# Inception3D/Motion324

Hardware: AMD Instinct MI355X
Metric: frames/sec (32-frame clip, 2048 pts, 512x512) (higher is better)
Workload: dtype bf16; 1 GPU; Motion_Latent_Model.forward inference, B=1 x 32 frames x 2048 points x 512x512 video, 4096 surface samples, training.frames=32, random-init weights (one clip per GPU; BASELINE configs[1]); the clip sits in the replayed graph's input buffers in HBM; bf16 speed mode with the decoder's residual stream in bf16 and the head fused (no [rows, C] intermediate) (secondary.headline_without_precision_shortcu; parallelism=clip-parallel x1

## Files before the change

include/m324.h:

```cpp
#ifndef M324_H
#define M324_H

#ifdef __cplusplus
extern "C" {
#endif

typedef enum { M324_OK = 0, M324_ERR_INVALID = -1, M324_ERR_HIP = -2, M324_ERR_UNSUPPORTED = -3 } m324_status;
typedef enum { M324_F32 = 0, M324_BF16 = 1, M324_MXFP8 = 2 } m324_dtype;
typedef enum { M324_ACT_NONE = 0, M324_ACT_GELU = 1 } m324_act;
typedef enum { M324_AUX_NONE = 0, M324_AUX_STORE_PREACT = 1, M324_AUX_MUL_GELU_GRAD = 2, M324_AUX_QKV_HEADS = 3,
               M324_AUX_QKV_HEADS_VT = 4, M324_AUX_N3 = 5, M324_AUX_STORE_GELU_GRAD = 6, M324_AUX_MUL = 7 } m324_aux_mode;

int m324_abi_version(void);
int m324_last_error(char* buf, int n);
int m324_device_info(char* name, int n);
int m324_set_tunable(const char* name, int value);

typedef struct {
    const void* A;  long lda;
    const void* W;  long ldw;
    void* C;        long ldc;
    int M, N, K;
    int in_dtype, out_dtype;
    const float* bias;
    int act;
    const float* gamma;
    const float* residual; long ldr; int res_rows;
    int row_gin, row_gout, row_off;
    int batch;
    long strideA, strideW, strideC;
    void* aux; long ldaux; int aux_mode;
    void* qkv_q; void* qkv_k; void* qkv_v;
    const float* qkv_qw; const float* qkv_kw;
    float qkv_eps, qkv_qscale;
    int qkv_L, qkv_H;
    const float* ln_rowstat; const float* ln_colsum;
    float* ln_stats_out;
    void* ln_copy_out; long ln_ldcopy;
    int ln_ncb; float ln_eps;
} m324_gemm_args;
int m324_gemm(const m324_gemm_args* a, void* stream);
int m324_gemm_pair(const m324_gemm_args* a, const m324_gemm_args* b, void* stream);
int m324_gemm_plan(const m324_gemm_args* a, char* buf, int n);

int m324_mx_quant(const void* x, int x_dtype, long ldx, int rows, int K, void* q, long ldq, void* s, long lds, void* stream);
int m324_layernorm_mx(const float* x, long ldx, const float* w, const float* b, float eps, int rows, int C, void* q, long ldq,
                      void* s, long lds, void* stream);
int m324_gemm_mx(const m324_gemm_args* a, const void* A_scale, long lds_a, const void* W_scale, long lds_w, void* C_scale,
                 long lds_c, void* stream);

int m324_rowstats_finish(const float* part, int ncb, int M, float eps, float* rowstat, void* stream);
int m324_rowstats(const float* x, long ldx, int rows, int C, float eps, float* rowstat, void* copy, long ldcopy, void* stream);

int m324_n3_finish(const float* part, int ncb, int M, const float* bias3, float* out, void* stream);

int m324_gemm_tn(const void* X, long ldx, const void* Y, long ldy, float* C, long ldc, int M, int N, int Kc,
                 int slices, long strideC, void* stream);

int m324_layernorm(const float* x, long ldx, const float* w, const float* b, float eps,
                   void* y, long ldy, int out_dtype, int rows, int C,
                   int gin, int gout, int off, void* stream);
int m324_layernorm_pair(const float* x0, long ldx0, const float* w0, const float* b0, float eps0, void* y0, long ldy0, int rows0,
                        int gin0, int gout0, int off0, const float* x1, long ldx1, const float* w1, const float* b1, float eps1,
                        void* y1, long ldy1, int rows1, int gin1, int gout1, int off1, int C, int out_dtype, void* stream);
int m324_layernorm_in(const void* x, int x_dtype, long ldx, const float* w, const float* b, float eps,
                      void* y, long ldy, int out_dtype, int rows, int C,
                      int gin, int gout, int off, void* stream);

int m324_qkv_split(const void* q_src, long ldq, const void* k_src, long ldk, const void* v_src, long ldv,
                   const float* q_w, const float* k_w, float eps, float q_scale,
                   void* Q, void* K, void* V, void* Qt, void* Kt, void* Vt,
                   int B, int L, int H, int dtype, void* stream);

enum { M324_ATTN_Q_PRESCALED = 1, M324_ATTN_V_ROWMAJOR = 2, M324_ATTN_SCORES_BOUNDED = 4 };
int m324_attention(const void* Q, long q_bstride, const void* K, const void* Vt, void* O, long ldo,
                   int B, int H, int Lq, int Lk, float scale, int q_prescaled, float* lse, int dtype, void* stream);
int m324_attention_plan(int B, int H, int Lq, int Lk, int flags, int dtype, char* buf, int n);

int m324_attention_merge(const void* O0, const float* lse0, const void* O1, const float* lse1, const void* O2, const float* lse2,
                         long ldp, void* O, long ldo, int B, int H, int Lq, int dtype, void* stream);

int m324_patchify(const float* video, int F, int Hin, int Win, int size, int patch,
                  void* out, int Kp, int dtype, void* stream);
int m324_patchify_u8(const unsigned char* video, int F, int Hin, int Win, int size, int patch,
                     void* out, int Kp, int dtype, void* stream);

int m324_point_encode(const float* xyz, int P, void* out, long ld, int dtype, void* stream);
int m324_point_concat(const float* normal, const float* rgb, int P, void* feat, int C, int Kp,
                      int dtype, void* stream);

int m324_dino_cls_rows(const float* cls, const float* pos0, float* x, int F, int rows_per_frame, int C,
                       void* stream);

int m324_assemble_tokens(const float* dino_x, const float* dino_w, const float* dino_b, float eps_dino,
                         const float* pos, const float* sp0, const float* spr, const float* mesh,
                         const float* ln_w, float eps_in, float* out,
                         int B, int T, int K, int P, int C, float drop_p, unsigned long long drop_seed, void* stream);

int m324_linear_n3(const void* A, long lda, const float* W, const float* bias, float* out,
                   int M, int K, int dtype, void* stream);

int m324_mse(const float* pred, const float* target, long n, float weight, float* partial, float* out,
             void* stream);

int m324_smooth_trajectories(const float* trajs, float* tmp, float* out, int B, int T, int N,
                             float threshold, float sigma, void* stream);
int m324_smooth_savgol(const float* trajs, float* out, int B, int T, int N, const double* coef, int window, void* stream);
int m324_smooth_oneeuro(const float* trajs, float* out, int B, int T, int N, float mincutoff, float beta, float dcutoff,
                        void* stream);
int m324_nearest_point(const float* query, int n_query, const float* ref, int n_ref, int* index, void* stream);

int m324_transpose(const void* in, long ld_in, void* out, long ld_out, int rows, int cols, int rows_pad,
                   int dtype, void* stream);
int m324_colsum(const void* x, long ld, float* out, int rows, int cols, int dtype, int accumulate,
                float* scratch, int scratch_rows, void* stream);
typedef struct {
    float* dst;
    const float* src;
    long ld;
    int rows, cols;
    int accumulate;
    int chain;
} m324_colsum_item;
int m324_colsum_multi(const m324_colsum_item* items, int n, void* stream);
int m324_gelu(const void* z, void* h, long n, int dtype, void* stream);
int m324_gelu_bwd(const void* z, const void* dh, void* dz, long n, int dtype, void* stream);
int m324_layernorm_bwd(const float* x, long ldx, const float* w, float eps, const void* dy, long ldy, int dy_dtype,
                       float* dx, long lddx, int accumulate, float* partial, int n_partial, int rows, int C,
                       int gin, int gout, int off, void* stream);
int m324_layernorm_bwd_cast(const float* x, long ldx, const float* w, float eps, const void* dy, long ldy, int dy_dtype,
                            float* dx, long lddx, int accumulate, float* partial, int n_partial, int rows, int C,
                            int gin, int gout, int off, void* dx_bf16, long ldc, void* stream);

int m324_cast(const void* in, long ld_in, int in_dtype, void* out, long ld_out, int out_dtype, int rows, int cols,
              void* stream);
int m324_attention_delta(const void* O, const void* dO, long ld, float* D, int B, int H, int L, int dtype, void* stream);
int m324_attention_bwd(const void* Qs, long q_bstride, const void* K, const void* V, const void* dO, const float* lse,
                       const float* D, void* dQ, void* dK, void* dV, int B, int H, int Lq, int Lk, float scale,
                       int dtype, void* stream);
int m324_attention_bwd_mfma(const void* Qs, const void* Qst, long q_bstride, long qt_bstride, const void* K, const void* Kt,
                            const void* V, const void* dO, const void* dOt, const float* lse, const float* D,
                            void* dQ, void* dK, void* dV, int B, int H, int Lq, int Lk, float scale, void* stream);
int m324_qkv_split_bwd(const void* dQ, const void* dK, const void* dV, const void* q_raw, long ldq, const void* k_raw,
                       long ldk, const float* q_w, const float* k_w, float eps, void* dq_out, long ldoq, void* dk_out,
                       long ldok, void* dv_out, long ldov, float* partial, int n_partial, int B, int L, int H, int dtype,
                       void* stream);
int m324_linear_n3_bwd(const void* A, long lda, const float* W, const float* dout, void* dA, long ldda, float* partial,
                       int n_partial, int M, int K, int dtype, const void* mul, long ldmul, void* stream);
int m324_mse_bwd(const float* pred, const float* target, const float* grad_scale, float coef, float* d, long n,
                 void* stream);
int m324_adamw(float* p, const float* g, float* m, float* v, long n, float lr, float beta1, float beta2, float eps,
               float weight_decay, int step, const float* grad_scale, void* stream);
int m324_adamw_flat(float* p, const float* g, float* m, float* v, long n, long n_decay, float lr, float beta1, float beta2,
                    float eps, float weight_decay, int step, const float* grad_scale, void* stream);
typedef struct m324_mirror_item {
    long src_off, dst_off, dstT_off;
    long first_tile;
    int rows, cols, ldT, pad_;
} m324_mirror_item;
int m324_weight_mirror(const float* src, void* dst, void* dstT, const m324_mirror_item* items_dev, int n_items, long n_tiles,
                       void* stream);
int m324_grad_sumsq(float* g, long n, int sanitize, float* partial, float* out, int accumulate, void* stream);

typedef struct m324_comm m324_comm;
int m324_comm_unique_id(char* hex, int n);
int m324_comm_init(m324_comm** comm, const char* unique_id_hex, int rank, int world);
int m324_comm_allreduce(m324_comm* comm, void* buf, long count, int dtype, int average, void* stream);
int m324_comm_allgather(m324_comm* comm, const void* send, void* recv, long count_per_rank, int dtype, void* stream);
int m324_comm_destroy(m324_comm* comm);

#ifdef __cplusplus
}
#endif
#endif
```

motion324_amd/Pcd_motion.py:

```python
from __future__ import annotations

import contextlib
import os

from typing import Dict, Optional

import torch
import torch.nn as nn
import torch.nn.functional as F

from . import ops, parallel, switches
from .easydict import EasyDict as edict
from .image_encoder import DINO_EPS, DinoEncoder
from .latent import MotionLatent
from .lib import ACT_GELU, M324Error
from .loss import MSELossComputer
from .prepared import Prepared, bump_generation, compute_dtype, pad_k
from .timing import span
from . import transformer as _transformer
from .transformer import (LN_EPS, LNFold, QK_Norm_CrossAttentionBlock, QK_Norm_TransformerBlock, fusion_off, init_weights,
                          mx_scope)

AUTO_GRAPH = switches.flag("M324_AUTO_GRAPH")
FUSE_HEAD_N3 = switches.flag("M324_FUSE_HEAD")
# ... 535 lines not shown
                    pf, Q = hoisted[b]
                elif paired is not None:
                    pf, Q = paired
                else:
                    pf = self._point_features(P, pcd[b, n0:n1], nrm[b, n0:n1].contiguous(), rgb[b, n0:n1].contiguous())
                if tchunk < T and hoisted is None and paired is None:
                    with span("stage:decoder_cross_attn_block", 0.0):
                        Q = dec.project_q(P, pf, 1, n1 - n0)
                for t0 in range(0, T, tchunk):
                    if frame_chunks:
                        t0 = min(t0, T - tchunk)
                    t1 = min(T, t0 + tchunk)
                    with span("stage:decoder_cross_attn_block", 0.0):
                        x, fold_d = self.decoder_block(P, Kd[b * T + t0:b * T + t1], Vd[b * T + t0:b * T + t1], pf,
                                                       None if (hoisted is None and paired is None and tchunk == T) else Q)
                    if cap is not None and n0 == 0 and n1 == N and tchunk == T:
                        cap.setdefault("decoder_out_t0", []).append(x[:N].clone())
                    if fold_d is not None:
                        hw, hcs, hb = P.folded(head_ln.weight, head_ln.bias, head_fc1.weight, head_fc1.bias)
                        h, lnk = fold_d.xb, dict(ln=fold_d.ln(head_ln.eps, hcs))
                    else:
                        h = torch.empty(x.shape, dtype=P.dtype, device=dev)
                        ops.layernorm(x, P.vec(head_ln.weight), P.vec(head_ln.bias), head_ln.eps, h)
                        hw, hb, lnk = P.mat(head_fc1.weight), P.vec(head_fc1.bias), {}
                    whole = n0 == 0 and n1 == N and tchunk == T
                    o = out[b] if whole else torch.empty((t1 - t0, n1 - n0, 3), dtype=torch.float32, device=dev)
                    if FUSE_HEAD_N3 and P.dtype == torch.bfloat16 and C % 256 == 0 and not torch.is_grad_enabled():
                        part = torch.empty((C // 64, x.shape[0], 3), dtype=torch.float32, device=dev)
                        ops.gemm(h, hw, None, bias=hb, act=ACT_GELU, n3=(w3, part), **lnk)
                        ops.n3_finish(part, b3, o)
                    else:
                        h2 = torch.empty(x.shape, dtype=P.dtype, device=dev)
                        ops.gemm(h, hw, h2, bias=hb, act=ACT_GELU, **lnk)
                        ops.linear_n3(h2, w3, b3, o)
                    if not whole:
                        out[b, t0:t1, n0:n1] = o
        if cap is not None and "decoder_out_t0" in cap:
            cap["decoder_out_t0"] = torch.stack(cap["decoder_out_t0"], dim=0)
        return out

    def _forward(self, sample: Dict[str, torch.Tensor], shard):
        latent_in = sample.get("m324_latent")
        encode_only = bool(sample.get("m324_encode_only", False))
        keep_latent = bool(sample.get("m324_keep_latent", False)) or encode_only
        if latent_in is not None or keep_latent:
            self._latent_guard(shard, latent_in is not None and keep_latent)
        if latent_in is not None:
            return self._forward_decode(sample, latent_in)
        ref_pcd = sample["rgb_video"] if encode_only else sample["ref_pcd"]
        dev = ref_pcd.device
        if dev.type != "cuda":
            raise M324Error("motion324_amd.Motion_Latent_Model runs only on a HIP device (model.to('cuda'), inputs on "
                            "'cuda'); there is no CPU fallback on this path")
        P = Prepared.for_module(self, dev, compute_dtype())
        mx = mx_scope(_transformer.MX_ROLES if shard is None and self.mx_effective() else ())
        cap = getattr(self, "_capture", None)
        B, N = ref_pcd.shape[0], (0 if encode_only else ref_pcd.shape[1])
        C, K = self.embed_dim, self.num_learnable_tokens
        S = sample["ref_shape_pcd"].shape[1]

        main_stream = torch.cuda.current_stream(dev)
        side = _side_stream(dev) if OVERLAP_SHAPE_ENCODER and cap is None else None
        if side is not None:
            side.wait_stream(main_stream)
        mesh_in, anchor_in = sample.get("m324_mesh_tokens"), sample.get("m324_anchor_tokens")
        keep_reuse = bool(sample.get("m324_keep_reuse", False))
        if (mesh_in is not None or anchor_in is not None) and (shard is not None or cap is not None):
            raise M324Error("m324_mesh_tokens / m324_anchor_tokens: single-GPU inference windows only")
        with torch.cuda.stream(side) if side is not None else contextlib.nullcontext():
            if mesh_in is not None:
                mesh = self._f32c(mesh_in).reshape(B * K, C)
            else:
                pts = self._point_features(P, self._f32c(sample["ref_shape_pcd"]).reshape(-1, 3),
                                           self._f32c(sample["ref_shape_normals"]), self._f32c(sample["ref_shape_rgbs"]))
                query = P.derived(f"latent_tokens_x{B}", (self.learnable_tokens,),
                                  lambda: self.learnable_tokens.detach().to(device=P.device, dtype=torch.float32).reshape(K, C).repeat(B, 1))
                mesh = self.encoder_cross_attn.run(P, query, pts, B, K, S)
                if cap is not None:
                    cap["shape_point_feat"], cap["encoder_out"] = pts.clone(), mesh.clone()
                for blk in self.points_transformer_blocks:
                    blk.run(P, mesh, B, K)
                if cap is not None:
                    cap["mesh_feat"] = mesh.clone()
            hoisted = None
            if (HOIST_DECODER_Q and side is not None and not encode_only and torch.cuda.is_current_stream_capturing()
                    and DECODE_ROWS // (sample["rgb_video"].shape[1] + (anchor_in is not None)) >= N):
                pcd_h, nrm_h, rgb_h = (self._f32c(sample[k]) for k in ("ref_pcd", "ref_normal", "ref_rgb"))
                hoisted = []
                for b in range(B):
                    pf_b = self._point_features(P, pcd_h[b], nrm_h[b].contiguous(), rgb_h[b].contiguous())
                    hoisted.append((pf_b, self.decoder_cross_attn.project_q(P, pf_b, 1, N)))

        video = sample["rgb_video"]
        T_full = video.shape[1]
        t0, kv_gather = 0, None
        if shard is not None:
            from . import parallel
            rank, world, group, t_local_of = shard
            if t_local_of is not None:
                T_full = t_local_of
            mine = parallel.partition(T_full, world, rank)
            if len(mine) == 0:
                raise M324Error(f"frame-parallel forward: {T_full} frames cannot feed {world} ranks")
            t0 = mine.start
            if t_local_of is None:
                video = video[:, mine.start:mine.stop]
            elif video.shape[1] != len(mine):
                raise M324Error(f"frame-parallel forward: rank {rank} of {world} owns {len(mine)} of {T_full} frames, rgb_video has {video.shape[1]}")
        video = video.detach().contiguous() if video.dtype == torch.uint8 else self._f32c(video)
        _, T, Hin, Win, _ = video.shape
        Pn = self.num_patches_h * self.num_patches_w
        if anchor_in is not None:
            if B != 1 or tuple(anchor_in.shape) != (1 + Pn, C):
                raise M324Error(f"m324_anchor_tokens: expected [{1 + Pn}, {C}] with one sample per call, got {tuple(anchor_in.shape)} (B = {B})")
            dino_x = torch.empty(((T + 1) * (1 + Pn), C), dtype=torch.float32, device=dev)
            ops.cast(self._f32c(anchor_in), torch.float32, out=dino_x[:1 + Pn])
            with mx:
                self.image_encoder.run(P, video.reshape(T, Hin, Win, 3), out=dino_x[1 + Pn:])
            T += 1
            T_full = T
        else:
            with mx:
                dino_x = self.image_encoder.run(P, video.reshape(B * T, Hin, Win, 3))

        if side is not None:
            main_stream.wait_stream(side)
            mesh.record_stream(main_stream)

        enc = self.image_encoder.model
        drop_p = self.drop_rate if self.training else 0.0
        drop_seed = int(torch.randint(0, 2 ** 62, (1,)).item()) if drop_p > 0.0 else 0
        pos = self._video_pos(P, T_full)[t0 * Pn:(t0 + T) * Pn]
        sp_rest = P.f32(self.special_token_rest).reshape(4, C)
        sp_first = P.f32(self.special_token_0).reshape(4, C) if t0 == 0 else sp_rest
        tok = ops.assemble_tokens(dino_x, P.vec(enc.norm.weight), P.vec(enc.norm.bias), DINO_EPS, pos, sp_first, sp_rest,
                                  mesh, P.vec(self.transformer_input_layernorm.weight),
                                  self.transformer_input_layernorm.eps, B, T, K, Pn, drop_p, drop_seed)
        Lt = 4 + K + Pn
        if cap is not None:
            dn = torch.empty((B * T * Pn, C), dtype=torch.float32, device=dev)
            ops.layernorm(dino_x, P.vec(enc.norm.weight), P.vec(enc.norm.bias), DINO_EPS, dn, row_map=(Pn, Pn + 1, 1))
            cap["dino_tokens"], cap["trunk_in"] = dn, tok.clone()

        if shard is not None and parallel.collectives_on(shard[1]):
            rank, world, group = shard[:3]
            kv_gather = _KVGather(B, T, Lt, parallel.counts(T_full, world), group, dev, rank=rank)

        fold = None
        if LNFold.usable(P, tok.shape[0], C) and "trunk.mlp" not in mx.roles:
            fold = LNFold(tok)
            if "trunk.qkv" not in mx.roles:
                fold.from_stream(tok, self.global_transformer_blocks[0].norm1.eps)
        n_pairs = len(self.global_transformer_blocks)
        for i, (gblk, lblk) in enumerate(zip(self.global_transformer_blocks, self.local_transformer_blocks)):
            with mx:
                gblk.run(P, tok, B, T * Lt, kv_gather=kv_gather, fold=fold)
                lblk.run(P, tok, B * T, Lt, fold=fold, feed_next=i + 1 < n_pairs)
            if cap is not None and "trunk_block0" not in cap:
                cap["trunk_block0"] = tok.clone()
        if cap is not None:
            cap["trunk_out"] = tok.clone()

        latent = None
        if keep_latent:
            latent = torch.empty((B * T, K * C), dtype=torch.float32, device=dev)
            ops.cast(tok.view(B * T, Lt * C)[:, 4 * C:(4 + K) * C], torch.float32, out=latent)
            latent = latent.view(B, T, K, C)
        if encode_only:
            return edict(input_data=sample, latent=latent)
        out = self._decode(P, sample, tok, (K, Lt, 4), B, T, hoisted, cap)

        if shard is not None and parallel.collectives_on(shard[1]):
            rank, world, group = shard[:3]
            frames = parallel.counts(T_full, world)
            buf = torch.zeros((max(frames), B, N, 3), dtype=torch.float32, device=dev)
            buf[:T] = out.transpose(0, 1)
            parts = torch.empty((world,) + tuple(buf.shape), dtype=torch.float32, device=dev)
            from . import graph
            seg = graph.active_segmenter()
            if seg is not None:
                seg.cut(lambda: parallel.all_gather_into(parts, buf, group=group))
            else:
                parallel.all_gather_into(parts, buf, group=group)
            if all(f == frames[0] for f in frames):
                out = parts.reshape(T_full, B, N, 3).transpose(0, 1).contiguous()
            else:
                out = torch.cat([parts[r, :f] for r, f in enumerate(frames)], dim=0).transpose(0, 1).contiguous()
        result = edict(input_data=sample, pcd_moved=out)
        if latent is not None:
            result.latent = latent
        if keep_reuse:
            Ld = 1 + Pn
            anchor = dino_x[:Ld] if B == 1 else dino_x.view(B, T, Ld, C)[:, 0].reshape(B * Ld, C).contiguous()
            result.reuse = edict(mesh_tokens=mesh, anchor_tokens=anchor)
        if "point_clouds" in sample:
            m = self.loss_computer(out, sample["point_clouds"].to(dev))
            lm = edict()
            lm.loss = m.loss
            lm.xyz_loss = m.coord_mse_loss
            result.loss_metrics = lm
        return result
```

motion324_amd/csrc/attention.hip:

```cpp
#include <stdio.h>
#include <stdlib.h>
#include <type_traits>
#include "common.h"

namespace {

constexpr int QW = 32;
constexpr int NW = 4;
constexpr int QB = QW * NW;
constexpr int KV = 64;
constexpr float LOG2E = 1.4426950408889634f;

__device__ __forceinline__ int k_off(int row, int c16) { return row * 128 + ((c16 ^ ((row >> 1) & 7)) << 4); }
typedef __attribute__((address_space(3))) void lds_ptr_t;
typedef __attribute__((address_space(1))) const void glb_ptr_t;
constexpr int ASTAGE = 16384;

__device__ __forceinline__ void dma_piece(__amdgpu_buffer_rsrc_t rs, unsigned char* lds, unsigned voff, unsigned soff) {
    __builtin_amdgcn_raw_ptr_buffer_load_lds(rs, (lds_ptr_t*)lds, 16, voff, soff, 0, 0);
}
__device__ __forceinline__ __amdgpu_buffer_rsrc_t dma_rsrc(const void* base, long bytes) {
    return __builtin_amdgcn_make_buffer_rsrc(const_cast<void*>(base), 0, (int)(bytes > 0x7FFFFFFFl ? 0x7FFFFFFFl : bytes), 0x00020000);
}


template <typename F>
__device__ __forceinline__ void store_row_chunks(const f32x16 (&acc)[2], float mul, int hi, bool ok, F&& put) {
#pragma unroll
    for (int db = 0; db < 2; ++db)
#pragma unroll
        for (int gp = 0; gp < 2; ++gp) {
            uint32_t a[2], c[2];
#pragma unroll
            for (int k = 0; k < 2; ++k) {
                a[k] = pack_bf16x2(acc[db][(2 * gp) * 4 + 2 * k] * mul, acc[db][(2 * gp) * 4 + 2 * k + 1] * mul);
                c[k] = pack_bf16x2(acc[db][(2 * gp + 1) * 4 + 2 * k] * mul, acc[db][(2 * gp + 1) * 4 + 2 * k + 1] * mul);
                const auto sw = __builtin_amdgcn_permlane32_swap(a[k], c[k], false, false);
                a[k] = sw[0];
                c[k] = sw[1];
            }
            if (ok) put(db * 4 + 2 * gp + hi, make_uint4(a[0], a[1], c[0], c[1]));
        }
}

typedef __attribute__((ext_vector_type(4))) short a_s16x4_t;
typedef __attribute__((ext_vector_type(8))) short a_s16x8_t;
typedef __attribute__((address_space(3))) a_s16x4_t a_lds_s16x4_t;

template <bool PRESCALED, int NQ, int NWV, bool VROW = false, int NST = 3>
__global__ __launch_bounds__(NWV * 64, NWV == 8 ? (VROW ? 2 : 4) : ((NST == 1 || NST == 2) ? 4 : 1)) void attn_bf16_kernel(const bf16_t* __restrict__ Q, long q_bstride,
                                                        const bf16_t* __restrict__ K, const bf16_t* __restrict__ Vt,
                                                        bf16_t* __restrict__ O, long ldo, int H, int Lq, int Lk,
                                                        int Lkp, float scale_log2e, float* __restrict__ lse, int nqt) {
    __shared__ __attribute__((aligned(1024))) unsigned char smem[NST * ASTAGE + (NST == 1 ? NWV * 4096 : 0)];
    const int tid = threadIdx.x, lane = tid & 63;
    const int wave = __builtin_amdgcn_readfirstlane(tid >> 6);
    const int l31 = lane & 31, hi = lane >> 5;
    int b = blockIdx.z, h = blockIdx.y, qt = blockIdx.x;
    if (nqt > 0) {
        const int nb = gridDim.x, q = nb >> 3, r = nb & 7, x = qt & 7, loc = qt >> 3;
        const int lid = (x < r ? x * (q + 1) : r * (q + 1) + (x - r) * q) + loc;
        qt = lid % nqt;
        h = (lid / nqt) % H;
        b = lid / (nqt * H);
    }
    const int q0 = (qt * NWV + wave) * (QW * NQ);

    const bf16_t* Qh = Q + (long)b * q_bstride + (long)h * Lq * 64;
    const bf16_t* Kh = K + ((long)b * H + h) * (long)Lk * 64;
    const bf16_t* Vh = Vt + ((long)b * H + h) * (VROW ? (long)Lk * 64 : 64 * (long)Lkp);

    bf16x8 qf[NQ][4];
#pragma unroll
    for (int n = 0; n < NQ; ++n) {
        const int q = q0 + n * QW + l31;
        const bool ok = q < Lq;
#pragma unroll
        for (int ks = 0; ks < 4; ++ks) {
            uint4 v = ok ? *reinterpret_cast<const uint4*>(Qh + (long)q * 64 + ks * 16 + hi * 8) : make_uint4(0, 0, 0, 0);
            qf[n][ks] = *reinterpret_cast<bf16x8*>(&v);
        }
    }

    constexpr int GPW = 8 / NWV;
    constexpr int PPT = 2 * GPW;
    unsigned vk[GPW], vv[GPW];
#pragma unroll
    for (int i = 0; i < GPW; ++i) {
        const int srow = (wave * GPW + i) * 8 + (lane >> 3);
        const int scol = ((lane & 7) ^ ((srow >> 1) & 7)) * 8;
        vk[i] = (unsigned)((srow * 64 + scol) * 2);
        vv[i] = VROW ? (unsigned)((srow * 64 + ((lane & 7) ^ (4 * ((srow >> 1) & 1))) * 8) * 2)
                     : (unsigned)(((long)srow * Lkp + scol) * 2);
    }
    const __amdgpu_buffer_rsrc_t rk = dma_rsrc(Kh, (long)Lk * 128);
    const __amdgpu_buffer_rsrc_t rv = dma_rsrc(Vh, VROW ? (long)Lk * 128 : 64l * Lkp * 2);
    auto issue_tile = [&](int t) {
        const int kv0 = t * KV;
        unsigned char* sk = smem + (t % NST) * ASTAGE + wave * (GPW * 1024);
        unsigned char* sv = sk + 8192;
#pragma unroll
        for (int i = 0; i < GPW; ++i) dma_piece(rk, sk + i * 1024, vk[i], (unsigned)(kv0 * 128));
#pragma unroll
        for (int i = 0; i < GPW; ++i) dma_piece(rv, sv + i * 1024, vv[i], (unsigned)(VROW ? kv0 * 128 : kv0 * 2));
    };

    f32x16 o[NQ][2];
#pragma unroll
    for (int n = 0; n < NQ; ++n)
#pragma unroll
        for (int i = 0; i < 2; ++i)
#pragma unroll
            for (int r = 0; r < 16; ++r) o[n][i][r] = 0.f;
    constexpr float THR = 8.0f;
    float m_ref[NQ], l_run[NQ];
#pragma unroll
    for (int n = 0; n < NQ; ++n) m_ref[n] = 0.f, l_run[n] = 0.f;
    bool first = true;

    const int nt = (Lk + KV - 1) / KV;
    issue_tile(0);
    if (NST != 2 && nt > 1) issue_tile(1);
    const int ko0 = k_off(l31, hi);

    const bool idle = q0 >= Lq;
    auto tiles = [&](auto guard_tag) {
        constexpr bool GUARD = decltype(guard_tag)::value;
        for (int t = 0; t < nt; ++t) {
            if (NST != 2 && t + 1 < nt) asm volatile("s_waitcnt vmcnt(%0)" ::"n"(PPT) : "memory");
            else asm volatile("s_waitcnt vmcnt(0)" ::: "memory");
            __builtin_amdgcn_s_barrier();
            asm volatile("" ::: "memory");
            if (NST == 2) {
                if (t + 1 < nt) issue_tile(t + 1);
            } else if (t + 2 < nt) issue_tile(t + 2);
            if (GUARD && idle) continue;
            const unsigned char* sk = smem + (t % NST) * ASTAGE;
            const unsigned char* sv = sk + 8192;
            const int kos = ko0 + (t % NST) * ASTAGE;

            f32x16 s[NQ][2];
    #pragma unroll
            for (int n = 0; n < NQ; ++n) {
                const float init = PRESCALED ? -m_ref[n] : -m_ref[n] / scale_log2e;
    #pragma unroll
                for (int kb = 0; kb < 2; ++kb)
    #pragma unroll
                    for (int r = 0; r < 16; ++r) s[n][kb][r] = init;
            }
            if constexpr (NQ == 1 && !VROW && NWV == 8) {
                bf16x8 kfa[8];
                auto rd = [&](int i) { kfa[i] = *reinterpret_cast<const bf16x8*>(smem + (i & 1) * 4096 + (kos ^ ((i >> 1) << 5))); };
                rd(0); rd(1); rd(2); rd(3);
                __builtin_amdgcn_sched_barrier(0);
    #pragma unroll
                for (int i = 0; i < 8; ++i) {
                    s[0][i & 1] = __builtin_amdgcn_mfma_f32_32x32x16_bf16(kfa[i], qf[0][i >> 1], s[0][i & 1], 0, 0, 0);
                    if (i + 4 < 8) rd(i + 4);
                    __builtin_amdgcn_sched_group_barrier(0x008, 1, 0);
                    if (i + 4 < 8) __builtin_amdgcn_sched_group_barrier(0x100, 1, 0);
                }
            } else {
    #pragma unroll
            for (int kb = 0; kb < 2; ++kb)
    #pragma unroll
                for (int ks = 0; ks < 4; ++ks) {
                    bf16x8 kf = *reinterpret_cast<const bf16x8*>(smem + kb * 4096 + (kos ^ (ks << 5)));
    #pragma unroll
                    for (int n = 0; n < NQ; ++n)
                        s[n][kb] = __builtin_amdgcn_mfma_f32_32x32x16_bf16(kf, qf[n][ks], s[n][kb], 0, 0, 0);
                }
            }
            if (!PRESCALED) {
    #pragma unroll
                for (int n = 0; n < NQ; ++n)
    #pragma unroll
                    for (int kb = 0; kb < 2; ++kb)
    #pragma unroll
                        for (int r = 0; r < 16; ++r) s[n][kb][r] *= scale_log2e;
            }
            const int kv0 = t * KV;
            if (kv0 + KV > Lk) {
    #pragma unroll
                for (int n = 0; n < NQ; ++n)
    #pragma unroll
                    for (int kb = 0; kb < 2; ++kb)
    #pragma unroll
                        for (int r = 0; r < 16; ++r)
                            if (kv0 + kb * 32 + (r & 3) + 8 * (r >> 2) + 4 * hi >= Lk) s[n][kb][r] = -INFINITY;
            }
            float mx[NQ];
            bool calm = true;
    #pragma unroll
            for (int n = 0; n < NQ; ++n) {
                float v = -INFINITY;
    #pragma unroll
                for (int kb = 0; kb < 2; ++kb)
    #pragma unroll
                    for (int r = 0; r < 16; ++r) v = fmaxf(v, s[n][kb][r]);
                mx[n] = v;
                calm = calm && (v <= THR);
            }
            if (first || !__all(calm)) {
    #pragma unroll
                for (int n = 0; n < NQ; ++n) {
                    mx[n] = fmaxf(mx[n], __shfl_xor(mx[n], 32, 64));
                    const float shift = first ? mx[n] : fmaxf(mx[n], 0.f);
                    const float alpha = first ? 0.f : __builtin_amdgcn_exp2f(-shift);
                    m_ref[n] += shift;
                    l_run[n] *= alpha;
    #pragma unroll
                    for (int i = 0; i < 2; ++i)
    #pragma unroll
                        for (int r = 0; r < 16; ++r) o[n][i][r] *= alpha;
    #pragma unroll
                    for (int kb = 0; kb < 2; ++kb)
    #pragma unroll
                        for (int r = 0; r < 16; ++r) s[n][kb][r] -= shift;
                }
                first = false;
            }
            bf16x8 pf[NQ][4];
    #pragma unroll
            for (int n = 0; n < NQ; ++n) {
                f32x2 rs2 = {0.f, 0.f};
    #pragma unroll
                for (int kb = 0; kb < 2; ++kb) {
                    uint32_t pk[8];
    #pragma unroll
                    for (int r = 0; r < 16; r += 2) {
                        f32x2 p = {__builtin_amdgcn_exp2f(s[n][kb][r]), __builtin_amdgcn_exp2f(s[n][kb][r + 1])};
                        rs2 += p;
                        pk[r >> 1] = pack_bf16x2(p[0], p[1]);
                    }
                    uint4 lo = make_uint4(pk[0], pk[1], pk[2], pk[3]), hi4 = make_uint4(pk[4], pk[5], pk[6], pk[7]);
                    pf[n][kb * 2] = *reinterpret_cast<bf16x8*>(&lo);
                    pf[n][kb * 2 + 1] = *reinterpret_cast<bf16x8*>(&hi4);
                }
                l_run[n] += rs2[0] + rs2[1];
            }

    #pragma unroll
            for (int j = 0; j < 4; ++j) {
    #pragma unroll
                for (int db = 0; db < 2; ++db) {
                    bf16x8 vf;
                    if constexpr (VROW) {
                        const int li = lane & 15, gg = lane >> 4;
                        const int d0 = db * 32 + 16 * (gg & 1) + 4 * (li & 3);
                        const int off = (j * 16 + 4 * hi + (li >> 2)) * 128 + (((d0 >> 3) ^ (4 * ((li >> 3) & 1))) << 4) + ((d0 & 7) << 1);
                        const a_s16x4_t lo = __builtin_amdgcn_ds_read_tr16_b64_v4i16((a_lds_s16x4_t*)(sv + off));
                        const a_s16x4_t hi4 = __builtin_amdgcn_ds_read_tr16_b64_v4i16((a_lds_s16x4_t*)(sv + off + 8 * 128));
                        const a_s16x8_t v8 = __builtin_shufflevector(lo, hi4, 0, 1, 2, 3, 4, 5, 6, 7);
                        vf = __builtin_bit_cast(bf16x8, v8);
                    } else {
                        vf = *reinterpret_cast<const bf16x8*>(smem + 8192 + db * 4096 + (kos ^ (j << 5)));
                    }
    #pragma unroll
                    for (int n = 0; n < NQ; ++n)
                        o[n][db] = __builtin_amdgcn_mfma_f32_32x32x16_bf16(vf, pf[n][j], o[n][db], 0, 0, 0);
                }
            }

        }
    };
    if (NWV == 4 && NQ == 1 && NST == 3 && (qt + 1) * NWV * QW > Lq) tiles(std::true_type{});
    else tiles(std::false_type{});

#pragma unroll
    for (int n = 0; n < NQ; ++n) {
        const float l_tot = l_run[n] + __shfl_xor(l_run[n], 32, 64);
        const float inv = 1.0f / l_tot;
        const int q = q0 + n * QW + l31;
        if (lse && q < Lq && hi == 0) lse[((long)b * H + h) * Lq + q] = m_ref[n] + log2f(l_tot);
        unsigned char* scr = NST == 1 ? smem + ASTAGE + wave * 4096 : smem + ((nt + (wave >> 2)) % NST) * ASTAGE + (wave & 3) * 4096;
        if (n > 0) asm volatile("s_waitcnt lgkmcnt(0)" ::: "memory");
#pragma unroll
        for (int db = 0; db < 2; ++db)
#pragma unroll
            for (int gp = 0; gp < 2; ++gp) {
                uint32_t a[2], c[2];
#pragma unroll
                for (int k = 0; k < 2; ++k) {
                    a[k] = pack_bf16x2(o[n][db][(2 * gp) * 4 + 2 * k] * inv, o[n][db][(2 * gp) * 4 + 2 * k + 1] * inv);
                    c[k] = pack_bf16x2(o[n][db][(2 * gp + 1) * 4 + 2 * k] * inv, o[n][db][(2 * gp + 1) * 4 + 2 * k + 1] * inv);
                    const auto sw = __builtin_amdgcn_permlane32_swap(a[k], c[k], false, false);
                    a[k] = sw[0];
                    c[k] = sw[1];
                }
                const int chunk = db * 4 + 2 * gp + hi;
                *reinterpret_cast<uint4*>(scr + l31 * 128 + ((chunk ^ (l31 & 7)) << 4)) = make_uint4(a[0], a[1], c[0], c[1]);
            }
        const int r8 = lane >> 3, c8 = lane & 7;
        bf16_t* obase = O + ((long)b * Lq + q0 + n * QW) * ldo + h * 64 + c8 * 8;
#pragma unroll
        for (int p = 0; p < 4; ++p) {
            const int r = p * 8 + r8;
            const uint4 v = *reinterpret_cast<const uint4*>(scr + r * 128 + ((c8 ^ (r & 7)) << 4));
            if (q0 + n * QW + r < Lq) *reinterpret_cast<uint4*>(obase + (long)r * ldo) = v;
        }
    }
}

template <int FB, bool NT>
__global__ __launch_bounds__(256, 3) void attn_frames_kernel(const bf16_t* __restrict__ Q, const bf16_t* __restrict__ K,
                                                             const bf16_t* __restrict__ Vt, bf16_t* __restrict__ O, long ldo, int H, int Lq,
                                                             int Lk, int Lkp, float* __restrict__ lse) {
    __shared__ __attribute__((aligned(1024))) unsigned char smem[2 * ASTAGE + 4 * 4096];
    const int tid = threadIdx.x, lane = tid & 63;
    const int wave = __builtin_amdgcn_readfirstlane(tid >> 6);
    const int l31 = lane & 31, hi = lane >> 5;
    const int h = blockIdx.y, qt = blockIdx.x, b0 = blockIdx.z * FB;
    const int q0 = (qt * 4 + wave) * QW;
    const int q = q0 + l31;
    const bf16_t* Qh = Q + (long)h * Lq * 64;
    bf16x8 qf[4];
#pragma unroll
    for (int ks = 0; ks < 4; ++ks) {
        uint4 v = q < Lq ? *reinterpret_cast<const uint4*>(Qh + (long)q * 64 + ks * 16 + hi * 8) : make_uint4(0, 0, 0, 0);
        qf[ks] = *reinterpret_cast<bf16x8*>(&v);
    }
    unsigned vk[2], vv[2];
#pragma unroll
    for (int i = 0; i < 2; ++i) {
        const int srow = (wave * 2 + i) * 8 + (lane >> 3);
        const int scol = ((lane & 7) ^ ((srow >> 1) & 7)) * 8;
        vk[i] = (unsigned)((srow * 64 + scol) * 2);
        vv[i] = (unsigned)((srow * Lkp + scol) * 2);
    }
    auto issue = [&](int j) {
        const long bh = (long)(b0 + j) * H + h;
        const __amdgpu_buffer_rsrc_t rk = dma_rsrc(K + bh * (long)Lk * 64, (long)Lk * 128);
        const __amdgpu_buffer_rsrc_t rv = dma_rsrc(Vt + bh * 64 * Lkp, 64l * Lkp * 2);
        unsigned char* sk = smem + (j & 1) * ASTAGE + wave * 2048;
#pragma unroll
        for (int i = 0; i < 2; ++i) dma_piece(rk, sk + i * 1024, vk[i], 0u);
#pragma unroll
        for (int i = 0; i < 2; ++i) dma_piece(rv, sk + 8192 + i * 1024, vv[i], 0u);
    };
    unsigned char* scr = smem + 2 * ASTAGE + wave * 4096;
    const int r8 = lane >> 3, c8 = lane & 7;
    auto flush = [&](int j) {
        bf16_t* obase = O + ((long)(b0 + j) * Lq + q0) * ldo + h * 64 + c8 * 8;
#pragma unroll
        for (int p = 0; p < 4; ++p) {
            const int r = p * 8 + r8;
            const uint4 v = *reinterpret_cast<const uint4*>(scr + r * 128 + ((c8 ^ (r & 7)) << 4));
            if (q0 + r < Lq) {
                if (NT) __builtin_nontemporal_store(*reinterpret_cast<const f32x4*>(&v), reinterpret_cast<f32x4*>(obase + (long)r * ldo));
                else *reinterpret_cast<uint4*>(obase + (long)r * ldo) = v;
            }
        }
    };
    const int ko0 = k_off(l31, hi);
    issue(0);
#pragma unroll 1
    for (int j = 0; j < FB; ++j) {
        asm volatile("s_waitcnt vmcnt(0)" ::: "memory");
        __builtin_amdgcn_s_barrier();
        asm volatile("" ::: "memory");
        if (j + 1 < FB) issue(j + 1);
        if (j > 0) flush(j - 1);
        const int kos = ko0 + (j & 1) * ASTAGE;
        f32x16 s[2];
#pragma unroll
        for (int kb = 0; kb < 2; ++kb) {
#pragma unroll
            for (int r = 0; r < 16; ++r) s[kb][r] = 0.f;
#pragma unroll
            for (int ks = 0; ks < 4; ++ks) {
                const bf16x8 kf = *reinterpret_cast<const bf16x8*>(smem + kb * 4096 + (kos ^ (ks << 5)));
                s[kb] = __builtin_amdgcn_mfma_f32_32x32x16_bf16(kf, qf[ks], s[kb], 0, 0, 0);
            }
        }
        if (Lk < KV) {
#pragma unroll
            for (int kb = 0; kb < 2; ++kb)
#pragma unroll
                for (int r = 0; r < 16; ++r)
                    if (kb * 32 + (r & 3) + 8 * (r >> 2) + 4 * hi >= Lk) s[kb][r] = -INFINITY;
        }
        float mx = -INFINITY;
#pragma unroll
        for (int kb = 0; kb < 2; ++kb)
#pragma unroll
            for (int r = 0; r < 16; ++r) mx = fmaxf(mx, s[kb][r]);
        mx = fmaxf(mx, __shfl_xor(mx, 32, 64));
        f32x2 rs2 = {0.f, 0.f};
        bf16x8 pf[4];
#pragma unroll
        for (int kb = 0; kb < 2; ++kb) {
            uint32_t pk[8];
#pragma unroll
            for (int r = 0; r < 16; r += 2) {
                f32x2 p = {__builtin_amdgcn_exp2f(s[kb][r] - mx), __builtin_amdgcn_exp2f(s[kb][r + 1] - mx)};
                rs2 += p;
                pk[r >> 1] = pack_bf16x2(p[0], p[1]);
            }
            uint4 lo = make_uint4(pk[0], pk[1], pk[2], pk[3]), hi4 = make_uint4(pk[4], pk[5], pk[6], pk[7]);
            pf[kb * 2] = *reinterpret_cast<bf16x8*>(&lo);
            pf[kb * 2 + 1] = *reinterpret_cast<bf16x8*>(&hi4);
        }
        f32x16 o[2];
#pragma unroll
        for (int db = 0; db < 2; ++db) {
#pragma unroll
            for (int r = 0; r < 16; ++r) o[db][r] = 0.f;
#pragma unroll
            for (int jj = 0; jj < 4; ++jj) {
                const bf16x8 vf = *reinterpret_cast<const bf16x8*>(smem + 8192 + db * 4096 + (kos ^ (jj << 5)));
                o[db] = __builtin_amdgcn_mfma_f32_32x32x16_bf16(vf, pf[jj], o[db], 0, 0, 0);
            }
        }
        float l_tot = rs2[0] + rs2[1];
        l_tot += __shfl_xor(l_tot, 32, 64);
        const float inv = 1.0f / l_tot;
        if (lse && q < Lq && hi == 0) lse[((long)(b0 + j) * H + h) * Lq + q] = mx + log2f(l_tot);
        store_row_chunks(o, inv, hi, true, [&](int chunk, uint4 v) {
            *reinterpret_cast<uint4*>(scr + l31 * 128 + ((chunk ^ (l31 & 7)) << 4)) = v;
        });
    }
    flush(FB - 1);
}


template <int NWV>
__device__ __forceinline__ void dma_rows(unsigned char* part, __amdgpu_buffer_rsrc_t rs, long row_stride, int row0, long col0, int wave,
                                         int lane) {
    constexpr int G = 8 / NWV;
    const unsigned soff = (unsigned)(((long)row0 * row_stride + col0) * 2);
#pragma unroll
    for (int i = 0; i < G; ++i) {
        const int r = (wave * G + i) * 8 + (lane >> 3);
        const int c = (lane & 7) ^ ((r >> 1) & 7);
        __builtin_amdgcn_raw_ptr_buffer_load_lds(rs, (lds_ptr_t*)(part + (wave * G + i) * 8 * 128), 16,
                                                 (unsigned)(((long)r * row_stride + c * 8) * 2), soff, 0, 0);
    }
}

__device__ __forceinline__ void pack_frags(const f32x16 (&x)[2], bf16x8 (&f)[4]) {
#pragma unroll
    for (int kb = 0; kb < 2; ++kb) {
        uint32_t pk[8];
#pragma unroll
        for (int r = 0; r < 16; r += 2) pk[r >> 1] = pack_bf16x2(x[kb][r], x[kb][r + 1]);
        uint4 lo = make_uint4(pk[0], pk[1], pk[2], pk[3]), hi4 = make_uint4(pk[4], pk[5], pk[6], pk[7]);
        f[kb * 2] = *reinterpret_cast<bf16x8*>(&lo);
        f[kb * 2 + 1] = *reinterpret_cast<bf16x8*>(&hi4);
    }
}

template <int NWV>
__global__ __launch_bounds__(NWV * 64) void attn_bwd_dq_mfma_kernel(const bf16_t* __restrict__ Qs, long q_bstride,
                                                               const bf16_t* __restrict__ K, const bf16_t* __restrict__ V,
// ... 413 lines not shown
        }
        float mx = -INFINITY;
#pragma unroll
        for (int kb = 0; kb < 2; ++kb)
#pragma unroll
            for (int r = 0; r < 16; ++r) mx = fmaxf(mx, s[kb][r]);
        mx = fmaxf(mx, __shfl_xor(mx, 32, 64));
        const float m_new = fmaxf(m_run, mx * scale_log2e);
        const float alpha = exp2f(m_run - m_new);
        m_run = m_new;
        float rs = 0.f;
#pragma unroll
        for (int kb = 0; kb < 2; ++kb)
#pragma unroll
            for (int r = 0; r < 16; ++r) {
                s[kb][r] = exp2f(fmaf(s[kb][r], scale_log2e, -m_new));
                rs += s[kb][r];
            }
        l_run = l_run * alpha + rs;
#pragma unroll
        for (int i = 0; i < 2; ++i)
#pragma unroll
            for (int r = 0; r < 16; ++r) o[i][r] *= alpha;
#pragma unroll
        for (int kb = 0; kb < 2; ++kb)
#pragma unroll
            for (int r = 0; r < 16; ++r) {
                const int kv = kb * 32 + (r & 3) + 8 * (r >> 2) + 4 * hi;
#pragma unroll
                for (int db = 0; db < 2; ++db)
                    o[db] = __builtin_amdgcn_mfma_f32_32x32x2f32(sv[(db * 32 + l31) * FLD + kv], s[kb][r], o[db], 0, 0, 0);
            }
    }
    const float l_tot = l_run + __shfl_xor(l_run, 32, 64);
    const float inv = 1.0f / l_tot;
    const int q = q0 + l31;
    if (lse && q < Lq && hi == 0) lse[((long)b * H + h) * Lq + q] = m_run + log2f(l_tot);
    if (q < Lq) {
        float* orow = O + ((long)b * Lq + q) * ldo + h * 64;
#pragma unroll
        for (int db = 0; db < 2; ++db)
#pragma unroll
            for (int g = 0; g < 4; ++g) {
                float4 w = make_float4(o[db][g * 4 + 0] * inv, o[db][g * 4 + 1] * inv, o[db][g * 4 + 2] * inv,
                                       o[db][g * 4 + 3] * inv);
                *reinterpret_cast<float4*>(orow + db * 32 + g * 8 + hi * 4) = w;
            }
    }
}

}

void m324_attn_pwg_launch(const void* Q, long q_bstride, const void* K, const void* Vt, void* O, long ldo, int B, int H, int Lq, int Lk,
                          float* lse, bool bounded, hipStream_t s);

enum AttnFamily { ATTN_F32, ATTN_PWG, ATTN_PWG_BOUNDED, ATTN_FRAMES, ATTN_BF16 };
struct AttnPlan {
    AttnFamily family;
    bool ps, vrow;
    int nw, nst;
    dim3 grid;
    unsigned threads;
    int nqt;
};

static AttnPlan attn_plan(int B, int H, int Lq, int Lk, int flags, int dtype) {
    AttnPlan p{};
    p.nw = NW, p.nst = 3, p.threads = 256;
    p.grid = dim3(ceil_div(Lq, QB), H, B);
    if (dtype != M324_BF16) {
        p.family = ATTN_F32;
        return p;
    }
    const bool vrow = (flags & M324_ATTN_V_ROWMAJOR) != 0, ps = (flags & M324_ATTN_Q_PRESCALED) != 0;
    const int fnw = m324::tunable(m324::TUN_ATTN_NW);
    const bool w8 = fnw ? fnw == 8 : (Lq >= 2048 && Lk >= 512);
    if (m324::tunable(m324::TUN_ATTN_PWG) != 0 && ps && !vrow && fnw == 0 && Lq >= 2048 && Lk >= 512) {
        p.family = (flags & M324_ATTN_SCORES_BOUNDED) ? ATTN_PWG_BOUNDED : ATTN_PWG;
        p.grid = dim3((unsigned)((long)ceil_div(Lq, 256) * H * B));
        return p;
    }
    p.family = ATTN_BF16, p.ps = ps, p.vrow = vrow, p.nw = w8 ? 8 : 4, p.threads = p.nw * 64;
    p.grid.x = ceil_div(Lq, w8 ? 2 * QB : QB);
    const bool one_tile = ps && !w8 && !vrow && Lk <= KV;
    if (w8 || (!one_tile && p.grid.x > 1 && (long)p.grid.x * H * B >= 512)) {
        p.nqt = (int)p.grid.x;
        p.grid = dim3(p.grid.x * H * B, 1, 1);
    }
    if (ps && !w8 && Lk > KV && Lk <= 16 * KV) {
        p.nst = 2;
    } else if (one_tile && (flags & 256) && B % 2 == 0 && Lq >= 512 && m324::tunable(m324::TUN_ATTN_EXP) != 8) {
        p.family = ATTN_FRAMES;
        p.grid.z = B / 2;
    } else if (one_tile) {
        p.nst = 1;
    }
    return p;
}

static constexpr int attn_key(bool ps, int nw, bool vrow, int nst) { return (int)ps | nw << 1 | (int)vrow << 5 | nst << 6; }

extern "C" int m324_attention(const void* Q, long q_bstride, const void* K, const void* Vt, void* O, long ldo, int B,
                              int H, int Lq, int Lk, float scale, int q_prescaled, float* lse, int dtype, void* stream) {
    M324_REQUIRE(Q && K && Vt && O, "m324_attention: null pointer");
    M324_REQUIRE(B > 0 && H > 0 && Lq > 0 && Lk > 0, "m324_attention: empty problem B=%d H=%d Lq=%d Lk=%d", B, H, Lq, Lk);
    M324_REQUIRE(ldo >= (long)H * 64, "m324_attention: ldo too small");
    M324_REQUIRE(H <= 65535 && B <= 65535, "m324_attention: grid too large");
    M324_REQUIRE(!(q_prescaled & M324_ATTN_V_ROWMAJOR) || dtype == M324_BF16, "m324_attention: row-major V needs the bf16 kernel (transposing LDS reads)");
    if (dtype != M324_BF16 && dtype != M324_F32) M324_FAIL(M324_ERR_UNSUPPORTED, "m324_attention: dtype %d", dtype);
    M324_REQUIRE(dtype == M324_BF16 ? (ldo * 2) % 8 == 0 : ldo % 4 == 0, "m324_attention: ldo misaligned");
    const int Lkp = (Lk + 63) / 64 * 64;
    hipStream_t s = (hipStream_t)stream;
    const float sl = (q_prescaled & M324_ATTN_Q_PRESCALED) ? 1.0f : scale * LOG2E;
    const AttnPlan p = attn_plan(B, H, Lq, Lk, (q_prescaled & 7) | (q_bstride == 0 ? 256 : 0), dtype);
#define M324_ATTN(PS, NWV, VROW, NST)                                                                                   \
    case attn_key(PS, NWV, VROW, NST):                                                                                  \
        hipLaunchKernelGGL((attn_bf16_kernel<PS, 1, NWV, VROW, NST>), p.grid, dim3(p.threads), 0, s,                    \
                           (const bf16_t*)Q, q_bstride, (const bf16_t*)K, (const bf16_t*)Vt, (bf16_t*)O, ldo, H, Lq, Lk, \
                           Lkp, sl, lse, p.nqt);                                                                         \
        break
    switch (p.family) {
        case ATTN_F32:
            hipLaunchKernelGGL(attn_f32_kernel, p.grid, dim3(p.threads), 0, s, (const float*)Q, q_bstride, (const float*)K,
                               (const float*)Vt, (float*)O, ldo, H, Lq, Lk, Lkp, sl, lse);
            break;
        case ATTN_PWG:
        case ATTN_PWG_BOUNDED:
            M324_REQUIRE((long)ceil_div(Lq, 256) * H * B < (1l << 31), "m324_attention: grid too large");
            m324_attn_pwg_launch(Q, q_bstride, K, Vt, O, ldo, B, H, Lq, Lk, lse, p.family == ATTN_PWG_BOUNDED, s);
            break;
        case ATTN_FRAMES:
            hipLaunchKernelGGL((attn_frames_kernel<2, true>), p.grid, dim3(p.threads), 0, s, (const bf16_t*)Q,
                               (const bf16_t*)K, (const bf16_t*)Vt, (bf16_t*)O, ldo, H, Lq, Lk, Lkp, lse);
            break;
        case ATTN_BF16:
            switch (attn_key(p.ps, p.nw, p.vrow, p.nst)) {
                M324_ATTN(true, 4, false, 3); M324_ATTN(true, 8, false, 3);
                M324_ATTN(false, 4, false, 3); M324_ATTN(false, 8, false, 3);
                M324_ATTN(true, 4, true, 3); M324_ATTN(true, 8, true, 3);
                M324_ATTN(false, 4, true, 3); M324_ATTN(false, 8, true, 3);
                M324_ATTN(true, 4, false, 2); M324_ATTN(true, 4, true, 2);
                M324_ATTN(true, 4, false, 1);
                default:
                    M324_FAIL(M324_ERR_UNSUPPORTED, "m324_attention: attn_bf16_kernel<%d, 1, %d, %d, %d> is not built", (int)p.ps, p.nw,
                              (int)p.vrow, p.nst);
            }
            break;
    }
#undef M324_ATTN
    M324_CHECK_LAUNCH("m324_attention");
    return M324_OK;
}

extern "C" int m324_attention_plan(int B, int H, int Lq, int Lk, int flags, int dtype, char* buf, int n) {
    M324_REQUIRE(buf && n > 0 && B > 0 && H > 0 && Lq > 0 && Lk > 0, "m324_attention_plan: bad arguments");
    const AttnPlan p = attn_plan(B, H, Lq, Lk, flags, dtype);
    const char* tf[2] = {"false", "true"};
    char name[96];
    switch (p.family) {
        case ATTN_F32: snprintf(name, sizeof(name), "attn_f32_kernel"); break;
        case ATTN_PWG: snprintf(name, sizeof(name), "attn_pwg_kernel"); break;
        case ATTN_PWG_BOUNDED: snprintf(name, sizeof(name), "attn_pwg_bounded_kernel"); break;
        case ATTN_FRAMES: snprintf(name, sizeof(name), "attn_frames_kernel<2, true>"); break;
        case ATTN_BF16: snprintf(name, sizeof(name), "attn_bf16_kernel<%s, 1, %d, %s, %d>", tf[p.ps], p.nw, tf[p.vrow], p.nst); break;
    }
    snprintf(buf, (size_t)n, "%s grid=%ldx%ux%u", name, (long)p.grid.x * p.threads, p.grid.y, p.grid.z);
    return p.family == ATTN_F32 ? 0 : p.nw;
}

extern "C" int m324_attention_bwd_mfma(const void* Qs, const void* Qst, long q_bstride, long qt_bstride, const void* K,
                                       const void* Kt, const void* V, const void* dO, const void* dOt, const float* lse,
                                       const float* D, void* dQ, void* dK, void* dV, int B, int H, int Lq, int Lk, float scale,
                                       void* stream) {
    M324_REQUIRE(Qs && Qst && K && Kt && V && dO && dOt && lse && D && dQ && dK && dV, "m324_attention_bwd_mfma: null pointer");
    M324_REQUIRE(B > 0 && H > 0 && Lq > 0 && Lk > 0 && H <= 65535 && B <= 65535, "m324_attention_bwd_mfma: bad sizes");
    const int Lkp = (Lk + 63) / 64 * 64, Lqp = (Lq + 63) / 64 * 64;
    hipStream_t s = (hipStream_t)stream;
    const int fbw = m324::tunable(m324::TUN_ATTN_BWD_NW);
    const bool big = Lk >= 1024;
    const bool dq8 = fbw == 8 || fbw == 84, dkv8 = fbw == 8 || fbw == 48 || fbw == 2;
    if (fbw == 2 && big)
        hipLaunchKernelGGL(attn_bwd_dq2_mfma_kernel, dim3(ceil_div(Lq, 2 * QB), H, B), dim3(256), 0, s, (const bf16_t*)Qs, q_bstride,
                           (const bf16_t*)K, (const bf16_t*)V, (const bf16_t*)Kt, (const bf16_t*)dO, lse, D, (bf16_t*)dQ, H, Lq, Lk, Lkp, scale);
    else if (dq8)
        hipLaunchKernelGGL(attn_bwd_dq_mfma_kernel<8>, dim3(ceil_div(Lq, 2 * QB), H, B), dim3(512), 0, s, (const bf16_t*)Qs,
                           q_bstride, (const bf16_t*)K, (const bf16_t*)V, (const bf16_t*)Kt, (const bf16_t*)dO, lse, D,
                           (bf16_t*)dQ, H, Lq, Lk, Lkp, scale);
    else
        hipLaunchKernelGGL(attn_bwd_dq_mfma_kernel<4>, dim3(ceil_div(Lq, QB), H, B), dim3(256), 0, s, (const bf16_t*)Qs,
                           q_bstride, (const bf16_t*)K, (const bf16_t*)V, (const bf16_t*)Kt, (const bf16_t*)dO, lse, D,
                           (bf16_t*)dQ, H, Lq, Lk, Lkp, scale);
    if (dkv8)
        hipLaunchKernelGGL(attn_bwd_dkv_mfma_kernel<8>, dim3(ceil_div(Lk, 2 * QB), H, B), dim3(512), 0, s, (const bf16_t*)Qs,
                           (const bf16_t*)Qst, q_bstride, qt_bstride, (const bf16_t*)K, (const bf16_t*)V, (const bf16_t*)dO,
                           (const bf16_t*)dOt, lse, D, (bf16_t*)dK, (bf16_t*)dV, H, Lq, Lk, Lqp);
    else
        hipLaunchKernelGGL(attn_bwd_dkv_mfma_kernel<4>, dim3(ceil_div(Lk, QB), H, B), dim3(256), 0, s, (const bf16_t*)Qs,
                           (const bf16_t*)Qst, q_bstride, qt_bstride, (const bf16_t*)K, (const bf16_t*)V, (const bf16_t*)dO,
                           (const bf16_t*)dOt, lse, D, (bf16_t*)dK, (bf16_t*)dV, H, Lq, Lk, Lqp);
    M324_CHECK_LAUNCH("m324_attention_bwd_mfma");
    return M324_OK;
}
```

motion324_amd/csrc/elementwise.hip:

```cpp
#include "common.h"

namespace {

constexpr int LN_MAXV = 4;

__device__ __forceinline__ long remap_row(long r, int gin, int gout, int off) {
    return gin > 0 ? (r / gin) * gout + (r % gin) + off : r;
}

#define LN_FOR(i, c) _Pragma("unroll") for (int i = 0, c = lane * 4; i < LN_MAXV; ++i, c += 256) if (c < C)

__device__ __forceinline__ void row_load(float4 (&v)[LN_MAXV], const float* src, int lane, int C) {
    LN_FOR(i, c) v[i] = *reinterpret_cast<const float4*>(src + c);
}
__device__ __forceinline__ void row_stats(const float4 (&v)[LN_MAXV], int lane, int C, float eps, float& mean, float& rstd) {
    float s = 0.f;
    LN_FOR(i, c) s += v[i].x + v[i].y + v[i].z + v[i].w;
    mean = wave_sum(s) / (float)C;
    float q = 0.f;
    LN_FOR(i, c) {
        float a = v[i].x - mean, b = v[i].y - mean, cc = v[i].z - mean, d = v[i].w - mean;
        q += a * a + b * b + cc * cc + d * d;
    }
    rstd = rsqrtf(wave_sum(q) / (float)C + eps);
}

template <typename T>
__device__ __forceinline__ void store4(T* p, float a, float b, float c, float d);
template <>
__device__ __forceinline__ void store4<float>(float* p, float a, float b, float c, float d) {
    *reinterpret_cast<float4*>(p) = make_float4(a, b, c, d);
}
template <>
__device__ __forceinline__ void store4<bf16_t>(bf16_t* p, float a, float b, float c, float d) {
    *reinterpret_cast<uint2*>(p) = make_uint2(pack_bf16x2(a, b), pack_bf16x2(c, d));
}
template <typename T>
__device__ __forceinline__ float4 load4(const T* p);
template <>
__device__ __forceinline__ float4 load4<float>(const float* p) { return *reinterpret_cast<const float4*>(p); }
template <>
__device__ __forceinline__ float4 load4<bf16_t>(const bf16_t* p) {
    uint2 u = *reinterpret_cast<const uint2*>(p);
    return make_float4(__uint_as_float(u.x << 16), __uint_as_float(u.x & 0xffff0000u), __uint_as_float(u.y << 16),
                       __uint_as_float(u.y & 0xffff0000u));
}

template <typename T, typename TX = float>
__global__ __launch_bounds__(256) void layernorm1_kernel(const TX* __restrict__ x, long ldx, const float* __restrict__ w,
                                                         const float* __restrict__ b, float eps, T* __restrict__ y, long ldy,
                                                         int rows, int C, int gin, int gout, int off) {
    const int lane = threadIdx.x & 63;
    const long row = (long)blockIdx.x * 4 + (threadIdx.x >> 6);
    if (row >= rows) return;
    const TX* xr = x + remap_row(row, gin, gout, off) * ldx;
    float4 v[LN_MAXV];
    LN_FOR(i, c) v[i] = load4<TX>(xr + c);
    float mean, rstd;
    row_stats(v, lane, C, eps, mean, rstd);
    T* yr = y + row * ldy;
    LN_FOR(i, c) {
        float4 ww = *reinterpret_cast<const float4*>(w + c);
        float4 bb = b ? *reinterpret_cast<const float4*>(b + c) : make_float4(0.f, 0.f, 0.f, 0.f);
        store4<T>(yr + c, (v[i].x - mean) * rstd * ww.x + bb.x, (v[i].y - mean) * rstd * ww.y + bb.y,
                  (v[i].z - mean) * rstd * ww.z + bb.z, (v[i].w - mean) * rstd * ww.w + bb.w);
    }
}

template <typename T, typename TX = float>
__device__ __forceinline__ void ln_rows2(const TX* __restrict__ x, long ldx, const float* __restrict__ w, const float* __restrict__ b,
                                         float eps, T* __restrict__ y, long ldy, int rows, int C, int gin, int gout, int off, int block) {
    const int lane = threadIdx.x & 63;
    const long row0 = (long)block * 8 + (threadIdx.x >> 6) * 2;
    if (row0 >= rows) return;
    const bool two = row0 + 1 < rows;
    const long row1 = two ? row0 + 1 : row0;
    const TX* xa = x + remap_row(row0, gin, gout, off) * ldx;
    const TX* xb = x + remap_row(row1, gin, gout, off) * ldx;
    float4 va[LN_MAXV], vb[LN_MAXV];
    LN_FOR(i, c) { va[i] = load4<TX>(xa + c); vb[i] = load4<TX>(xb + c); }
    float sa = 0.f, sb = 0.f;
    LN_FOR(i, c) { sa += va[i].x + va[i].y + va[i].z + va[i].w; sb += vb[i].x + vb[i].y + vb[i].z + vb[i].w; }
    wave_sum2(sa, sb);
    const float ma = sa / (float)C, mb = sb / (float)C;
    float qa = 0.f, qb = 0.f;
    LN_FOR(i, c) {
        float p = va[i].x - ma, q = va[i].y - ma, r = va[i].z - ma, t = va[i].w - ma;
        qa += p * p + q * q + r * r + t * t;
        p = vb[i].x - mb, q = vb[i].y - mb, r = vb[i].z - mb, t = vb[i].w - mb;
        qb += p * p + q * q + r * r + t * t;
    }
    wave_sum2(qa, qb);
    const float ra = rsqrtf(qa / (float)C + eps), rb = rsqrtf(qb / (float)C + eps);
    T* ya = y + row0 * ldy;
    T* yb = y + row1 * ldy;
    LN_FOR(i, c) {
        const float4 ww = *reinterpret_cast<const float4*>(w + c);
        const float4 bb = b ? *reinterpret_cast<const float4*>(b + c) : make_float4(0.f, 0.f, 0.f, 0.f);
        store4<T>(ya + c, (va[i].x - ma) * ra * ww.x + bb.x, (va[i].y - ma) * ra * ww.y + bb.y,
                  (va[i].z - ma) * ra * ww.z + bb.z, (va[i].w - ma) * ra * ww.w + bb.w);
        store4<T>(yb + c, (vb[i].x - mb) * rb * ww.x + bb.x, (vb[i].y - mb) * rb * ww.y + bb.y,
                  (vb[i].z - mb) * rb * ww.z + bb.z, (vb[i].w - mb) * rb * ww.w + bb.w);
    }
}

template <typename T, typename TX = float>
__global__ __launch_bounds__(256) void layernorm_kernel(const TX* __restrict__ x, long ldx, const float* __restrict__ w,
                                                        const float* __restrict__ b, float eps, T* __restrict__ y, long ldy,
                                                        int rows, int C, int gin, int gout, int off) {
    ln_rows2<T, TX>(x, ldx, w, b, eps, y, ldy, rows, C, gin, gout, off, (int)blockIdx.x);
}

struct LnProblem {
    const float* x; long ldx;
    const float* w; const float* b; float eps;
    void* y; long ldy;
    int rows, gin, gout, off;
};
template <typename T>
__global__ __launch_bounds__(256) void layernorm_pair_kernel(LnProblem p0, LnProblem p1, int C, int blocks0) {
    if ((int)blockIdx.x < blocks0)
        ln_rows2<T, float>(p0.x, p0.ldx, p0.w, p0.b, p0.eps, (T*)p0.y, p0.ldy, p0.rows, C, p0.gin, p0.gout, p0.off, (int)blockIdx.x);
    else
        ln_rows2<T, float>(p1.x, p1.ldx, p1.w, p1.b, p1.eps, (T*)p1.y, p1.ldy, p1.rows, C, p1.gin, p1.gout, p1.off, (int)blockIdx.x - blocks0);
}

__global__ __launch_bounds__(256) void rowstats_finish_kernel(const float2* __restrict__ part, int ncb, int M, float eps,
                                                              float2* __restrict__ rowstat) {
    const long m = (long)blockIdx.x * 256 + threadIdx.x;
    if (m >= M) return;
    if ((ncb & 1) == 0) {
        const int h = ncb >> 1;
        float mean[2], m2[2];
        for (int half = 0; half < 2; ++half) {
            const float2 p0 = part[(long)(half * h) * M + m];
            mean[half] = p0.x * (1.0f / 64.0f), m2[half] = p0.y;
            for (int i = 1; i < h; ++i) {
                const float2 pb = part[(long)(half * h + i) * M + m];
                const float d = pb.x * (1.0f / 64.0f) - mean[half];
                mean[half] = fmaf(d, 1.0f / (float)(i + 1), mean[half]);
                m2[half] = m2[half] + fmaf(d * d, 64.0f * (float)i / (float)(i + 1), pb.y);
            }
        }
        const float d = mean[1] - mean[0];
        const float mm2 = (m2[0] + m2[1]) + (d * d) * (32.0f * (float)h);
        const float mean_ = fmaf(0.5f, d, mean[0]);
        const float rstd = rsqrtf(mm2 / (64.0f * (float)ncb) + eps);
        rowstat[m] = make_float2(rstd, -rstd * mean_);
        return;
    }
    float s = 0.f;
    for (int b = 0; b < ncb; ++b) s += part[(long)b * M + m].x;
    const float n = 64.0f * (float)ncb, mean = s / n;
    float m2 = 0.f;
    for (int b = 0; b < ncb; ++b) {
        const float2 pb = part[(long)b * M + m];
        const float d = pb.x * (1.0f / 64.0f) - mean;
        m2 += fmaf(64.0f * d, d, pb.y);
    }
    const float rstd = rsqrtf(m2 / n + eps);
    rowstat[m] = make_float2(rstd, -rstd * mean);
}

__global__ __launch_bounds__(256) void rowstats_kernel(const float* __restrict__ x, long ldx, int rows, int C, float eps,
                                                       float2* __restrict__ rowstat, bf16_t* __restrict__ copy, long ldcopy) {
    const int lane = threadIdx.x & 63;
    const long row = (long)blockIdx.x * 4 + (threadIdx.x >> 6);
    if (row >= rows) return;
    float4 v[LN_MAXV];
    row_load(v, x + row * ldx, lane, C);
    float mean, rstd;
    row_stats(v, lane, C, eps, mean, rstd);
    if (lane == 0) rowstat[row] = make_float2(rstd, -rstd * mean);
    if (copy) {
        LN_FOR(i, c) store4<bf16_t>(copy + row * ldcopy + c, v[i].x, v[i].y, v[i].z, v[i].w);
    }
}

template <typename T>
__global__ __launch_bounds__(256) void qkv_split_kernel(const T* __restrict__ qs, long ldq, const T* __restrict__ ks, long ldk,
                                                        const T* __restrict__ vs, long ldv, const float* __restrict__ qw,
                                                        const float* __restrict__ kw, float eps, float q_scale,
                                                        T* __restrict__ Q, T* __restrict__ K, T* __restrict__ V,
                                                        T* __restrict__ Qt, T* __restrict__ Kt, T* __restrict__ Vt, int L, int H,
                                                        int Lp) {
    __shared__ float tile[64][65];
    const int t = threadIdx.x, tok = t >> 2, part = t & 3;
    const int b = blockIdx.z, h = blockIdx.y, l0 = blockIdx.x * 64;
    const int l = l0 + tok;
    const bool ok = l < L;
    const long srow = (long)b * L + l;
    const long hbase = ((long)b * H + h);

    auto one = [&](const T* src, long ld, const float* w, float post, T* dst, T* dstT) {
        float v[16];
        if (ok) {
            const T* p = src + srow * ld + h * 64 + part * 16;
            float lo[8], hi8[8];
            load8(p, lo);
            load8(p + 8, hi8);
#pragma unroll
            for (int i = 0; i < 8; ++i) { v[i] = lo[i]; v[8 + i] = hi8[i]; }
        } else {
#pragma unroll
            for (int i = 0; i < 16; ++i) v[i] = 0.f;
        }
        if (w) {
            float ss = 0.f;
#pragma unroll
            for (int i = 0; i < 16; ++i) ss += v[i] * v[i];
            ss += __shfl_xor(ss, 1, 64);
            ss += __shfl_xor(ss, 2, 64);
            const float r = rsqrtf(ss * (1.0f / 64.0f) + eps);
#pragma unroll
            for (int i = 0; i < 16; ++i) v[i] = v[i] * r * w[part * 16 + i];
        }
        if (post != 1.0f) {
#pragma unroll
            for (int i = 0; i < 16; ++i) v[i] *= post;
        }
        if (dst && ok) {
            T* o = dst + (hbase * L + l) * 64 + part * 16;
            const float lo[8] = {v[0], v[1], v[2], v[3], v[4], v[5], v[6], v[7]};
            const float hi8[8] = {v[8], v[9], v[10], v[11], v[12], v[13], v[14], v[15]};
            store8(o, lo);
            store8(o + 8, hi8);
        }
        if (dstT) {
            __syncthreads();
#pragma unroll
            for (int i = 0; i < 16; ++i) tile[part * 16 + i][tok] = v[i];
            __syncthreads();
            const int d = t >> 2;
            T* o = dstT + (hbase * 64 + d) * (long)Lp + l0 + part * 16;
            const float* tr = &tile[d][part * 16];
            const float c0[8] = {tr[0], tr[1], tr[2], tr[3], tr[8], tr[9], tr[10], tr[11]};
            const float c1[8] = {tr[4], tr[5], tr[6], tr[7], tr[12], tr[13], tr[14], tr[15]};
            store8(o, c0);
            store8(o + 8, c1);
        }
    };
    if (qs) one(qs, ldq, qw, q_scale, Q, Qt);
    if (ks) one(ks, ldk, kw, 1.0f, K, Kt);
    if (vs) one(vs, ldv, nullptr, 1.0f, V, Vt);
}

template <typename TIN>
__device__ __forceinline__ float patch_tap(const TIN* p, int c) {
    if constexpr (sizeof(TIN) == 1) return (float)p[c] / 255.0f;
    else return p[c];
}
template <typename T, typename TIN>
__global__ __launch_bounds__(256) void patchify_kernel(const TIN* __restrict__ video, int F, int Hin, int Win, int size,
                                                       int patch, T* __restrict__ out, int Kp) {
    const long idx = (long)blockIdx.x * 256 + threadIdx.x;
    const long total = (long)F * size * size;
    if (idx >= total) return;
    const int ox = (int)(idx % size), oy = (int)((idx / size) % size), f = (int)(idx / ((long)size * size));
    const float sh = (float)Hin / (float)size, sw = (float)Win / (float)size;
    float fy = fmaxf(sh * ((float)oy + 0.5f) - 0.5f, 0.f), fx = fmaxf(sw * ((float)ox + 0.5f) - 0.5f, 0.f);
    const int y0 = min((int)fy, Hin - 1), x0 = min((int)fx, Win - 1);
    const int y1 = min(y0 + 1, Hin - 1), x1 = min(x0 + 1, Win - 1);
    const float ly = fy - (float)y0, lx = fx - (float)x0;
    const float hy = 1.f - ly, hx = 1.f - lx;
    const TIN* base = video + (long)f * Hin * Win * 3;
    const TIN* p00 = base + ((long)y0 * Win + x0) * 3;
    const TIN* p01 = base + ((long)y0 * Win + x1) * 3;
    const TIN* p10 = base + ((long)y1 * Win + x0) * 3;
    const TIN* p11 = base + ((long)y1 * Win + x1) * 3;
    const float mean[3] = {0.485f, 0.456f, 0.406f}, stdv[3] = {0.229f, 0.224f, 0.225f};
    const int g = size / patch;
    const int py = oy / patch, ky = oy % patch, px = ox / patch, kx = ox % patch;
    T* orow = out + ((long)f * g * g + (long)py * g + px) * Kp;
#pragma unroll
    for (int c = 0; c < 3; ++c) {
        const float v = hy * (hx * patch_tap(p00, c) + lx * patch_tap(p01, c)) + ly * (hx * patch_tap(p10, c) + lx * patch_tap(p11, c));
        Elem<T>::store(orow + c * patch * patch + ky * patch + kx, (v - mean[c]) / stdv[c]);
    }
    if (ky == 0 && kx == 0)
        for (int c = 3 * patch * patch; c < Kp; ++c) Elem<T>::store(orow + c, 0.f);
}

template <typename T>
__global__ __launch_bounds__(256) void point_encode_kernel(const float* __restrict__ xyz, int P, T* __restrict__ out, long ld) {
    const long idx = (long)blockIdx.x * 256 + threadIdx.x;
    const long p = idx >> 6;
    const int c = (int)(idx & 63);
    if (p >= P) return;
    float v = 0.f;
    if (c < 48) {
        const int cc = c % 24, axis = cc >> 3, j = cc & 7;
        const float e = (float)(1 << j) * 3.14159274101257324f;
        const float arg = xyz[p * 3 + axis] * e;
        v = c < 24 ? sinf(arg) : cosf(arg);
    } else if (c < 51) {
        v = xyz[p * 3 + (c - 48)];
    }
    Elem<T>::store(out + p * ld + c, v);
}

template <typename T>
__global__ __launch_bounds__(256) void point_concat_kernel(const float* __restrict__ normal, const float* __restrict__ rgb,
                                                           int P, T* __restrict__ feat, int C, int Kp) {
    const int w = Kp - C;
    const long idx = (long)blockIdx.x * 256 + threadIdx.x;
    const long p = idx / w;
    const int c = (int)(idx % w);
    if (p >= P) return;
    float v = 0.f;
    if (c < 3) v = normal[p * 3 + c];
    else if (c < 6) v = rgb[p * 3 + c - 3];
    Elem<T>::store(feat + p * Kp + C + c, v);
}

__global__ void dino_cls_kernel(const float* __restrict__ cls, const float* __restrict__ pos0, float* __restrict__ x, int F,
                                int rpf, int C) {
    const long idx = (long)blockIdx.x * 256 + threadIdx.x;
    if (idx >= (long)F * C) return;
    const int c = (int)(idx % C);
    const long f = idx / C;
    x[f * rpf * C + c] = cls[c] + pos0[c];
}

__device__ __forceinline__ unsigned long long splitmix64(unsigned long long x) {
    unsigned long long z = x + 0x9E3779B97F4A7C15ull;
    z = (z ^ (z >> 30)) * 0xBF58476D1CE4E5B9ull;
    z = (z ^ (z >> 27)) * 0x94D049BB133111EBull;
    return z ^ (z >> 31);
// ... 438 lines not shown
        for (int k = 0; k < 8; ++k) {
            const float cdf = 0.5f * (1.0f + erff(x[k] * 0.70710678118654752440f));
            const float pdf = 0.39894228040143267794f * expf(-0.5f * x[k] * x[k]);
            g[k] *= cdf + x[k] * pdf;
        }
        store8(dz + i * 8, g);
    }
}

constexpr int LNB_WAVES = 8;
template <typename T, bool CAST>
__global__ __launch_bounds__(64 * LNB_WAVES) void layernorm_bwd_kernel(const float* __restrict__ x, long ldx, const float* __restrict__ w,
                                                            float eps, const T* __restrict__ dy, long ldy,
                                                            float* __restrict__ dx, long lddx, int accumulate,
                                                            float* __restrict__ partial, int rows, int C, int gin, int gout,
                                                            int off, bf16_t* __restrict__ dxc, long ldc) {
    constexpr int NB = CAST ? 3 : 2;
    extern __shared__ float lnb_red[];
    const int lane = threadIdx.x & 63, wave = threadIdx.x >> 6;
    const int gw = blockIdx.x * LNB_WAVES + wave, nw = gridDim.x * LNB_WAVES;
    float4 pw[LN_MAXV], pb[LN_MAXV], pc[CAST ? LN_MAXV : 1];
    LN_FOR(i, c) { pw[i] = make_float4(0.f, 0.f, 0.f, 0.f); pb[i] = make_float4(0.f, 0.f, 0.f, 0.f); if (CAST) pc[i] = pw[i]; }
    for (long row = gw; row < rows; row += nw) {
        const long xr = remap_row(row, gin, gout, off);
        float4 v[LN_MAXV];
        row_load(v, x + xr * ldx, lane, C);
        float mean, rstd;
        row_stats(v, lane, C, eps, mean, rstd);
        float4 g[LN_MAXV];
        float s1 = 0.f, s2 = 0.f;
        LN_FOR(i, c) {
            const float4 d = load4<T>(dy + row * ldy + c);
            const float4 ww = *reinterpret_cast<const float4*>(w + c);
            v[i].x = (v[i].x - mean) * rstd; v[i].y = (v[i].y - mean) * rstd;
            v[i].z = (v[i].z - mean) * rstd; v[i].w = (v[i].w - mean) * rstd;
            pw[i].x += d.x * v[i].x; pw[i].y += d.y * v[i].y; pw[i].z += d.z * v[i].z; pw[i].w += d.w * v[i].w;
            pb[i].x += d.x; pb[i].y += d.y; pb[i].z += d.z; pb[i].w += d.w;
            g[i] = make_float4(d.x * ww.x, d.y * ww.y, d.z * ww.z, d.w * ww.w);
            s1 += g[i].x + g[i].y + g[i].z + g[i].w;
            s2 += g[i].x * v[i].x + g[i].y * v[i].y + g[i].z * v[i].z + g[i].w * v[i].w;
        }
        s1 = wave_sum(s1) / (float)C;
        s2 = wave_sum(s2) / (float)C;
        float* dr = dx + xr * lddx;
        LN_FOR(i, c) {
            float4 o = make_float4(rstd * (g[i].x - s1 - v[i].x * s2), rstd * (g[i].y - s1 - v[i].y * s2),
                                   rstd * (g[i].z - s1 - v[i].z * s2), rstd * (g[i].w - s1 - v[i].w * s2));
            if (accumulate) {
                const float4 p = *reinterpret_cast<const float4*>(dr + c);
                o.x += p.x; o.y += p.y; o.z += p.z; o.w += p.w;
            }
            *reinterpret_cast<float4*>(dr + c) = o;
            if constexpr (CAST) {
                const uint32_t lo = pack_bf16x2(o.x, o.y), hi2 = pack_bf16x2(o.z, o.w);
                *reinterpret_cast<uint2*>(dxc + xr * ldc + c) = make_uint2(lo, hi2);
                pc[i].x += __uint_as_float(lo << 16); pc[i].y += __uint_as_float(lo & 0xFFFF0000u);
                pc[i].z += __uint_as_float(hi2 << 16); pc[i].w += __uint_as_float(hi2 & 0xFFFF0000u);
            }
        }
    }
    float* mine = lnb_red + wave * 2 * C;
    LN_FOR(i, c) {
        *reinterpret_cast<float4*>(mine + c) = pw[i];
        *reinterpret_cast<float4*>(mine + C + c) = pb[i];
    }
    __syncthreads();
    float* pr = partial + (long)blockIdx.x * NB * C;
    for (int c = threadIdx.x; c < 2 * C; c += 64 * LNB_WAVES) {
        float a = lnb_red[c];
#pragma unroll
        for (int w = 1; w < LNB_WAVES; ++w) a += lnb_red[w * 2 * C + c];
        pr[c] = a;
    }
    if constexpr (CAST) {
        __syncthreads();
        LN_FOR(i, c) *reinterpret_cast<float4*>(mine + c) = pc[i];
        __syncthreads();
        for (int c = threadIdx.x; c < C; c += 64 * LNB_WAVES) {
            float a = lnb_red[c];
#pragma unroll
            for (int w = 1; w < LNB_WAVES; ++w) a += lnb_red[w * 2 * C + c];
            pr[2 * C + c] = a;
        }
    }
}

__global__ __launch_bounds__(256) void n3_finish_kernel(const float* __restrict__ part, int ncb, int M, const float* __restrict__ bias3,
                                                        float* __restrict__ out) {
    const long i = (long)blockIdx.x * 256 + threadIdx.x;
    if (i >= (long)M * 3) return;
    float s = bias3[i % 3];
    for (int cb = 0; cb < ncb; ++cb) s += part[(long)cb * M * 3 + i];
    out[i] = s;
}

template <typename T>
__global__ __launch_bounds__(256) void attention_merge_kernel(const T* __restrict__ O0, const float* __restrict__ l0, const T* __restrict__ O1,
                                                              const float* __restrict__ l1, const T* __restrict__ O2,
                                                              const float* __restrict__ l2, long ldp, T* __restrict__ O, long ldo, int B,
                                                              int H, int Lq) {
    const long i = (long)blockIdx.x * 256 + threadIdx.x;
    const int cpr = H * 8;
    if (i >= (long)B * Lq * cpr) return;
    const long row = i / cpr;
    const int c = (int)(i - row * cpr), h = c >> 3;
    const long b = row / Lq, q = row - b * Lq;
    const long li = (b * H + h) * Lq + q;
    const float a0 = l0[li], a1 = l1[li], a2 = O2 ? l2[li] : -INFINITY;
    const float m = fmaxf(a0, fmaxf(a1, a2));
    float w0 = exp2f(a0 - m), w1 = exp2f(a1 - m), w2 = O2 ? exp2f(a2 - m) : 0.f;
    const float inv = 1.0f / (w0 + w1 + w2);
    w0 *= inv, w1 *= inv, w2 *= inv;
    float x[8], y[8];
    load8(O0 + row * ldp + c * 8, x);
    load8(O1 + row * ldp + c * 8, y);
#pragma unroll
    for (int e = 0; e < 8; ++e) x[e] = w0 * x[e] + w1 * y[e];
    if (O2) {
        load8(O2 + row * ldp + c * 8, y);
#pragma unroll
        for (int e = 0; e < 8; ++e) x[e] = fmaf(w2, y[e], x[e]);
    }
    store8(O + row * ldo + c * 8, x);
}

}

#define DISPATCH_DTYPE(dtype, name, ...)                                  \
    if ((dtype) == M324_BF16) { using T = bf16_t; __VA_ARGS__; }          \
    else if ((dtype) == M324_F32) { using T = float; __VA_ARGS__; }       \
    else M324_FAIL(M324_ERR_UNSUPPORTED, name ": dtype %d", (int)(dtype))

extern "C" int m324_rowstats_finish(const float* part, int ncb, int M, float eps, float* rowstat, void* stream) {
    M324_REQUIRE(part && rowstat && ncb > 0 && M > 0, "m324_rowstats_finish: bad arguments (ncb=%d M=%d)", ncb, M);
    M324_REQUIRE(((uintptr_t)part % 8) == 0 && ((uintptr_t)rowstat % 8) == 0, "m324_rowstats_finish: tables must be 8-byte aligned");
    hipLaunchKernelGGL(rowstats_finish_kernel, dim3(ceil_div(M, 256)), dim3(256), 0, (hipStream_t)stream,
                       reinterpret_cast<const float2*>(part), ncb, M, eps, reinterpret_cast<float2*>(rowstat));
    M324_CHECK_LAUNCH("m324_rowstats_finish");
    return M324_OK;
}

extern "C" int m324_rowstats(const float* x, long ldx, int rows, int C, float eps, float* rowstat, void* copy, long ldcopy,
                             void* stream) {
    M324_REQUIRE(x && rowstat && rows > 0, "m324_rowstats: bad arguments");
    M324_REQUIRE(C % 4 == 0 && C > 0 && C <= 256 * LN_MAXV && ldx % 4 == 0 && ldx >= C, "m324_rowstats: C=%d ldx=%ld unsupported", C, ldx);
    M324_REQUIRE(((uintptr_t)rowstat % 8) == 0 && (!copy || (ldcopy % 4 == 0 && ldcopy >= C && ((uintptr_t)copy % 8) == 0)),
                 "m324_rowstats: misaligned outputs");
    hipLaunchKernelGGL(rowstats_kernel, dim3(ceil_div(rows, 4)), dim3(256), 0, (hipStream_t)stream, x, ldx, rows, C, eps,
                       reinterpret_cast<float2*>(rowstat), static_cast<bf16_t*>(copy), ldcopy);
    M324_CHECK_LAUNCH("m324_rowstats");
    return M324_OK;
}

extern "C" int m324_layernorm_in(const void* x, int x_dtype, long ldx, const float* w, const float* b, float eps, void* y, long ldy,
                                 int out_dtype, int rows, int C, int gin, int gout, int off, void* stream) {
    if (x_dtype == M324_F32) return m324_layernorm((const float*)x, ldx, w, b, eps, y, ldy, out_dtype, rows, C, gin, gout, off, stream);
    M324_REQUIRE(x && w && y, "m324_layernorm_in: null pointer");
    M324_REQUIRE(x_dtype == M324_BF16 && out_dtype == M324_BF16, "m324_layernorm_in: a bf16 input needs a bf16 output");
    M324_REQUIRE(rows > 0 && C % 4 == 0 && C > 0 && C <= 256 * LN_MAXV && ldx % 4 == 0 && ldy % 4 == 0,
                 "m324_layernorm_in: rows=%d C=%d ldx=%ld ldy=%ld unsupported", rows, C, ldx, ldy);
    if (m324::tunable(m324::TUN_LN_ROWS) == 1)
        hipLaunchKernelGGL((layernorm1_kernel<bf16_t, bf16_t>), dim3(ceil_div(rows, 4)), dim3(256), 0, (hipStream_t)stream,
                           (const bf16_t*)x, ldx, w, b, eps, (bf16_t*)y, ldy, rows, C, gin, gout, off);
    else
    hipLaunchKernelGGL((layernorm_kernel<bf16_t, bf16_t>), dim3(ceil_div(rows, 8)), dim3(256), 0, (hipStream_t)stream,
                       (const bf16_t*)x, ldx, w, b, eps, (bf16_t*)y, ldy, rows, C, gin, gout, off);
    M324_CHECK_LAUNCH("m324_layernorm_in");
    return M324_OK;
}

extern "C" int m324_layernorm(const float* x, long ldx, const float* w, const float* b, float eps, void* y, long ldy,
                              int out_dtype, int rows, int C, int gin, int gout, int off, void* stream) {
    M324_REQUIRE(x && w && y, "m324_layernorm: null pointer");
    M324_REQUIRE(rows > 0, "m324_layernorm: rows=%d", rows);
    M324_REQUIRE(C % 4 == 0 && C > 0 && C <= 256 * LN_MAXV, "m324_layernorm: C=%d unsupported", C);
    M324_REQUIRE(ldx % 4 == 0 && ldy % 4 == 0, "m324_layernorm: leading dims must be multiples of 4");
    hipStream_t s = (hipStream_t)stream;
    if (m324::tunable(m324::TUN_LN_ROWS) == 1) {
        DISPATCH_DTYPE(out_dtype, "m324_layernorm",
                       hipLaunchKernelGGL(layernorm1_kernel<T>, dim3(ceil_div(rows, 4)), dim3(256), 0, s, x, ldx, w, b, eps,
                                          (T*)y, ldy, rows, C, gin, gout, off));
    } else {
        DISPATCH_DTYPE(out_dtype, "m324_layernorm",
                       hipLaunchKernelGGL(layernorm_kernel<T>, dim3(ceil_div(rows, 8)), dim3(256), 0, s, x, ldx, w, b, eps,
                                          (T*)y, ldy, rows, C, gin, gout, off));
    }
    M324_CHECK_LAUNCH("m324_layernorm");
    return M324_OK;
}

extern "C" int m324_layernorm_pair(const float* x0, long ldx0, const float* w0, const float* b0, float eps0, void* y0, long ldy0, int rows0,
                                   int gin0, int gout0, int off0, const float* x1, long ldx1, const float* w1, const float* b1, float eps1,
                                   void* y1, long ldy1, int rows1, int gin1, int gout1, int off1, int C, int out_dtype, void* stream) {
    M324_REQUIRE(x0 && w0 && y0 && x1 && w1 && y1, "m324_layernorm_pair: null pointer");
    M324_REQUIRE(rows0 > 0 && rows1 > 0, "m324_layernorm_pair: rows=%d, %d", rows0, rows1);
    M324_REQUIRE(C % 4 == 0 && C > 0 && C <= 256 * LN_MAXV, "m324_layernorm_pair: C=%d unsupported", C);
    M324_REQUIRE(ldx0 % 4 == 0 && ldy0 % 4 == 0 && ldx1 % 4 == 0 && ldy1 % 4 == 0, "m324_layernorm_pair: leading dims must be multiples of 4");
    const LnProblem p0{x0, ldx0, w0, b0, eps0, y0, ldy0, rows0, gin0, gout0, off0}, p1{x1, ldx1, w1, b1, eps1, y1, ldy1, rows1, gin1, gout1, off1};
    const int blocks0 = ceil_div(rows0, 8);
    hipStream_t s = (hipStream_t)stream;
    DISPATCH_DTYPE(out_dtype, "m324_layernorm_pair",
                   hipLaunchKernelGGL(layernorm_pair_kernel<T>, dim3(blocks0 + ceil_div(rows1, 8)), dim3(256), 0, s, p0, p1, C, blocks0));
    M324_CHECK_LAUNCH("m324_layernorm_pair");
    return M324_OK;
}

extern "C" int m324_qkv_split(const void* q_src, long ldq, const void* k_src, long ldk, const void* v_src, long ldv,
                              const float* q_w, const float* k_w, float eps, float q_scale, void* Q, void* K, void* V, void* Qt,
                              void* Kt, void* Vt, int B, int L, int H, int dtype, void* stream) {
    M324_REQUIRE(B > 0 && L > 0 && H > 0, "m324_qkv_split: empty problem");
    M324_REQUIRE((!q_src || Q || Qt) && (!k_src || K || Kt) && (!v_src || V || Vt), "m324_qkv_split: missing output");
    const int al = dtype == M324_BF16 ? 8 : 4;
    M324_REQUIRE(ldq % al == 0 && ldk % al == 0 && ldv % al == 0, "m324_qkv_split: leading dims must be multiples of %d", al);
    const int Lp = (L + 63) / 64 * 64;
    dim3 grid(Lp / 64, H, B);
    hipStream_t s = (hipStream_t)stream;
    DISPATCH_DTYPE(dtype, "m324_qkv_split",
                   hipLaunchKernelGGL(qkv_split_kernel<T>, grid, dim3(256), 0, s, (const T*)q_src, ldq, (const T*)k_src, ldk,
                                      (const T*)v_src, ldv, q_w, k_w, eps, q_scale, (T*)Q, (T*)K, (T*)V, (T*)Qt, (T*)Kt, (T*)Vt,
                                      L, H, Lp));
    M324_CHECK_LAUNCH("m324_qkv_split");
    return M324_OK;
}

template <typename TIN>
static int patchify_launch(const TIN* video, int F, int Hin, int Win, int size, int patch, void* out, int Kp, int dtype, void* stream, const char* what) {
    M324_REQUIRE(video && out, "%s: null pointer", what);
    M324_REQUIRE(F > 0 && Hin > 0 && Win > 0 && size > 0 && patch > 0 && size % patch == 0, "%s: bad geometry", what);
    M324_REQUIRE(Kp >= 3 * patch * patch, "%s: Kp=%d too small", what, Kp);
    const long total = (long)F * size * size;
    hipStream_t s = (hipStream_t)stream;
    if (dtype == M324_BF16)
        hipLaunchKernelGGL((patchify_kernel<bf16_t, TIN>), dim3(ceil_div(total, 256)), dim3(256), 0, s, video, F, Hin, Win, size, patch, (bf16_t*)out, Kp);
    else if (dtype == M324_F32)
        hipLaunchKernelGGL((patchify_kernel<float, TIN>), dim3(ceil_div(total, 256)), dim3(256), 0, s, video, F, Hin, Win, size, patch, (float*)out, Kp);
    else
        M324_FAIL(M324_ERR_UNSUPPORTED, "%s: dtype %d", what, dtype);
    M324_CHECK_LAUNCH(what);
    return M324_OK;
}

extern "C" int m324_patchify(const float* video, int F, int Hin, int Win, int size, int patch, void* out, int Kp, int dtype,
                             void* stream) {
    return patchify_launch<float>(video, F, Hin, Win, size, patch, out, Kp, dtype, stream, "m324_patchify");
}

extern "C" int m324_patchify_u8(const unsigned char* video, int F, int Hin, int Win, int size, int patch, void* out, int Kp, int dtype,
                                void* stream) {
    return patchify_launch<unsigned char>(video, F, Hin, Win, size, patch, out, Kp, dtype, stream, "m324_patchify_u8");
}

extern "C" int m324_point_encode(const float* xyz, int P, void* out, long ld, int dtype, void* stream) {
    M324_REQUIRE(xyz && out && P > 0 && ld >= 64, "m324_point_encode: bad arguments");
    hipStream_t s = (hipStream_t)stream;
    DISPATCH_DTYPE(dtype, "m324_point_encode",
                   hipLaunchKernelGGL(point_encode_kernel<T>, dim3(ceil_div((long)P * 64, 256)), dim3(256), 0, s, xyz, P,
                                      (T*)out, ld));
    M324_CHECK_LAUNCH("m324_point_encode");
    return M324_OK;
}

extern "C" int m324_point_concat(const float* normal, const float* rgb, int P, void* feat, int C, int Kp, int dtype,
                                 void* stream) {
    M324_REQUIRE(normal && rgb && feat && P > 0 && Kp >= C + 6, "m324_point_concat: bad arguments");
    hipStream_t s = (hipStream_t)stream;
    DISPATCH_DTYPE(dtype, "m324_point_concat",
                   hipLaunchKernelGGL(point_concat_kernel<T>, dim3(ceil_div((long)P * (Kp - C), 256)), dim3(256), 0, s,
                                      normal, rgb, P, (T*)feat, C, Kp));
    M324_CHECK_LAUNCH("m324_point_concat");
    return M324_OK;
}

extern "C" int m324_dino_cls_rows(const float* cls, const float* pos0, float* x, int F, int rows_per_frame, int C,
                                  void* stream) {
    M324_REQUIRE(cls && pos0 && x && F > 0 && C > 0, "m324_dino_cls_rows: bad arguments");
    hipLaunchKernelGGL(dino_cls_kernel, dim3(ceil_div((long)F * C, 256)), dim3(256), 0, (hipStream_t)stream, cls, pos0, x, F,
                       rows_per_frame, C);
    M324_CHECK_LAUNCH("m324_dino_cls_rows");
    return M324_OK;
}

extern "C" int m324_assemble_tokens(const float* dino_x, const float* dino_w, const float* dino_b, float eps_dino,
                                    const float* pos, const float* sp0, const float* spr, const float* mesh,
                                    const float* ln_w, float eps_in, float* out, int B, int T, int K, int P, int C,
                                    float drop_p, unsigned long long drop_seed, void* stream) {
    M324_REQUIRE(dino_x && dino_w && dino_b && pos && sp0 && spr && mesh && out, "m324_assemble_tokens: null pointer");
    M324_REQUIRE(drop_p >= 0.f && drop_p < 1.f, "m324_assemble_tokens: drop_p=%g outside [0,1)", (double)drop_p);
    const unsigned drop_thr = (unsigned)(drop_p * 16777216.0f);
    const float drop_scale = 1.0f / (1.0f - drop_p);
    M324_REQUIRE(C % 4 == 0 && C <= 256 * LN_MAXV, "m324_assemble_tokens: C=%d unsupported", C);
    const long rows = (long)B * T * (4 + K + P);
    hipLaunchKernelGGL(assemble_kernel, dim3(ceil_div(rows, 4)), dim3(256), 0, (hipStream_t)stream, dino_x, dino_w, dino_b,
                       eps_dino, pos, sp0, spr, mesh, ln_w, eps_in, out, B, T, K, P, C, drop_thr, drop_scale, drop_seed);
    M324_CHECK_LAUNCH("m324_assemble_tokens");
    return M324_OK;
}

extern "C" int m324_attention_merge(const void* O0, const float* lse0, const void* O1, const float* lse1, const void* O2, const float* lse2,
                                    long ldp, void* O, long ldo, int B, int H, int Lq, int dtype, void* stream) {
    M324_REQUIRE(O0 && lse0 && O1 && lse1 && O && (!O2 == !lse2), "m324_attention_merge: two or three (output, lse) parts");
    M324_REQUIRE(B > 0 && H > 0 && Lq > 0 && ldp >= (long)H * 64 && ldo >= (long)H * 64, "m324_attention_merge: bad sizes");
    const int esz = dtype == M324_BF16 ? 2 : 4;
    M324_REQUIRE((ldp * esz) % 16 == 0 && (ldo * esz) % 16 == 0 && ((uintptr_t)O0 % 16) == 0 && ((uintptr_t)O1 % 16) == 0 &&
                     ((uintptr_t)O2 % 16) == 0 && ((uintptr_t)O % 16) == 0,
                 "m324_attention_merge: rows must be 16-byte aligned");
    const long n = (long)B * Lq * H * 8;
// ... 254 lines not shown
```

motion324_amd/csrc/gemm.hip:

```cpp

#include <stdio.h>
#include "gemm_tile.h"

namespace {

template <typename TIN, typename TOUT>
__global__ __launch_bounds__(256, 2) void gemm_kernel(const TIN* __restrict__ A, long lda, const TIN* __restrict__ W,
                                                      long ldw, TOUT* C, long ldc, int M, int N, int K,
                                                      Epilogue ep) {
    __shared__ __attribute__((aligned(16))) unsigned char smem[4 * TILE_BYTES];
    constexpr int EPC = Elem<TIN>::PER16;
    constexpr int BK = ROWB / sizeof(TIN);

    const int tid = threadIdx.x, lane = tid & 63, wave = tid >> 6;
    const int wm = wave >> 1, wn = wave & 1;
    const int l31 = lane & 31, hi = lane >> 5;
    const int m0 = blockIdx.y * BM, n0 = blockIdx.x * BN;

    int srow[4], schk[4];
    const TIN* ga[4];
    const TIN* gb[4];
    bool aval[4], bval[4];
#pragma unroll
    for (int i = 0; i < 4; ++i) {
// ... 1015 lines not shown
    }
    if (rc != M324_OK) return rc;
    M324_CHECK_LAUNCH("m324_gemm");
    return M324_OK;
}

}


extern "C" int m324_gemm_plan(const m324_gemm_args* a, char* buf, int n) {
    M324_REQUIRE(a && buf && n > 0, "m324_gemm_plan: bad arguments");
    const GemmPlan p = make_plan(a);
    const char* tout = a->out_dtype == M324_BF16 ? "unsigned short" : "float";
    const char* tin = a->in_dtype == M324_BF16 ? "unsigned short" : "float";
    char targs[64];
    if (p.variant == 1) snprintf(targs, sizeof(targs), "%s, %s", tin, tout);
    else if (p.variant == 9) snprintf(targs, sizeof(targs), "%s, %d", tout, p.actx);
    else if (p.variant == 2 || p.variant == 5) snprintf(targs, sizeof(targs), "%s, %s, %d, %d", tin, tout, p.actx, p.res);
    else snprintf(targs, sizeof(targs), "%s, %d, %d", tout, p.actx, p.res);
    snprintf(buf, (size_t)n, "%s<%s> grid=%ldx%dx1", p.name, targs, p.wg * p.threads, p.grid_y);
    return p.variant;
}

extern "C" int m324_gemm_tn(const void* X, long ldx, const void* Y, long ldy, float* C, long ldc, int M, int N, int Kc,
                            int slices, long strideC, void* stream) {
    M324_REQUIRE(X && Y && C, "m324_gemm_tn: null pointer");
    M324_REQUIRE(M > 0 && N >= 8 && Kc >= 8 && N % 8 == 0 && Kc % 8 == 0, "m324_gemm_tn: bad sizes M=%d N=%d Kc=%d", M, N, Kc);
    M324_REQUIRE(ldx >= N && ldy >= Kc && ldx % 8 == 0 && ldy % 8 == 0 && ldc >= Kc && ldc % 4 == 0 &&
                     ((uintptr_t)X % 16) == 0 && ((uintptr_t)Y % 16) == 0 && ((uintptr_t)C % 16) == 0,
                 "m324_gemm_tn: operands must be 16-byte aligned with leading dimensions that are multiples of 8");
    M324_REQUIRE(slices >= 1 && slices <= 65535 && (slices == 1 || strideC >= (long)N * ldc), "m324_gemm_tn: bad slicing");
    const int ks = ((M + slices - 1) / slices + 63) / 64 * 64;
    M324_REQUIRE((long)ks * (slices - 1) < M, "m324_gemm_tn: %d slices leave an empty slice for M=%d", slices, M);
    M324_REQUIRE(((long)ks + 64) * (ldx > ldy ? ldx : ldy) * 2 < 0x7FFFFFFFl,
                 "m324_gemm_tn: a slice of %d tokens x leading dimension %ld exceeds the 2 GiB the staging offsets cover; use more slices",
                 ks, ldx > ldy ? ldx : ldy);
    const bool big = m324::tunable(m324::TUN_GEMM_TN) != 128 && M % 32 == 0 && N % 256 == 0 && Kc % 256 == 0 && M / slices >= 256;
    if (big) {
        const int ntj = Kc / 256;
        const int ntiles = (N / 256) * ntj;
        hipLaunchKernelGGL(gemm_tn_pipe_kernel, dim3(ntiles * slices), dim3(512), 0, (hipStream_t)stream, (const bf16_t*)X, ldx,
                           (const bf16_t*)Y, ldy, C, ldc, M, N, Kc, ks, strideC, ntj, ntiles, slices, m324::tunable(m324::TUN_XCD) & 1);
    } else {
        const int ntj = ceil_div(Kc, 128), ntiles = ceil_div(N, 128) * ntj;
        hipLaunchKernelGGL(gemm_tn_kernel, dim3(ntiles * slices), dim3(256), 0, (hipStream_t)stream, (const bf16_t*)X, ldx,
                           (const bf16_t*)Y, ldy, C, ldc, M, N, Kc, ks, strideC, ntj, ntiles, slices, m324::tunable(m324::TUN_XCD) & 1);
    }
    M324_CHECK_LAUNCH("m324_gemm_tn");
    return M324_OK;
}

static int gemm_validate(const m324_gemm_args* a) {
    const bool qkv_mode = a && (a->aux_mode == M324_AUX_QKV_HEADS || a->aux_mode == M324_AUX_QKV_HEADS_VT);
    const bool n3_mode = a && a->aux_mode == M324_AUX_N3;
    M324_REQUIRE(a && a->A && a->W && (a->C || qkv_mode || n3_mode), "m324_gemm: null pointer");
    M324_REQUIRE(a->M > 0 && a->N > 0 && a->K > 0, "m324_gemm: empty problem M=%d N=%d K=%d", a->M, a->N, a->K);
    const int bk = a->in_dtype == M324_BF16 ? 64 : 32;
    M324_REQUIRE(a->K % bk == 0, "m324_gemm: K=%d must be a multiple of %d", a->K, bk);
    const int esz = a->in_dtype == M324_BF16 ? 2 : 4;
    M324_REQUIRE((a->lda * esz) % 16 == 0 && (a->ldw * esz) % 16 == 0 && ((uintptr_t)a->A % 16) == 0 &&
                     ((uintptr_t)a->W % 16) == 0,
                 "m324_gemm: A/W rows must be 16-byte aligned");
    M324_REQUIRE(a->lda >= a->K && a->ldw >= a->K && a->ldc >= a->N, "m324_gemm: leading dimension too small");
    M324_REQUIRE(257l * (a->lda > a->ldw ? a->lda : a->ldw) * esz + (long)a->K * esz < 0x7FFFFFFFl,
                 "m324_gemm: leading dimension %ld too large for the 256-row staging window", a->lda > a->ldw ? a->lda : a->ldw);
    M324_REQUIRE(!a->residual || a->ldr >= a->N, "m324_gemm: ldr too small");
    M324_REQUIRE(a->batch <= 1 || (vec_ok(a) && !a->residual && a->batch <= 65535),
                 "m324_gemm: a batched launch needs a vectorisable, residual-free problem");
    M324_REQUIRE(a->aux_mode >= 0 && a->aux_mode <= M324_AUX_MUL, "m324_gemm: aux_mode %d", a->aux_mode);
    if (n3_mode) {
        M324_REQUIRE(a->aux && a->qkv_qw && a->act == M324_ACT_GELU && !a->residual && !a->gamma && a->row_gin <= 0 && a->batch <= 1,
                     "m324_gemm: M324_AUX_N3 = Linear + GELU + [3, N] contraction: aux (partial sums) and qkv_qw (the [3, N] weight) "
                     "must be given, no residual / gamma / row map / batch");
        M324_REQUIRE(a->in_dtype == M324_BF16 && a->out_dtype == M324_BF16 && a->N % 256 == 0 && a->K % 64 == 0 && a->K >= 128,
                     "m324_gemm: M324_AUX_N3 needs bf16, N %% 256 == 0, K %% 64 == 0, K >= 128 (N=%d K=%d)", a->N, a->K);
        M324_REQUIRE(((uintptr_t)a->qkv_qw % 16) == 0 && (!a->bias || ((uintptr_t)a->bias % 16) == 0), "m324_gemm: M324_AUX_N3 operands misaligned");
    }
    if (qkv_mode) {
        M324_REQUIRE(a->aux_mode != M324_AUX_QKV_HEADS_VT || a->qkv_L % 64 == 0,
                     "m324_gemm: M324_AUX_QKV_HEADS_VT needs qkv_L %% 64 == 0 (L=%d)", a->qkv_L);
        const int parts = (a->qkv_q ? 1 : 0) + (a->qkv_k ? 1 : 0) + (a->qkv_v ? 1 : 0);
        const bool shape_ok = (a->qkv_q && a->qkv_k && a->qkv_v) || (!a->qkv_q && a->qkv_k && a->qkv_v) || (a->qkv_q && !a->qkv_k && !a->qkv_v);
        M324_REQUIRE(shape_ok && a->qkv_H > 0 && a->N == parts * a->qkv_H * 64,
                     "m324_gemm: M324_AUX_QKV_HEADS outputs must be q|k|v, k|v or q with N = parts * H * 64 (N=%d H=%d parts=%d)", a->N,
                     a->qkv_H, parts);
        M324_REQUIRE(a->in_dtype == M324_BF16 && a->out_dtype == M324_BF16 &&
                         a->qkv_L > 0 && a->M % a->qkv_L == 0 && !a->residual && !a->gamma &&
                         a->act == M324_ACT_NONE && a->row_gin <= 0 && a->batch <= 1 && a->M > 64 && vec_ok(a),
                     "m324_gemm: M324_AUX_QKV_HEADS needs a plain bf16 [B*L, 3*H*64] projection with M > 64");
        M324_REQUIRE(a->aux_mode != M324_AUX_QKV_HEADS_VT || a->qkv_v, "m324_gemm: M324_AUX_QKV_HEADS_VT without a V output");
        M324_REQUIRE(((uintptr_t)a->qkv_q % 16) == 0 && ((uintptr_t)a->qkv_k % 16) == 0 && ((uintptr_t)a->qkv_v % 16) == 0 &&
                         (!a->qkv_qw || ((uintptr_t)a->qkv_qw % 16) == 0) && (!a->qkv_kw || ((uintptr_t)a->qkv_kw % 16) == 0),
                     "m324_gemm: misaligned qkv outputs / norm weights");
    } else if (a->aux_mode && !n3_mode) {
        const int osz = a->out_dtype == M324_BF16 ? 2 : 4;
        M324_REQUIRE(a->aux && a->ldaux >= a->N && a->ldaux % 4 == 0 && ((uintptr_t)a->aux % (4 * osz)) == 0 && vec_ok(a) &&
                         a->row_gin <= 0 && a->batch <= 1,
                     "m324_gemm: aux operand needs a vectorisable, un-remapped, un-batched problem with ldaux >= N");
        M324_REQUIRE((a->aux_mode != M324_AUX_STORE_PREACT && a->aux_mode != M324_AUX_STORE_GELU_GRAD) || a->act == M324_ACT_GELU,
                     "m324_gemm: M324_AUX_STORE_PREACT / M324_AUX_STORE_GELU_GRAD only make sense with an activation");
        M324_REQUIRE((a->aux_mode != M324_AUX_MUL_GELU_GRAD && a->aux_mode != M324_AUX_MUL) || a->act == M324_ACT_NONE,
                     "m324_gemm: M324_AUX_MUL_GELU_GRAD / M324_AUX_MUL exclude an activation");
        M324_REQUIRE(!a->residual, "m324_gemm: the aux operand excludes a residual");
    }
    if (a->ln_rowstat || a->ln_stats_out || a->ln_copy_out) {
        M324_REQUIRE(a->in_dtype == M324_BF16 && a->N % 64 == 0 && a->M > 64 && vec_ok(a) && a->batch <= 1 && a->K >= 128,
                     "m324_gemm: the LayerNorm fold needs a bf16, vectorisable, un-batched problem with M > 64, N %% 64 == 0 and "
                     "K >= 128 (M=%d N=%d K=%d)", a->M, a->N, a->K);
        M324_REQUIRE(a->aux_mode != M324_AUX_STORE_PREACT && a->aux_mode != M324_AUX_MUL_GELU_GRAD && a->aux_mode != M324_AUX_STORE_GELU_GRAD &&
                         a->aux_mode != M324_AUX_MUL,
                     "m324_gemm: the LayerNorm fold is an inference feature (no training aux modes)");
        if (a->ln_rowstat) {
            M324_REQUIRE(!a->ln_stats_out && !a->ln_copy_out, "m324_gemm: one GEMM either consumes or produces LayerNorm statistics");
            M324_REQUIRE(!a->residual && !a->gamma && a->row_gin <= 0, "m324_gemm: a folded LayerNorm consumer takes no residual / gamma / row map");
            M324_REQUIRE(a->act == M324_ACT_NONE || a->out_dtype == M324_BF16, "m324_gemm: LayerNorm fold + GELU needs a bf16 output");
        } else {
            M324_REQUIRE(a->ln_stats_out && a->residual && a->act == M324_ACT_NONE,
                         "m324_gemm: a LayerNorm statistics producer is a residual update without activation");
            M324_REQUIRE((a->out_dtype == M324_F32) == (a->ln_copy_out != nullptr),
                         "m324_gemm: ln_copy_out goes with an fp32 output (and only with it)");
        }
        M324_REQUIRE(!a->ln_rowstat || (a->ln_colsum && ((uintptr_t)a->ln_rowstat % 8) == 0 && ((uintptr_t)a->ln_colsum % 16) == 0),
                     "m324_gemm: ln_rowstat needs ln_colsum (16-byte aligned) and an 8-byte aligned row table");
        M324_REQUIRE(!a->ln_rowstat || a->ln_ncb <= 0 || (a->ln_ncb <= 16 && a->ln_ncb % 2 == 0 && a->ln_ncb * 64 == a->K && a->ln_eps >= 0.f &&
                                                           (long)a->ln_ncb * a->M * 8 < (1l << 32)),
                     "m324_gemm: an unmerged row table has K / 64 blocks of 64 columns, an even count <= 16, and less than 4 GiB "
                     "(ln_ncb=%d K=%d M=%d)", a->ln_ncb, a->K, a->M);
        M324_REQUIRE((!a->ln_stats_out && !a->ln_copy_out) || (a->row_gin <= 0 && a->aux_mode == M324_AUX_NONE),
                     "m324_gemm: ln_stats_out / ln_copy_out describe the rows of C: no row remap, no aux mode");
        M324_REQUIRE(!a->ln_stats_out || ((uintptr_t)a->ln_stats_out % 8) == 0, "m324_gemm: ln_stats_out misaligned");
        M324_REQUIRE(!a->ln_copy_out || (a->out_dtype == M324_F32 && a->ln_ldcopy >= a->N && a->ln_ldcopy % 4 == 0 &&
                                         ((uintptr_t)a->ln_copy_out % 8) == 0),
                     "m324_gemm: ln_copy_out is the bf16 twin of an fp32 output (ldcopy >= N, multiple of 4, 8-byte aligned)");
    }
    return M324_OK;
}

extern "C" int m324_gemm(const m324_gemm_args* a, void* stream) {
    const int rc = gemm_validate(a);
    if (rc != M324_OK) return rc;
    hipStream_t s = (hipStream_t)stream;
    if (a->in_dtype == M324_BF16 && a->out_dtype == M324_BF16) return launch<bf16_t, bf16_t>(a, s);
    if (a->in_dtype == M324_BF16 && a->out_dtype == M324_F32) return launch<bf16_t, float>(a, s);
    if (a->in_dtype == M324_F32 && a->out_dtype == M324_F32) return launch<float, float>(a, s);
    M324_FAIL(M324_ERR_UNSUPPORTED, "m324_gemm: unsupported dtype pair in=%d out=%d", a->in_dtype, a->out_dtype);
}

extern "C" int m324_gemm_pair(const m324_gemm_args* a, const m324_gemm_args* b, void* stream) {
    int rc = gemm_validate(a);
    if (rc != M324_OK) return rc;
    rc = gemm_validate(b);
    if (rc != M324_OK) return rc;
    const GemmPlan pa = make_plan(a), pb = make_plan(b);
    if (pa.variant != 13 || pa.actx != 4 || pb.variant != 13 || pb.actx != 4)
        M324_FAIL(M324_ERR_UNSUPPORTED, "m324_gemm_pair: built for two bf16 head-major projections on the 128 x 128 chunk ring");
    auto problem = [](const m324_gemm_args* g, const GemmPlan& p) {
        return Ring2Problem{(const bf16_t*)g->A, g->lda, (const bf16_t*)g->W, g->ldw, g->C, g->ldc, g->M, g->N, g->K, make_epilogue(g),
                            ceil_div(g->N, BN), xcd_mode(g), (int)p.wg};
    };
    const Ring2Problem p0 = problem(a, pa), p1 = problem(b, pb);
    hipLaunchKernelGGL((gemm_ring2_pair_kernel<bf16_t, 4, 0>), dim3(p0.tiles + p1.tiles), dim3(256), 0, (hipStream_t)stream, p0, p1);
    M324_CHECK_LAUNCH("m324_gemm_pair");
    return M324_OK;
}
```

motion324_amd/lib.py:

```python
from __future__ import annotations

import ctypes as C
import os
import threading

HERE = os.path.dirname(os.path.abspath(__file__))
LIB_PATH = os.environ.get("M324_LIB") or os.path.join(HERE, "libm324.so")

F32, BF16, MXFP8 = 0, 1, 2
ACT_NONE, ACT_GELU = 0, 1
ABI_VERSION = 23
ERR_UNSUPPORTED = -3


class M324Error(RuntimeError):
    pass


class GemmArgs(C.Structure):
    _fields_ = [
        ("A", C.c_void_p), ("lda", C.c_long),
        ("W", C.c_void_p), ("ldw", C.c_long),
        ("C", C.c_void_p), ("ldc", C.c_long),
        ("M", C.c_int), ("N", C.c_int), ("K", C.c_int),
        ("in_dtype", C.c_int), ("out_dtype", C.c_int),
        ("bias", C.c_void_p),
        ("act", C.c_int),
        ("gamma", C.c_void_p),
        ("residual", C.c_void_p), ("ldr", C.c_long), ("res_rows", C.c_int),
        ("row_gin", C.c_int), ("row_gout", C.c_int), ("row_off", C.c_int),
        ("batch", C.c_int),
        ("strideA", C.c_long), ("strideW", C.c_long), ("strideC", C.c_long),
        ("aux", C.c_void_p), ("ldaux", C.c_long), ("aux_mode", C.c_int),
        ("qkv_q", C.c_void_p), ("qkv_k", C.c_void_p), ("qkv_v", C.c_void_p),
        ("qkv_qw", C.c_void_p), ("qkv_kw", C.c_void_p),
        ("qkv_eps", C.c_float), ("qkv_qscale", C.c_float), ("qkv_L", C.c_int), ("qkv_H", C.c_int),
        ("ln_rowstat", C.c_void_p), ("ln_colsum", C.c_void_p),
        ("ln_stats_out", C.c_void_p),
        ("ln_copy_out", C.c_void_p), ("ln_ldcopy", C.c_long), ("ln_ncb", C.c_int), ("ln_eps", C.c_float),
    ]


class ColsumItem(C.Structure):
    _fields_ = [("dst", C.c_void_p), ("src", C.c_void_p), ("ld", C.c_long), ("rows", C.c_int), ("cols", C.c_int),
                ("accumulate", C.c_int), ("chain", C.c_int)]


class MirrorItem(C.Structure):
    _fields_ = [("src_off", C.c_long), ("dst_off", C.c_long), ("dstT_off", C.c_long), ("first_tile", C.c_long), ("rows", C.c_int),
                ("cols", C.c_int), ("ldT", C.c_int), ("pad_", C.c_int)]


_P, _L, _I, _F = C.c_void_p, C.c_long, C.c_int, C.c_float

SIGNATURES = {
    "m324_abi_version": [],
    "m324_last_error": [C.c_char_p, _I],
    "m324_device_info": [C.c_char_p, _I],
    "m324_set_tunable": [C.c_char_p, _I],
    "m324_gemm": [C.POINTER(GemmArgs), _P],
    "m324_gemm_plan": [C.POINTER(GemmArgs), C.c_char_p, _I],
    "m324_gemm_pair": [C.POINTER(GemmArgs), C.POINTER(GemmArgs), _P],
    "m324_mx_quant": [_P, _I, _L, _I, _I, _P, _L, _P, _L, _P],
    "m324_layernorm_mx": [_P, _L, _P, _P, _F, _I, _I, _P, _L, _P, _L, _P],
    "m324_gemm_mx": [C.POINTER(GemmArgs), _P, _L, _P, _L, _P, _L, _P],
    "m324_attention_plan": [_I, _I, _I, _I, _I, _I, C.c_char_p, _I],
    "m324_gemm_tn": [_P, _L, _P, _L, _P, _L, _I, _I, _I, _I, _L, _P],
    "m324_n3_finish": [_P, _I, _I, _P, _P, _P],
    "m324_rowstats_finish": [_P, _I, _I, _F, _P, _P],
    "m324_rowstats": [_P, _L, _I, _I, _F, _P, _P, _L, _P],
    "m324_layernorm": [_P, _L, _P, _P, _F, _P, _L, _I, _I, _I, _I, _I, _I, _P],
    "m324_layernorm_in": [_P, _I, _L, _P, _P, _F, _P, _L, _I, _I, _I, _I, _I, _I, _P],
    "m324_layernorm_pair": [_P, _L, _P, _P, _F, _P, _L, _I, _I, _I, _I, _P, _L, _P, _P, _F, _P, _L, _I, _I, _I, _I, _I, _I, _P],
    "m324_qkv_split": [_P, _L, _P, _L, _P, _L, _P, _P, _F, _F, _P, _P, _P, _P, _P, _P, _I, _I, _I, _I, _P],
    "m324_attention": [_P, _L, _P, _P, _P, _L, _I, _I, _I, _I, _F, _I, _P, _I, _P],
    "m324_attention_merge": [_P, _P, _P, _P, _P, _P, _L, _P, _L, _I, _I, _I, _I, _P],
    "m324_patchify": [_P, _I, _I, _I, _I, _I, _P, _I, _I, _P],
    "m324_patchify_u8": [_P, _I, _I, _I, _I, _I, _P, _I, _I, _P],
    "m324_point_encode": [_P, _I, _P, _L, _I, _P],
    "m324_point_concat": [_P, _P, _I, _P, _I, _I, _I, _P],
    "m324_dino_cls_rows": [_P, _P, _P, _I, _I, _I, _P],
    "m324_assemble_tokens": [_P, _P, _P, _F, _P, _P, _P, _P, _P, _F, _P, _I, _I, _I, _I, _I, _F, C.c_ulonglong, _P],
    "m324_linear_n3": [_P, _L, _P, _P, _P, _I, _I, _I, _P],
    "m324_mse": [_P, _P, _L, _F, _P, _P, _P],
    "m324_smooth_trajectories": [_P, _P, _P, _I, _I, _I, _F, _F, _P],
    "m324_smooth_savgol": [_P, _P, _I, _I, _I, _P, _I, _P],
    "m324_smooth_oneeuro": [_P, _P, _I, _I, _I, _F, _F, _F, _P],
    "m324_nearest_point": [_P, _I, _P, _I, _P, _P],
    "m324_transpose": [_P, _L, _P, _L, _I, _I, _I, _I, _P],
    "m324_colsum": [_P, _L, _P, _I, _I, _I, _I, _P, _I, _P],
    "m324_colsum_multi": [C.POINTER(ColsumItem), _I, _P],
    "m324_gelu": [_P, _P, _L, _I, _P],
    "m324_gelu_bwd": [_P, _P, _P, _L, _I, _P],
    "m324_cast": [_P, _L, _I, _P, _L, _I, _I, _I, _P],
    "m324_attention_delta": [_P, _P, _L, _P, _I, _I, _I, _I, _P],
    "m324_attention_bwd": [_P, _L, _P, _P, _P, _P, _P, _P, _P, _P, _I, _I, _I, _I, _F, _I, _P],
    "m324_attention_bwd_mfma": [_P, _P, _L, _L, _P, _P, _P, _P, _P, _P, _P, _P, _P, _P, _I, _I, _I, _I, _F, _P],
    "m324_qkv_split_bwd": [_P, _P, _P, _P, _L, _P, _L, _P, _P, _F, _P, _L, _P, _L, _P, _L, _P, _I, _I, _I, _I, _I, _P],
    "m324_linear_n3_bwd": [_P, _L, _P, _P, _P, _L, _P, _I, _I, _I, _I, _P, _L, _P],
    "m324_mse_bwd": [_P, _P, _P, _F, _P, _L, _P],
    "m324_adamw": [_P, _P, _P, _P, _L, _F, _F, _F, _F, _F, _I, _P, _P],
    "m324_adamw_flat": [_P, _P, _P, _P, _L, _L, _F, _F, _F, _F, _F, _I, _P, _P],
    "m324_weight_mirror": [_P, _P, _P, _P, _I, _L, _P],
    "m324_grad_sumsq": [_P, _L, _I, _P, _P, _I, _P],
    "m324_comm_unique_id": [C.c_char_p, _I],
    "m324_comm_init": [C.POINTER(C.c_void_p), C.c_char_p, _I, _I],
    "m324_comm_allreduce": [_P, _P, _L, _I, _I, _P],
    "m324_comm_allgather": [_P, _P, _P, _L, _I, _P],
    "m324_comm_destroy": [_P],
    "m324_layernorm_bwd": [_P, _L, _P, _F, _P, _L, _I, _P, _L, _I, _P, _I, _I, _I, _I, _I, _I, _P],
    "m324_layernorm_bwd_cast": [_P, _L, _P, _F, _P, _L, _I, _P, _L, _I, _P, _I, _I, _I, _I, _I, _I, _P, _L, _P],
}

_lib = None
_lock = threading.Lock()


def load() -> C.CDLL:
    global _lib
    if _lib is not None:
        return _lib
    with _lock:
        if _lib is not None:
            return _lib
        if not os.path.exists(LIB_PATH):
            raise M324Error(
                f"{LIB_PATH} not found: the HIP extension is not built. Run `python -m motion324_amd.build` "
                "(there is no CPU or PyTorch fallback on this path).")
        lib = C.CDLL(LIB_PATH)
        for name, argtypes in SIGNATURES.items():
            fn = getattr(lib, name)
            fn.argtypes = argtypes
            fn.restype = C.c_int
        if lib.m324_abi_version() != ABI_VERSION:
            raise M324Error(f"libm324 ABI {lib.m324_abi_version()} != binding {ABI_VERSION}; rebuild")
        _lib = lib
    return _lib


def last_error() -> str:
    buf = C.create_string_buffer(512)
    load().m324_last_error(buf, 512)
    return buf.value.decode(errors="replace")


def check(rc: int, what: str) -> None:
    if rc != 0:
        raise M324Error(f"{what} failed ({rc}): {last_error()}")


TUNABLE_DEFAULT = -2 ** 31


def set_tunable(name: str, value: int = TUNABLE_DEFAULT) -> None:
    check(load().m324_set_tunable(name.encode(), int(value)), "m324_set_tunable")


class tunable:

    def __init__(self, name: str, value):
        self.name = name
        self.value = int(str(value).lstrip("vV")) if value is not None else TUNABLE_DEFAULT

    def __enter__(self):
        set_tunable(self.name, self.value)
        return self

    def __exit__(self, *exc):
        set_tunable(self.name)


def device_info():
    buf = C.create_string_buffer(256)
    n = load().m324_device_info(buf, 256)
    check(0 if n >= 0 else n, "m324_device_info")
    return buf.value.decode(), n
```

motion324_amd/ops.py:

```python
from __future__ import annotations

import ctypes as C
from typing import NamedTuple, Optional

import torch

from . import lib as L
from . import switches
from .timing import active as _timing, span

F32, BF16, MXFP8 = L.F32, L.BF16, L.MXFP8
_TORCH_DT = {F32: torch.float32, BF16: torch.bfloat16}


def code_of(dtype: torch.dtype) -> int:
    if dtype == torch.float32:
        return F32
    if dtype == torch.bfloat16:
        return BF16
    raise L.M324Error(f"unsupported dtype {dtype}")


def torch_dtype(code: int) -> torch.dtype:
    return _TORCH_DT[code]
# ... 189 lines not shown
        args.C, args.ldc = None, N
        args.in_dtype, args.out_dtype = BF16, BF16
        args.bias = _vec(bias, N, "bias")
        args.act = act
        args.aux, args.ldaux, args.aux_mode = _p(part), 3, 5
        args.qkv_qw = _p(w3)
        with span("gemm_bf16", 2.0 * M * N * K + 2.0 * M * N * 3, 2.0 * (M * K + N * K) + 4.0 * part.numel(),
                  f"{_gemm_plan(args)} | M={M} N={N} K={K} gelu n3" if _timing() else ""):
            L.check(L.load().m324_gemm(C.byref(args), _stream()), "m324_gemm")
        return part
    args.C, args.ldc = _rows(out, "out")
    _wrote(out)
    args.in_dtype, args.out_dtype = code_of(a.dtype), code_of(out.dtype)
    args.bias = _vec(bias, N, "bias")
    args.act = act
    args.gamma = _vec(gamma, N, "gamma")
    if residual is not None:
        in_place_bf16 = residual.dtype == torch.bfloat16 and out.dtype == torch.bfloat16 and residual.data_ptr() == out.data_ptr()
        if residual.dtype != torch.float32 and not in_place_bf16:
            raise L.M324Error("gemm: residual must be fp32 (or the bf16 output itself, updated in place)")
        args.residual, args.ldr = _rows(residual, "residual")
        args.res_rows = res_rows
    gin, gout, off = row_map
    need = ((M - 1) // gin * gout + (M - 1) % gin + off + 1) if gin > 0 else M
    if out.shape[0] < need or out.shape[1] < N:
        raise L.M324Error(f"gemm: out{tuple(out.shape)} too small for {need} x {N}")
    args.row_gin, args.row_gout, args.row_off = gin, gout, off
    auxes = [(t, mode) for t, mode in ((preact_out, 1), (gelu_grad_of, 2), (gelu_grad_out, 6), (mul_by, 7)) if t is not None]
    if auxes:
        if len(auxes) > 1:
            raise L.M324Error("gemm: preact_out, gelu_grad_of, gelu_grad_out and mul_by are mutually exclusive")
        aux, mode = auxes[0]
        if aux.dtype != out.dtype or aux.shape[0] < M or aux.shape[1] < N:
            raise L.M324Error(f"gemm: aux operand {aux.dtype}{tuple(aux.shape)} does not match out {out.dtype} [{M}, {N}]")
        args.aux, args.ldaux = _rows(aux, "aux")
        args.aux_mode = mode
    esz = a.element_size()
    tag = "" if not _timing() else (
        f"{_gemm_plan(args)} | M={M} N={N} K={K}{' bias' if bias is not None else ''}{' gelu' if act else ''}"
        f"{' gamma' if gamma is not None else ''}{' res' if residual is not None else ''} out={'bf16' if out.element_size() == 2 else 'f32'}"
        f"{' ln-fold' if ln is not None else ''}{' ln-stats' if stats_out is not None else ''}")
    nbytes = esz * (M * K + N * K) + out.element_size() * M * N
    if residual is not None:
        nbytes += residual.element_size() * N * (res_rows if 0 < res_rows < M else M)
    if copy_out is not None:
        nbytes += 2 * M * N
    with span(f"gemm_{'bf16' if esz == 2 else 'f32'}", 2.0 * M * N * K, nbytes, tag):
        L.check(L.load().m324_gemm(C.byref(args), _stream()), "m324_gemm")
    return out


class MX(NamedTuple):
    q: torch.Tensor
    s: torch.Tensor

    @property
    def shape(self):
        return self.q.shape


def mx_empty(rows: int, K: int, device) -> MX:
    return MX(torch.empty((rows, K), dtype=torch.uint8, device=device),
              torch.empty((rows, (K // 32 + 3) // 4 * 4), dtype=torch.uint8, device=device)[:, :K // 32])


def _mx_rows(t: MX, rows: int, K: int, name: str):
    if (not isinstance(t, MX) or t.q.dtype != torch.uint8 or t.s.dtype != torch.uint8 or t.q.shape[0] < rows or t.q.shape[1] < K
            or t.s.shape[0] < rows or t.s.shape[1] < K // 32):
        raise L.M324Error(f"{name}: expected an MX operand of at least [{rows}, {K}]")
    (pq, lq), (ps, ls) = _rows(t.q, name + ".q"), _rows(t.s, name + ".s")
    return pq, lq, ps, ls


def mx_quant(x: torch.Tensor, out: Optional[MX] = None) -> MX:
    rows, K = x.shape
    out = mx_empty(rows, K, x.device) if out is None else out
    px, ldx = _rows(x, "x")
    pq, lq, ps, ls = _mx_rows(out, rows, K, "out")
    with span("hbm_pass", 0.0, float(rows) * K * (x.element_size() + 1), f"mx_quant_kernel | rows={rows} K={K}" if _timing() else ""):
        L.check(L.load().m324_mx_quant(px, code_of(x.dtype), ldx, rows, K, pq, lq, ps, ls, _stream()), "m324_mx_quant")
    _wrote(out.q, out.s)
    return out


def layernorm_mx(x: torch.Tensor, w: torch.Tensor, b: Optional[torch.Tensor], eps: float, out: Optional[MX] = None) -> MX:
    if x.dtype != torch.float32:
        raise L.M324Error("layernorm_mx: x must be fp32")
    rows, Cdim = x.shape
    out = mx_empty(rows, Cdim, x.device) if out is None else out
    px, ldx = _rows(x, "x")
    pq, lq, ps, ls = _mx_rows(out, rows, Cdim, "out")
    with span("hbm_pass", 0.0, float(rows) * Cdim * 5, f"layernorm_mx_kernel | rows={rows} C={Cdim}" if _timing() else ""):
        L.check(L.load().m324_layernorm_mx(px, ldx, _vec(w, Cdim, "w"), _vec(b, Cdim, "b"), eps, rows, Cdim, pq, lq, ps, ls, _stream()),
                "m324_layernorm_mx")
    _wrote(out.q, out.s)
    return out


def gemm_mx(a: MX, w: MX, out, *, bias=None, act: int = L.ACT_NONE, gamma=None, residual: Optional[torch.Tensor] = None,
            qkv_heads: Optional[tuple] = None):
    M, K = a.q.shape[0], a.q.shape[1]
    N = w.q.shape[0]
    pa, la, psa, lsa = _mx_rows(a, M, K, "a")
    pw, lw, psw, lsw = _mx_rows(w, N, K, "w")
    args = L.GemmArgs()
    args.A, args.lda, args.W, args.ldw = pa, la, pw, lw
    args.M, args.N, args.K = M, N, K
    args.in_dtype, args.batch = MXFP8, 1
    args.bias = _vec(bias, N, "bias")
    args.act = act
    args.gamma = _vec(gamma, N, "gamma")
    pcs, lcs = None, 0
    first = out
    if qkv_heads is not None:
        Qo, Ko, Vo, qw, kw, eps, q_scale, Lh, Hh = qkv_heads[:9]
        Bh = M // Lh
        vt = Vo is not None and tuple(Vo.shape) == (Bh, Hh, 64, Lh) and Lh != 64
        for t in (Qo, Ko, Vo):
            if t is None:
                continue
            want = (Bh, Hh, 64, Lh) if (vt and t is Vo) else (Bh, Hh, Lh, 64)
            if t.dtype != torch.bfloat16 or not t.is_contiguous() or tuple(t.shape) != want:
                raise L.M324Error(f"gemm_mx: qkv_heads output {t.dtype}{tuple(t.shape)} (want bf16 {want})")
        args.C, args.ldc, args.out_dtype = None, N, BF16
        args.aux_mode = 4 if vt else 3
        args.qkv_q, args.qkv_k, args.qkv_v = _p(Qo), _p(Ko), _p(Vo)
        args.qkv_qw, args.qkv_kw = _vec(qw, 64, "q_w"), _vec(kw, 64, "k_w")
        args.qkv_eps, args.qkv_qscale, args.qkv_L, args.qkv_H = eps, q_scale, Lh, Hh
        first = next(t for t in (Qo, Ko, Vo) if t is not None)
        _wrote(Qo, Ko, Vo)
    elif isinstance(out, MX):
        args.C, args.ldc, pcs, lcs = _mx_rows(out, M, N, "out")
        args.out_dtype = MXFP8
        _wrote(out.q, out.s)
    else:
        args.C, args.ldc = _rows(out, "out")
        args.out_dtype = code_of(out.dtype)
        if out.shape[0] < M or out.shape[1] < N:
            raise L.M324Error(f"gemm_mx: out{tuple(out.shape)} too small for {M} x {N}")
        if residual is not None:
            args.residual, args.ldr = _rows(residual, "residual")
        _wrote(out)
    with span("gemm_mx", 2.0 * M * N * K, float(M * K + N * K + M * N * 2),
              f"gemm_mx_kernel | M={M} N={N} K={K}" if _timing() else ""):
        L.check(L.load().m324_gemm_mx(C.byref(args), psa, lsa, psw, lsw, pcs, lcs, _stream()), "m324_gemm_mx")
    return first


def gemm_pair(deferred: list) -> None:
    if len(deferred) != 2:
        raise L.M324Error("gemm_pair: exactly two deferred projections")
    (a0, f0, b0, t0, _), (a1, f1, b1, t1, _) = deferred
    lib = L.load()
    with span("gemm_bf16", f0 + f1, b0 + b1, f"gemm_ring2_pair_kernel<unsigned short, 4, 0> | {t0} + {t1}" if _timing() else "") as sp:
        rc = lib.m324_gemm_pair(C.byref(a0), C.byref(a1), _stream())
        if rc == L.ERR_UNSUPPORTED:
            sp.cancel()
    if rc == L.ERR_UNSUPPORTED:
        for args, fl, by, tag, _ in deferred:
            with span("gemm_bf16", fl, by, f"{_gemm_plan(args)} | {tag}" if _timing() else ""):
                L.check(lib.m324_gemm(C.byref(args), _stream()), "m324_gemm")
    else:
        L.check(rc, "m324_gemm_pair")
    deferred.clear()


def layernorm_pair(x0, w0, b0, eps0, out0, x1, w1, b1, eps1, out1, row_map1=(0, 0, 0)) -> None:
    Cdim = x0.shape[1]
    if (x0.dtype != torch.float32 or x1.dtype != torch.float32 or x1.shape[1] != Cdim or out0.shape[1] != Cdim or out1.shape[1] != Cdim
            or out0.dtype != out1.dtype or out0.shape[0] > x0.shape[0]):
        raise L.M324Error("layernorm_pair: two fp32 inputs of one width, outputs of one dtype")
    gin, gout, off = row_map1
    rows1 = out1.shape[0]
    need = ((rows1 - 1) // gin * gout + (rows1 - 1) % gin + off + 1) if gin > 0 else rows1
    if x1.shape[0] < need:
        raise L.M324Error("layernorm_pair: shape mismatch")
    (p0, l0), (q0, m0), (p1, l1), (q1, m1) = _rows(x0, "x0"), _rows(out0, "out0"), _rows(x1, "x1"), _rows(out1, "out1")
    tag = f"layernorm_pair_kernel | rows={out0.shape[0]}+{rows1} C={Cdim}" if _timing() else ""
    with span("hbm_pass", 0.0, float(out0.shape[0] + rows1) * Cdim * (4 + out0.element_size()), tag):
        L.check(L.load().m324_layernorm_pair(p0, l0, _vec(w0, Cdim, "w0"), _vec(b0, Cdim, "b0"), eps0, q0, m0, out0.shape[0], 0, 0, 0,
                                             p1, l1, _vec(w1, Cdim, "w1"), _vec(b1, Cdim, "b1"), eps1, q1, m1, rows1, gin, gout, off,
                                             Cdim, code_of(out0.dtype), _stream()), "m324_layernorm_pair")
    _wrote(out0, out1)


def rowstats_finish(part: torch.Tensor, eps: float, rowstat: torch.Tensor) -> torch.Tensor:
    ncb, M, two = part.shape
    if (two != 2 or part.dtype != torch.float32 or not part.is_contiguous() or rowstat.dtype != torch.float32
            or not rowstat.is_contiguous() or rowstat.numel() != 2 * M):
        raise L.M324Error("rowstats_finish: part [ncb, M, 2] and rowstat [M, 2] must be contiguous fp32")
    with span("hbm_pass", 0.0, 8.0 * (ncb + 1) * M, f"rowstats_finish_kernel | rows={M} blocks={ncb}" if _timing() else ""):
        L.check(L.load().m324_rowstats_finish(_p(part), ncb, M, eps, _p(rowstat), _stream()), "m324_rowstats_finish")
    return rowstat


def rowstats(x: torch.Tensor, eps: float, rowstat: torch.Tensor, copy: Optional[torch.Tensor] = None) -> torch.Tensor:
    px, ldx = _rows(x, "x")
    rows, Cdim = x.shape
    if x.dtype != torch.float32 or rowstat.dtype != torch.float32 or not rowstat.is_contiguous() or rowstat.numel() != 2 * rows:
        raise L.M324Error("rowstats: x fp32 [rows, C], rowstat contiguous fp32 [rows, 2]")
    pc, ldc = (None, 0)
    if copy is not None:
        if copy.dtype != torch.bfloat16 or copy.shape[0] < rows or copy.shape[1] != Cdim:
            raise L.M324Error("rowstats: copy must be bf16 [rows, C]")
        pc, ldc = _rows(copy, "copy")
    with span("hbm_pass", 0.0, rows * Cdim * (4.0 + (2.0 if copy is not None else 0.0)), f"rowstats_kernel | rows={rows} C={Cdim}" if _timing() else ""):
        L.check(L.load().m324_rowstats(px, ldx, rows, Cdim, eps, _p(rowstat), pc, ldc, _stream()), "m324_rowstats")
    return rowstat


def layernorm(x: torch.Tensor, w: torch.Tensor, b: Optional[torch.Tensor], eps: float, out: torch.Tensor,
              rows: Optional[int] = None, row_map=(0, 0, 0)) -> torch.Tensor:
    if x.dtype != torch.float32 and not (x.dtype == torch.bfloat16 and out.dtype == torch.bfloat16):
        raise L.M324Error("layernorm: x must be fp32 (or bf16 with a bf16 output)")
    px, ldx = _rows(x, "x")
    py, ldy = _rows(out, "out")
    Cdim = x.shape[1]
    rows = out.shape[0] if rows is None else rows
    gin, gout, off = row_map
    need = ((rows - 1) // gin * gout + (rows - 1) % gin + off + 1) if gin > 0 else rows
    if x.shape[0] < need or out.shape[0] < rows or out.shape[1] != Cdim:
        raise L.M324Error("layernorm: shape mismatch")
    tag = (f"layernorm_kernel<{'unsigned short' if out.element_size() == 2 else 'float'}, {'unsigned short' if x.element_size() == 2 else 'float'}>"
           f" | rows={rows} C={Cdim}") if _timing() else ""
    with span("hbm_pass", 0.0, float(rows) * Cdim * (x.element_size() + out.element_size()), tag):
        if x.dtype == torch.bfloat16:
            L.check(L.load().m324_layernorm_in(px, BF16, ldx, _vec(w, Cdim, "w"), _vec(b, Cdim, "b"), eps, py, ldy, code_of(out.dtype),
                                               rows, Cdim, gin, gout, off, _stream()), "m324_layernorm_in")
        else:
            L.check(L.load().m324_layernorm(px, ldx, _vec(w, Cdim, "w"), _vec(b, Cdim, "b"), eps, py, ldy, code_of(out.dtype),
                                            rows, Cdim, gin, gout, off, _stream()), "m324_layernorm")
    return out


LOG2E = 1.4426950408889634
Q_PRESCALE = (64 ** -0.5) * LOG2E


def qkv_split(q_src, k_src, v_src, q_w, k_w, eps: float, B: int, Lq: int, H: int, dtype: torch.dtype, *,
              q_scale: float = 1.0, train: bool = False):
    dev = next(t for t in (q_src, k_src, v_src) if t is not None).device
    Lp = (Lq + 63) // 64 * 64

    def row():
        return torch.empty((B, H, Lq, 64), dtype=dtype, device=dev)

    def tr():
        return torch.empty((B, H, 64, Lp), dtype=dtype, device=dev)
    Q = row() if q_src is not None else None
    K = row() if k_src is not None else None
    V = row() if (v_src is not None and train) else None
    Qt = tr() if (q_src is not None and train) else None
    Kt = tr() if (k_src is not None and train) else None
    Vt = tr() if v_src is not None else None

    def src(t, name):
        if t is None:
            return None, 0
        if t.dtype != dtype or t.shape[0] < B * Lq:
            raise L.M324Error(f"qkv_split: {name} {t.dtype}{tuple(t.shape)}")
        return _rows(t, name)
    pq, ldq = src(q_src, "q_src")
    pk, ldk = src(k_src, "k_src")
    pv, ldv = src(v_src, "v_src")
    L.check(L.load().m324_qkv_split(pq, ldq, pk, ldk, pv, ldv, _vec(q_w, 64, "q_w"), _vec(k_w, 64, "k_w"), eps, q_scale,
                                    _p(Q), _p(K), _p(V), _p(Qt), _p(Kt), _p(Vt), B, Lq, H, code_of(dtype), _stream()),
            "m324_qkv_split")
    if train:
        return {"Q": Q, "K": K, "V": V, "Qt": Qt, "Kt": Kt, "Vt": Vt}
    return Q, K, Vt


def attention(Q: torch.Tensor, K: torch.Tensor, Vt: torch.Tensor, out: torch.Tensor, *, shared_q: bool = False,
              scale: Optional[float] = None, prescaled: bool = False, lse: Optional[torch.Tensor] = None,
              v_rowmajor: bool = False, bounded: bool = False) -> torch.Tensor:
    B, H, Lk, D = K.shape
    Lq = Q.shape[2]
    vshape = (B, H, Lk, 64) if v_rowmajor else (B, H, 64, (Lk + 63) // 64 * 64)
    if D != 64 or Q.shape[3] != 64 or Q.shape[1] != H or tuple(Vt.shape) != vshape:
        raise L.M324Error(f"attention: Q{tuple(Q.shape)} K{tuple(K.shape)} V{tuple(Vt.shape)} (want {vshape})")
    if not (Q.is_contiguous() and K.is_contiguous() and Vt.is_contiguous()):
        raise L.M324Error("attention: operands must be contiguous")
    if Q.dtype != K.dtype or K.dtype != Vt.dtype or out.dtype != Q.dtype:
        raise L.M324Error("attention: dtype mismatch")
    if not shared_q and Q.shape[0] != B:
        raise L.M324Error("attention: batch mismatch")
    po, ldo = _rows(out, "out")
    if out.shape[0] < B * Lq or out.shape[1] < H * 64:
        raise L.M324Error("attention: out too small")
    qbs = 0 if shared_q else H * Lq * 64
    scale = 64 ** -0.5 if scale is None else scale
    esz = Q.element_size()
    flags = int(prescaled) | (2 if v_rowmajor else 0) | (4 if bounded else 0)
    with span(f"attention_{'bf16' if esz == 2 else 'f32'}", 4.0 * B * H * Lq * Lk * 64,
              esz * 64.0 * H * ((1 if shared_q else B) * Lq + 2 * B * Lk + B * Lq),
              f"{_attn_plan(B, H, Lq, Lk, flags | (256 if shared_q else 0), code_of(Q.dtype))} | B={B} H={H} Lq={Lq} Lk={Lk}"
              if _timing() else ""):
        L.check(L.load().m324_attention(_p(Q), qbs, _p(K), _p(Vt), po, ldo, B, H, Lq, Lk, scale, flags, _p(lse), code_of(Q.dtype), _stream()),
                "m324_attention")
    return out


def attention_merge(parts, out: torch.Tensor, B: int, H: int, Lq: int) -> torch.Tensor:
    if not 2 <= len(parts) <= 3:
        raise L.M324Error("attention_merge: two or three (output, lse) parts")
    O0 = parts[0][0]
    p0, ldp = _rows(O0, "O0")
    ptrs = []
    for O, lse in parts:
        po, ld = _rows(O, "part")
        if (O.dtype != out.dtype or ld != ldp or O.shape[0] < B * Lq or O.shape[1] < H * 64 or lse.dtype != torch.float32
                or not lse.is_contiguous() or lse.numel() != B * H * Lq):
            raise L.M324Error(f"attention_merge: part {O.dtype}{tuple(O.shape)} / lse {lse.dtype}{tuple(lse.shape)}")
        ptrs += [po, _p(lse)]
    if len(parts) == 2:
        ptrs += [None, None]
    po, ldo = _rows(out, "out")
    if out.shape[0] < B * Lq or out.shape[1] < H * 64:
        raise L.M324Error("attention_merge: out too small")
    esz = out.element_size()
    with span("hbm_pass", 0.0, float(B * Lq) * H * 64 * esz * (len(parts) + 1),
              f"attention_merge_kernel | rows={B * Lq} parts={len(parts)}" if _timing() else ""):
        L.check(L.load().m324_attention_merge(*ptrs, ldp, po, ldo, B, H, Lq, code_of(out.dtype), _stream()), "m324_attention_merge")
    _wrote(out)
    return out


def patchify(video: torch.Tensor, size: int, patch: int, Kp: int, dtype: torch.dtype) -> torch.Tensor:
    if video.dtype not in (torch.float32, torch.uint8) or not video.is_contiguous() or video.dim() != 4 or video.shape[3] != 3:
        raise L.M324Error(f"patchify: video {video.dtype}{tuple(video.shape)}")
    Fr, Hin, Win, _ = video.shape
    g = size // patch
    out = torch.empty((Fr * g * g, Kp), dtype=dtype, device=video.device)
    fn, name = (L.load().m324_patchify_u8, "m324_patchify_u8") if video.dtype == torch.uint8 else (L.load().m324_patchify, "m324_patchify")
    L.check(fn(_p(video), Fr, Hin, Win, size, patch, _p(out), Kp, code_of(dtype), _stream()), name)
    _wrote(out)
    return out


def point_encode(xyz: torch.Tensor, dtype: torch.dtype) -> torch.Tensor:
    xyz = xyz.reshape(-1, 3)
    if xyz.dtype != torch.float32 or not xyz.is_contiguous():
        raise L.M324Error("point_encode: xyz must be contiguous fp32")
    out = torch.empty((xyz.shape[0], 64), dtype=dtype, device=xyz.device)
    L.check(L.load().m324_point_encode(_p(xyz), xyz.shape[0], _p(out), 64, code_of(dtype), _stream()), "m324_point_encode")
    return out


def point_concat(normal: torch.Tensor, rgb: torch.Tensor, feat: torch.Tensor, Cdim: int) -> torch.Tensor:
    normal, rgb = normal.reshape(-1, 3), rgb.reshape(-1, 3)
    for t in (normal, rgb):
        if t.dtype != torch.float32 or not t.is_contiguous():
            raise L.M324Error("point_concat: normal/rgb must be contiguous fp32")
    P, Kp = feat.shape
    if not feat.is_contiguous() or normal.shape[0] != P or rgb.shape[0] != P:
        raise L.M324Error("point_concat: shape mismatch")
    L.check(L.load().m324_point_concat(_p(normal), _p(rgb), P, _p(feat), Cdim, Kp, code_of(feat.dtype), _stream()),
            "m324_point_concat")
    return feat


def dino_cls_rows(cls: torch.Tensor, pos0: torch.Tensor, x: torch.Tensor, Fr: int, rows_per_frame: int) -> None:
    Cdim = x.shape[1]
    L.check(L.load().m324_dino_cls_rows(_vec(cls, Cdim, "cls"), _vec(pos0, Cdim, "pos0"), _p(x), Fr, rows_per_frame, Cdim,
                                        _stream()), "m324_dino_cls_rows")


def assemble_tokens(dino_x, dino_w, dino_b, eps_dino, pos, sp0, spr, mesh, ln_w, eps_in, B, T, K, P,
                    drop_p: float = 0.0, drop_seed: int = 0) -> torch.Tensor:
    Cdim = dino_x.shape[1]
    for name, t, n in (("dino_x", dino_x, B * T * (P + 1) * Cdim), ("pos", pos, T * P * Cdim), ("sp0", sp0, 4 * Cdim),
                       ("spr", spr, 4 * Cdim), ("mesh", mesh, B * K * Cdim)):
        if t.dtype != torch.float32 or not t.is_contiguous() or t.numel() != n:
            raise L.M324Error(f"assemble_tokens: {name} {t.dtype}{tuple(t.shape)} (want {n} fp32)")
    out = torch.empty((B * T * (4 + K + P), Cdim), dtype=torch.float32, device=dino_x.device)
    L.check(L.load().m324_assemble_tokens(_p(dino_x), _vec(dino_w, Cdim, "dino_w"), _vec(dino_b, Cdim, "dino_b"), eps_dino,
                                          _p(pos), _p(sp0), _p(spr), _p(mesh), _vec(ln_w, Cdim, "ln_w") if ln_w is not None else None, eps_in, _p(out),
                                          B, T, K, P, Cdim, float(drop_p), int(drop_seed) & 0xFFFFFFFFFFFFFFFF, _stream()),
            "m324_assemble_tokens")
    return out


def linear_n3(a: torch.Tensor, w: torch.Tensor, bias: torch.Tensor, out: torch.Tensor) -> torch.Tensor:
    M, K = a.shape
    pa, lda = _rows(a, "a")
    if w.dtype != torch.float32 or not w.is_contiguous() or tuple(w.shape) != (3, K):
        raise L.M324Error("linear_n3: w must be contiguous fp32 [3,K]")
    if out.dtype != torch.float32 or not out.is_contiguous() or out.numel() != M * 3:
        raise L.M324Error("linear_n3: out must be contiguous fp32 [M,3]")
    L.check(L.load().m324_linear_n3(pa, lda, _p(w), _vec(bias, 3, "bias"), _p(out), M, K, code_of(a.dtype), _stream()),
            "m324_linear_n3")
    return out


def n3_finish(part: torch.Tensor, bias: torch.Tensor, out: torch.Tensor) -> torch.Tensor:
    ncb, M, three = part.shape
    if three != 3 or part.dtype != torch.float32 or not part.is_contiguous() or out.dtype != torch.float32 \
            or not out.is_contiguous() or out.numel() != M * 3:
        raise L.M324Error("n3_finish: part [ncb, M, 3] and out [M, 3] must be contiguous fp32")
    L.check(L.load().m324_n3_finish(_p(part), ncb, M, _vec(bias, 3, "bias"), _p(out), _stream()), "m324_n3_finish")
    return out


def mse(pred: torch.Tensor, target: torch.Tensor, weight: float) -> torch.Tensor:
    if pred.shape != target.shape:
        raise L.M324Error(f"mse: shape mismatch {tuple(pred.shape)} vs {tuple(target.shape)}")
    pred = pred.contiguous().float()
    target = target.contiguous().float()
    partial = torch.empty(1024, dtype=torch.float32, device=pred.device)
    out = torch.empty((), dtype=torch.float32, device=pred.device)
    L.check(L.load().m324_mse(_p(pred), _p(target), pred.numel(), weight, _p(partial), _p(out), _stream()), "m324_mse")
    return out


def smooth_trajectories(trajs: torch.Tensor, threshold: float, sigma: float) -> torch.Tensor:
    if trajs.dim() != 4 or trajs.shape[3] != 3:
        raise L.M324Error(f"smooth_trajectories: expected [B,T,N,3], got {tuple(trajs.shape)}")
    x = trajs.detach().to(torch.float32).contiguous()
    B, T, N, _ = x.shape
    tmp, out = torch.empty_like(x), torch.empty_like(x)
    L.check(L.load().m324_smooth_trajectories(_p(x), _p(tmp), _p(out), B, T, N, threshold, sigma, _stream()),
            "m324_smooth_trajectories")
    return out


def smooth_savgol(trajs: torch.Tensor, coef: torch.Tensor) -> torch.Tensor:
    x = trajs.detach().to(torch.float32).contiguous()
    B, T, N, _ = x.shape
    if coef.dtype != torch.float64 or not coef.is_cuda or not coef.is_contiguous():
        raise L.M324Error("smooth_savgol: coef must be a contiguous fp64 HIP tensor")
    out = torch.empty_like(x)
    L.check(L.load().m324_smooth_savgol(_p(x), _p(out), B, T, N, _p(coef), coef.numel(), _stream()), "m324_smooth_savgol")
    return out


def smooth_oneeuro(trajs: torch.Tensor, mincutoff: float, beta: float, dcutoff: float = 1.0) -> torch.Tensor:
    x = trajs.detach().to(torch.float32).contiguous()
    B, T, N, _ = x.shape
    out = torch.empty_like(x)
    L.check(L.load().m324_smooth_oneeuro(_p(x), _p(out), B, T, N, mincutoff, beta, dcutoff, _stream()), "m324_smooth_oneeuro")
    return out


def nearest_point(query: torch.Tensor, ref: torch.Tensor) -> torch.Tensor:
    q = query.detach().to(torch.float32).contiguous()
    r = ref.detach().to(torch.float32).contiguous()
    if q.dim() != 2 or q.shape[1] != 3 or r.dim() != 2 or r.shape[1] != 3:
        raise L.M324Error(f"nearest_point: expected [n,3] point sets, got {tuple(q.shape)} / {tuple(r.shape)}")
    idx = torch.empty((q.shape[0],), dtype=torch.int32, device=q.device)
    L.check(L.load().m324_nearest_point(_p(q), q.shape[0], _p(r), r.shape[0], _p(idx), _stream()), "m324_nearest_point")
    return idx.long()

# ... 262 lines not shown
```

motion324_amd/switches.py:

```python
from __future__ import annotations

import os
from typing import Dict, Tuple

HOST: Dict[str, Tuple[str, str, str]] = {
    "M324_AUTO_GRAPH": ("1", "Pcd_motion.AUTO_GRAPH", "inference forward(): hipGraph replay from the third call with the same shapes on"),
    "M324_FUSE_HEAD": ("1", "Pcd_motion.FUSE_HEAD_N3", "bf16 inference: head Linear + GELU + Linear(C -> 3) in one GEMM epilogue (M324_AUX_N3)"),
    "M324_BF16_DECODER": ("1", "Pcd_motion.BF16_DECODER_STREAM", "bf16 inference: the decoder's two-addition residual stream in bf16 (0: fp32 like the trunk)"),
    "M324_HOIST_Q": ("1", "Pcd_motion.HOIST_DECODER_Q", "graph capture: decoder point features + q projection on the shape-encoder branch"),
    "M324_DECODE_ROWS": (str(1 << 17), "Pcd_motion.DECODE_ROWS", "max (frames x points) rows per decoder pass"),
    "M324_OVERLAP": ("1", "Pcd_motion.OVERLAP_SHAPE_ENCODER", "inference: shape encoder on a second HIP stream under the image encoder"),
    "M324_KV_OVERLAP": ("0", "Pcd_motion.KV_OVERLAP", "frame-parallel (one sample), opt-in until it has run on a multi-GPU RCCL node: 1 = every global block attends to the rank's own keys while the k|v all-gather is in flight, then to the gathered remote keys, and merges the partial softmaxes by their log-sum-exps (0: one attention after the gather)"),
    "M324_KV_REHEARSE": ("0", "Pcd_motion.KV_REHEARSE", "one rank with forced collectives (bench.py M324_BENCH_COLLECT=1): W > 1 runs every global block's overlapped form as rank 0 of W would (own keys = the first 1 / W of the frames), to price the split attention + merge on one GPU"),
    "M324_FOLD_LN": ("2", "transformer.FOLD_LN", "LayerNorm fold: 0 off, 1 bf16 streams only (the decoder), 2 every stream (trunk, DINO too)"),
    "M324_FOLD_MERGE": ("1", "transformer.FOLD_MERGE", "LayerNorm fold: the consumer GEMM merges the producer's per-block row statistics itself (0: m324_rowstats_finish launch between them)"),
    "M324_PAIR_PROJ": ("1", "transformer.PAIR_PROJ", "bf16 inference, decoder: norm_q + norm_kv in one launch and the q + k|v projections in one launch when the q projection runs inside the block (0: four launches)"),
    "M324_ATTN_BOUNDED": ("1", "transformer.ATTN_BOUNDED", "bf16 inference, long sequences: softmax without a reference maximum when the q / k RMSNorm weights bound every score (M324_ATTN_SCORES_BOUNDED)"),
    "M324_FUSE_QKV": ("1", "transformer.FUSE_QKV", "bf16 inference: q|k|v projection epilogue writes head-major Q / K / V (RMSNorm, pre-scale)"),
    "M324_FUSE_QKV_VT": ("1", "transformer.FUSE_QKV_VT", "the same for long sequences: the epilogue writes the transposed, key-permuted V"),
    "M324_TRAIN_STORE": ("1", "training.TRAIN_STORE", "training: the forward keeps block internals while they fit half of the free HBM (0: always recompute, the reference's checkpoint policy)"),
    "M324_WEIGHT_MIRROR": ("1", "optim.WEIGHT_MIRROR", "training: FusedAdamW keeps bf16 row-major and transposed copies of every Linear weight in two flat buffers, rewritten by one m324_weight_mirror launch after each update (0: Prepared casts / m324_transpose per weight and step)"),
    "M324_DEFER_COLSUM": ("1", "ops.DEFER_COLSUM", "training: the sums of the weight gradients' split-K partials and of the norm-weight partials wait in a queue and leave in one m324_colsum_multi launch per block (0: one m324_colsum launch each, at once)"),
    "M324_MXFP8": ("0", "Pcd_motion.MXFP8_DEFAULT", "1: a model whose config names no model.inference_precision uses \"mxfp8\" -- block-scaled e4m3 operands for the GEMM roles of transformer.MX_ROLES (the trunk and DINOv2 q|k|v projections) in a bf16 inference forward (DESIGN section 4)"),
    "M324_PRECISION": ("", "prepared.compute_dtype()", "force bf16 / fp32 (default: follow torch.autocast like the reference)"),
    "M324_LIB": ("", "lib.LIB_PATH", "path of an alternative libm324.so (lab builds)"),
    "M324_RCCL_LIB": ("", "csrc/comm.hip", "m324_comm_*: path of the RCCL library to bind (default: the copy already loaded, else librccl.so)"),
}
LIBRARY: Dict[str, Tuple[str, str]] = {
    "M324_GEMM": ("0", "force a GEMM schedule (v2 | v5 | v9 | v10 | v11 | v12 | v13 | v15); 0 = chooser"),
    "M324_GEMM_TN": ("0", "128: force the 128 x 128 weight-gradient kernel"),
    "M324_XCD": ("3", "tile order: bit 0 XCD-contiguous ranges (NN GEMMs; the weight-gradient GEMM's (slice, tile) items since round 6), bit 1 4 x 2 group order for wide weights, bit 2 force it"),
    "M324_ATTN_NW": ("0", "attention forward: waves per workgroup (4 | 8); 0 = by sequence length"),
    "M324_ATTN_BWD_NW": ("0", "attention backward: waves per workgroup -- 0 = four (the default since round 6), 8 = eight for both kernels, 84 = dQ eight + dK/dV four, 48 = the reverse, 2 = dQ with 64 queries per wave (A/B)"),
    "M324_ATTN_EXP": ("0", "attention: 8 = one workgroup per frame in the shared-query one-tile form instead of the frame-pair kernel (the parity test's other arm)"),
    "M324_ATTN_PWG": ("1", "attention forward, long sequences: 1 = one wave per SIMD with the hand-placed stream (attention_pwg.hip), 0 = the eight-wave kernel"),
    "M324_QKV_RING": ("1", "128 x 128 chunk ring (v13) instead of the two-stage v2: bit 0 for the fused q|k|v projection (head-major epilogue), bit 1 for plain bf16 outputs (A/B)"),
    "M324_LN_ROWS": ("2", "LayerNorm: rows per wave (2 = two interleaved rows, 1 = one row: A/B)"),
    "M324_NT_MB": ("128", "GEMM: bf16 outputs (no residual) larger than this many MiB are stored nontemporal"),
    "M324_HP": ("6", "schedule v15 (one wave per SIMD, hand-placed stream, the previous tile's epilogue between the MFMAs of the current one) for K = 768 GEMMs with bf16 output and at least two 256 x 128 tiles per CU: bit 1 the bias-only / plain epilogues (the training step's projections), bit 2 the GELU epilogues from 4096 tiles on (the decoder's fc1, the 256-frame clip's), bit 0 every GELU epilogue; folded consumers it takes get the merged statistics table from the host (transformer.hp_consumer); 0: never"),
    "M324_GEMM_PERSIST": ("1", "256 x 256 chunk-ring GEMM (v10): 1 = one persistent workgroup per CU, next tile's first chunks under the epilogue; 0 = one workgroup per tile"),
}


def get(name: str) -> str:
    return os.environ.get(name, (HOST.get(name) or LIBRARY[name])[0])


def flag(name: str) -> bool:
    return get(name) != "0"


def non_default() -> Dict[str, str]:
    out = {}
    for name, spec in list(HOST.items()) + list(LIBRARY.items()):
        v = os.environ.get(name)
        if v is not None and v.lstrip("vV") != spec[0] and v != spec[0]:
            out[name] = v
    return out


def table() -> str:
    rows = ["| switch | default | meaning |", "|---|---|---|"]
    rows += [f"| `{n}` | {d or '(unset)'} | {doc} (`{const}`) |" for n, (d, const, doc) in HOST.items()]
    rows += [f"| `{n}` | {d} | libm324: {doc} |" for n, (d, doc) in LIBRARY.items()]
    return "\n".join(rows)
```

motion324_amd/transformer.py:

```python
from __future__ import annotations

import os

from typing import Optional

import torch
import torch.nn as nn

from . import ops, switches
from .lib import ACT_GELU
from .prepared import Prepared

LN_EPS = 1e-5
RMS_EPS = 1e-5


def init_weights(module, std=0.02):
    if isinstance(module, (nn.Linear, nn.Embedding)):
        torch.nn.init.normal_(module.weight, mean=0.0, std=std)
        if isinstance(module, nn.Linear) and module.bias is not None:
            torch.nn.init.zeros_(module.bias)


class RMSNorm(nn.Module):
    def __init__(self, dim: int, eps: float = RMS_EPS):
        super().__init__()
        self.eps = eps
        self.weight = nn.Parameter(torch.ones(dim))


class MLP(nn.Module):
    def __init__(self, dim, mlp_ratio=4, bias=False, dropout=0.0, activation=nn.GELU, mlp_dim=None):
        super().__init__()
        if bias or dropout != 0.0 or activation is not nn.GELU:
            raise NotImplementedError("the HIP path implements the configuration the reference instantiates "
                                      "(no bias, no dropout, exact GELU)")
        hidden = mlp_dim if mlp_dim is not None else int(dim * mlp_ratio)
        self.mlp = nn.Sequential(nn.Linear(dim, hidden, bias=False), nn.GELU(), nn.Linear(hidden, dim, bias=False),
                                 nn.Dropout(0.0))


class _AttnBase(nn.Module):
    def __init__(self, dim, head_dim, use_qk_norm):
        super().__init__()
        if head_dim != 64:
            raise NotImplementedError("libm324 attention kernels are specialised for head_dim 64 (config d_head)")
        assert dim % head_dim == 0, f"Token dimension {dim} should be divisible by head dimension {head_dim}"
        self.dim, self.head_dim, self.num_heads, self.use_qk_norm = dim, head_dim, dim // head_dim, use_qk_norm

    def _register_qk_norm(self):
        if self.use_qk_norm:
            self.q_norm = RMSNorm(self.head_dim)
            self.k_norm = RMSNorm(self.head_dim)

    def _qk_w(self, P: Prepared):
        if not self.use_qk_norm:
            return None, None
        return P.vec(self.q_norm.weight), P.vec(self.k_norm.weight)

    def scores_bounded(self, P: Prepared) -> bool:
        if not (ATTN_BOUNDED and not _FUSE_OFF and self.use_qk_norm and P.dtype == torch.bfloat16):
            return False
        t = P.derived("qk_score_bound", (self.q_norm.weight, self.k_norm.weight), lambda: torch.tensor(
            [64.0 * ops.Q_PRESCALE * float(self.q_norm.weight.detach().abs().max()) * float(self.k_norm.weight.detach().abs().max())]))
        return float(t[0]) <= 48.0


class QK_Norm_SelfAttention(_AttnBase):
    def __init__(self, dim, head_dim, qkv_bias=False, fc_bias=True, attn_dropout=0.0, fc_dropout=0.0, use_qk_norm=True):
        super().__init__(dim, head_dim, use_qk_norm)
        if attn_dropout != 0.0 or fc_dropout != 0.0:
            raise NotImplementedError("attention / projection dropout is 0 everywhere in the reference model")
        self.to_qkv = nn.Linear(dim, 3 * dim, bias=qkv_bias)
        self.fc = nn.Linear(dim, dim, bias=fc_bias)
        self._register_qk_norm()


class QK_Norm_CrossAttention(_AttnBase):
    def __init__(self, dim, head_dim, kv_dim=None, qkv_bias=False, fc_bias=True, attn_dropout=0.0, fc_dropout=0.0,
                 use_qk_norm=True):
        super().__init__(dim, head_dim, use_qk_norm)
        if attn_dropout != 0.0 or fc_dropout != 0.0:
            raise NotImplementedError("attention / projection dropout is 0 everywhere in the reference model")
        kv_dim = dim if kv_dim is None else kv_dim
        self.kv_dim = kv_dim
        self.to_q = nn.Linear(dim, dim, bias=qkv_bias)
        self.to_k = nn.Linear(kv_dim, dim, bias=qkv_bias)
        self.to_v = nn.Linear(kv_dim, dim, bias=qkv_bias)
        self.fc = nn.Linear(dim, dim, bias=fc_bias)
        self._register_qk_norm()


FOLD_LN = int(switches.get("M324_FOLD_LN"))
PAIR_PROJ = switches.flag("M324_PAIR_PROJ")
FOLD_MERGE = switches.flag("M324_FOLD_MERGE")
ATTN_BOUNDED = switches.flag("M324_ATTN_BOUNDED")


class LNFold:

    def __init__(self, x: torch.Tensor):
        rows, C = x.shape
        self.rows, self.C = rows, C
        self.xb = x if x.dtype == torch.bfloat16 else torch.empty((rows, C), dtype=torch.bfloat16, device=x.device)
        self.part = torch.empty((C // 64, rows, 2), dtype=torch.float32, device=x.device)
        self.stat = torch.empty((rows, 2), dtype=torch.float32, device=x.device)
        self.pending = False
        self.own_copy = x.dtype != torch.bfloat16

    @staticmethod
    def usable(P: Prepared, rows: int, C: int, bf16_stream: bool = False) -> bool:
        return (FOLD_LN >= (1 if bf16_stream else 2) and not _FUSE_OFF and P.dtype == torch.bfloat16 and rows > 64
                and C % 64 == 0 and C >= 128 and not torch.is_grad_enabled())

    def from_stream(self, x: torch.Tensor, eps: float) -> "LNFold":
        ops.rowstats(x, eps, self.stat, self.xb if self.own_copy else None)
        self.pending = False
        return self

    def producer(self) -> dict:
        self.pending = True
        return dict(stats_out=self.part, copy_out=self.xb if self.own_copy else None)

    def ln(self, eps: float, colsum: torch.Tensor, merged: bool = False) -> tuple:
        if self.pending and FOLD_MERGE and not merged and self.C <= 1024 and self.C % 128 == 0:
            return (self.part, colsum, eps)
        return (self.ready(eps), colsum)

    def ready(self, eps: float) -> torch.Tensor:
        if self.pending:
            ops.rowstats_finish(self.part, eps, self.stat)
            self.pending = False
        return self.stat


def hp_consumer(rows: int, n_out: int, k: int) -> bool:
    if k != 768 or n_out % 128 != 0 or rows < 1:
        return False
    return ops.gemm_schedule(rows, n_out, k, act=ACT_GELU, fold_merged=True) == 15


def _mlp_residual(P: Prepared, norm2: nn.LayerNorm, mlp: MLP, x: torch.Tensor, fold: Optional[LNFold] = None,
                  feed_next: bool = True, mx: bool = False) -> torch.Tensor:
    rows, C = x.shape
    fc1, fc2 = mlp.mlp[0], mlp.mlp[2]
    if mx and fold is None and x.dtype == torch.float32:
        a2 = ops.layernorm_mx(x, P.vec(norm2.weight), P.vec(norm2.bias), norm2.eps)
        hq = ops.mx_empty(rows, fc1.out_features, x.device)
        ops.gemm_mx(a2, P.mx(fc1.weight), hq, bias=P.vec(fc1.bias), act=ACT_GELU)
        ops.gemm_mx(hq, P.mx(fc2.weight), x, bias=P.vec(fc2.bias), residual=x)
        return x
    h1 = torch.empty((rows, fc1.out_features), dtype=P.dtype, device=x.device)
    if fold is not None:
        w1, cs1, b1 = P.folded(norm2.weight, norm2.bias, fc1.weight, fc1.bias)
        ops.gemm(fold.xb, w1, h1, bias=b1, act=ACT_GELU, ln=fold.ln(norm2.eps, cs1, merged=hp_consumer(rows, fc1.out_features, C)))
        ops.gemm(h1, P.mat(fc2.weight), x, bias=P.vec(fc2.bias), residual=x, **(fold.producer() if feed_next else {}))
        return x
    h = torch.empty((rows, C), dtype=P.dtype, device=x.device)
    ops.layernorm(x, P.vec(norm2.weight), P.vec(norm2.bias), norm2.eps, h)
    ops.gemm(h, P.mat(fc1.weight), h1, bias=P.vec(fc1.bias), act=ACT_GELU)
    ops.gemm(h1, P.mat(fc2.weight), x, bias=P.vec(fc2.bias), residual=x)
    return x


FUSE_QKV = switches.flag("M324_FUSE_QKV")
FUSE_QKV_VT = switches.flag("M324_FUSE_QKV_VT")


_FUSE_OFF = 0


class fusion_disabled:

    def __enter__(self):
        global _FUSE_OFF, _MX_ROLES_ON
        _FUSE_OFF += 1
        self._mx, _MX_ROLES_ON = _MX_ROLES_ON, frozenset()

    def __exit__(self, *exc):
        global _FUSE_OFF, _MX_ROLES_ON
        _FUSE_OFF -= 1
        _MX_ROLES_ON = self._mx


def fusion_off() -> bool:
    return _FUSE_OFF > 0


MX_ROLES_BUILT = frozenset({"trunk.qkv", "trunk.mlp", "dino.qkv", "dino.mlp"})
MX_ROLES = frozenset({"trunk.qkv", "dino.qkv"})
_MX_ROLES_ON: frozenset = frozenset()


class mx_scope:

    def __init__(self, roles):
        self.roles = frozenset(roles)

    def __enter__(self):
        global _MX_ROLES_ON
        self._saved, _MX_ROLES_ON = _MX_ROLES_ON, self.roles
        return self

    def __exit__(self, *exc):
        global _MX_ROLES_ON
        _MX_ROLES_ON = self._saved


def mx_role(P: Prepared, role: str) -> bool:
    return role in _MX_ROLES_ON and not _FUSE_OFF and P.dtype == torch.bfloat16 and not torch.is_grad_enabled()


class fusion_allowed:

    def __enter__(self):
        global _FUSE_OFF
        self._saved, _FUSE_OFF = _FUSE_OFF, 0

    def __exit__(self, *exc):
        global _FUSE_OFF
        _FUSE_OFF = self._saved


def fuse_qkv(P: Prepared, rows: int, L: int) -> bool:
    return (FUSE_QKV and not _FUSE_OFF and P.dtype == torch.bfloat16 and rows > 64 and (L < 2048 or (FUSE_QKV_VT and L % 128 == 0))
            and not torch.is_grad_enabled())


def fuse_proj(P: Prepared, rows: int) -> bool:
    return FUSE_QKV and not _FUSE_OFF and P.dtype == torch.bfloat16 and rows > 64 and not torch.is_grad_enabled()


class QK_Norm_TransformerBlock(nn.Module):

    def __init__(self, dim, head_dim, ln_bias=False, attn_qkv_bias=False, attn_dropout=0.0, attn_fc_bias=False,
                 attn_fc_dropout=0.0, mlp_ratio=4, mlp_bias=False, mlp_dropout=0.0, use_qk_norm=True):
        super().__init__()
        self.norm1 = nn.LayerNorm(dim, bias=ln_bias)
        self.attn = QK_Norm_SelfAttention(dim, head_dim, qkv_bias=attn_qkv_bias, fc_bias=attn_fc_bias,
                                          attn_dropout=attn_dropout, fc_dropout=attn_fc_dropout, use_qk_norm=use_qk_norm)
        self.norm2 = nn.LayerNorm(dim, bias=ln_bias)
        self.mlp = MLP(dim, mlp_ratio=mlp_ratio, bias=mlp_bias, dropout=mlp_dropout)

    def run(self, P: Prepared, x: torch.Tensor, B: int, L: int, kv_gather=None, fold: Optional[LNFold] = None,
            feed_next: bool = True) -> torch.Tensor:
        rows, C = x.shape
        assert rows == B * L
        a = self.attn
        h = torch.empty((rows, C), dtype=P.dtype, device=x.device)
        qw, kw = a._qk_w(P)
        mx_qkv = kv_gather is None and mx_role(P, "trunk.qkv")
        mlp_mx = fold is None and mx_role(P, "trunk.mlp")
        proj = ops.gemm_mx if mx_qkv else ops.gemm
        if mx_qkv:
            src = ops.layernorm_mx(x, P.vec(self.norm1.weight), P.vec(self.norm1.bias), self.norm1.eps)
            w, bias = P.mx(a.to_qkv.weight), P.vec(a.to_qkv.bias)
            lnk = lambda lo, hi: {}
            feed_next = False
        elif fold is not None:
            w, cs, bias = P.folded(self.norm1.weight, self.norm1.bias, a.to_qkv.weight, a.to_qkv.bias)
            src, lnk = fold.xb, (lambda lo, hi: dict(ln=fold.ln(self.norm1.eps, cs[lo:hi])))
        else:
            ops.layernorm(x, P.vec(self.norm1.weight), P.vec(self.norm1.bias), self.norm1.eps, h)
            w, bias = P.mat(a.to_qkv.weight), P.vec(a.to_qkv.bias)
            src, lnk = h, (lambda lo, hi: {})
        out_kw = fold.producer if fold is not None else dict
        if fuse_qkv(P, rows, L) and kv_gather is None:
            long_seq = L >= 2048
            Q, K = (torch.empty((B, a.num_heads, L, 64), dtype=P.dtype, device=x.device) for _ in range(2))
            V = torch.empty((B, a.num_heads, 64, L) if long_seq else (B, a.num_heads, L, 64), dtype=P.dtype, device=x.device)
            proj(src, w, None, bias=bias, qkv_heads=(Q, K, V, qw, kw, RMS_EPS, ops.Q_PRESCALE, L, a.num_heads),
                 **lnk(0, 3 * C))
            ops.attention(Q, K, V, h, prescaled=True, v_rowmajor=not long_seq, bounded=long_seq and a.scores_bounded(P))
            ops.gemm(h, P.mat(a.fc.weight), x, bias=P.vec(a.fc.bias), residual=x, **out_kw())
            return _mlp_residual(P, self.norm2, self.mlp, x, fold, feed_next, mx=mlp_mx)
        if kv_gather is None:
            qkv = torch.empty((rows, 3 * C), dtype=P.dtype, device=x.device)
            proj(src, w, qkv, bias=bias, **lnk(0, 3 * C))
            Q, K, Vt = ops.qkv_split(qkv[:, :C], qkv[:, C:2 * C], qkv[:, 2 * C:], qw, kw, RMS_EPS, B, L, a.num_heads,
                                     P.dtype, q_scale=ops.Q_PRESCALE)
        else:
            kv = torch.empty((rows, 2 * C), dtype=P.dtype, device=x.device)
            ops.gemm(src, w[C:], kv, bias=None if bias is None else bias[C:], **lnk(C, 3 * C))
            kv_gather.start(kv)
            q = torch.empty((rows, C), dtype=P.dtype, device=x.device)
            ops.gemm(src, w[:C], q, bias=None if bias is None else bias[:C], **lnk(0, C))
            Q, _, _ = ops.qkv_split(q, None, None, qw, None, RMS_EPS, B, L, a.num_heads, P.dtype, q_scale=ops.Q_PRESCALE)
            if getattr(kv_gather, "overlap", False):
                H = a.num_heads
                bounded = a.scores_bounded(P)

                def part(kv_rows, Lk):
                    _, Kp, Vp = ops.qkv_split(None, kv_rows[:, :C], kv_rows[:, C:], None, kw, RMS_EPS, B, Lk, H, P.dtype)
                    o = torch.empty((rows, C), dtype=P.dtype, device=x.device)
                    lse = torch.empty((B, H, L), dtype=torch.float32, device=x.device)
                    ops.attention(Q, Kp, Vp, o, prescaled=True, bounded=bounded, lse=lse)
                    return o, lse
                lo, hi = kv_gather.local_rows()
                own = kv[lo:hi] if getattr(kv_gather, "rehearse", 0) else kv
                parts = [part(own, hi - lo)]
                kv_full, L_full = kv_gather.finish()
                for r0, r1 in ((0, lo), (hi, L_full)):
                    if r1 > r0:
                        parts.append(part(kv_full[r0:r1], r1 - r0))
                ops.attention_merge(parts, h, B, H, L)
                ops.gemm(h, P.mat(a.fc.weight), x, bias=P.vec(a.fc.bias), residual=x, **out_kw())
                return _mlp_residual(P, self.norm2, self.mlp, x, fold, feed_next)
            kv_full, L_full = kv_gather.finish()
            _, K, Vt = ops.qkv_split(None, kv_full[:, :C], kv_full[:, C:], None, kw, RMS_EPS, B, L_full, a.num_heads,
                                     P.dtype)
        ops.attention(Q, K, Vt, h, prescaled=True, bounded=a.scores_bounded(P))
        ops.gemm(h, P.mat(a.fc.weight), x, bias=P.vec(a.fc.bias), residual=x, **out_kw())
        return _mlp_residual(P, self.norm2, self.mlp, x, fold, feed_next, mx=mlp_mx)

    def forward(self, x: torch.Tensor) -> torch.Tensor:
        B, L, C = x.shape
        P = Prepared.for_module(self, x.device)
        y = x.detach().float().reshape(B * L, C).clone()
        return self.run(P, y, B, L).reshape(B, L, C)


class QK_Norm_CrossAttentionBlock(nn.Module):

    def __init__(self, dim, head_dim, kv_dim=None, ln_bias=False, attn_qkv_bias=False, attn_dropout=0.0,
                 attn_fc_bias=False, attn_fc_dropout=0.0, mlp_ratio=4, mlp_bias=False, mlp_dropout=0.0, use_qk_norm=True):
        super().__init__()
        self.norm_q = nn.LayerNorm(dim, bias=ln_bias)
        self.norm_kv = nn.LayerNorm(kv_dim if kv_dim is not None else dim, bias=ln_bias)
        self.attn = QK_Norm_CrossAttention(dim, head_dim, kv_dim=kv_dim, qkv_bias=attn_qkv_bias, fc_bias=attn_fc_bias,
                                           attn_dropout=attn_dropout, fc_dropout=attn_fc_dropout, use_qk_norm=use_qk_norm)
        self.norm2 = nn.LayerNorm(dim, bias=ln_bias)
        self.mlp = MLP(dim, mlp_ratio=mlp_ratio, bias=mlp_bias, dropout=mlp_dropout)

    def project_q(self, P: Prepared, query: torch.Tensor, B: int, Lq: int) -> torch.Tensor:
        a = self.attn
        qn = torch.empty(query.shape, dtype=P.dtype, device=query.device)
        ops.layernorm(query, P.vec(self.norm_q.weight), P.vec(self.norm_q.bias), self.norm_q.eps, qn)
        qw, _ = a._qk_w(P)
        if fuse_proj(P, B * Lq):
            Q = torch.empty((B, a.num_heads, Lq, 64), dtype=P.dtype, device=query.device)
            ops.gemm(qn, P.mat(a.to_q.weight), None, bias=P.vec(a.to_q.bias),
                     qkv_heads=(Q, None, None, qw, None, RMS_EPS, ops.Q_PRESCALE, Lq, a.num_heads))
            return Q
        q = torch.empty(query.shape, dtype=P.dtype, device=query.device)
        ops.gemm(qn, P.mat(a.to_q.weight), q, bias=P.vec(a.to_q.bias))
        Q, _, _ = ops.qkv_split(q, None, None, qw, None, RMS_EPS, B, Lq, a.num_heads, P.dtype, q_scale=ops.Q_PRESCALE)
        return Q

    def project_kv(self, P: Prepared, kv: torch.Tensor, B: int, Lk: int, row_map=(0, 0, 0)):
        a = self.attn
        C = kv.shape[1]
        kn = torch.empty((B * Lk, C), dtype=P.dtype, device=kv.device)
        ops.layernorm(kv, P.vec(self.norm_kv.weight), P.vec(self.norm_kv.bias), self.norm_kv.eps, kn, row_map=row_map)
        w_kv, b_kv = P.cat_rows((a.to_k.weight, a.to_v.weight)), P.cat_vecs((a.to_k.bias, a.to_v.bias))
        _, kw = a._qk_w(P)
        if fuse_proj(P, B * Lk) and Lk % 64 == 0:
            K = torch.empty((B, a.num_heads, Lk, 64), dtype=P.dtype, device=kv.device)
            Vt = torch.empty((B, a.num_heads, 64, Lk), dtype=P.dtype, device=kv.device)
            ops.gemm(kn, w_kv, None, bias=b_kv, qkv_heads=(None, K, Vt, None, kw, RMS_EPS, 1.0, Lk, a.num_heads, True))
            return K, Vt
        kvp = torch.empty((B * Lk, 2 * a.dim), dtype=P.dtype, device=kv.device)
        ops.gemm(kn, w_kv, kvp, bias=b_kv)
        _, K, Vt = ops.qkv_split(None, kvp[:, :a.dim], kvp[:, a.dim:], None, kw, RMS_EPS, B, Lk, a.num_heads, P.dtype)
        return K, Vt

    def project_q_kv(self, P: Prepared, query: torch.Tensor, Lq: int, kv: torch.Tensor, Bk: int, Lk: int, row_map=(0, 0, 0)):
        a = self.attn
        if not (PAIR_PROJ and fuse_proj(P, Lq) and fuse_proj(P, Bk * Lk) and Lk % 64 == 0 and query.shape[1] == kv.shape[1]
                and query.dtype == torch.float32 and kv.dtype == torch.float32):
            Q = self.project_q(P, query, 1, Lq)
            K, Vt = self.project_kv(P, kv, Bk, Lk, row_map=row_map)
            return Q, K, Vt
        dev = query.device
        qn = torch.empty(query.shape, dtype=P.dtype, device=dev)
        kn = torch.empty((Bk * Lk, kv.shape[1]), dtype=P.dtype, device=dev)
        ops.layernorm_pair(query, P.vec(self.norm_q.weight), P.vec(self.norm_q.bias), self.norm_q.eps, qn,
                           kv, P.vec(self.norm_kv.weight), P.vec(self.norm_kv.bias), self.norm_kv.eps, kn, row_map1=row_map)
        qw, kw = a._qk_w(P)
        Q = torch.empty((1, a.num_heads, Lq, 64), dtype=P.dtype, device=dev)
        K = torch.empty((Bk, a.num_heads, Lk, 64), dtype=P.dtype, device=dev)
        Vt = torch.empty((Bk, a.num_heads, 64, Lk), dtype=P.dtype, device=dev)
        w_kv, b_kv = P.cat_rows((a.to_k.weight, a.to_v.weight)), P.cat_vecs((a.to_k.bias, a.to_v.bias))
        pair: list = []
        ops.gemm(qn, P.mat(a.to_q.weight), None, bias=P.vec(a.to_q.bias),
                 qkv_heads=(Q, None, None, qw, None, RMS_EPS, ops.Q_PRESCALE, Lq, a.num_heads), defer=pair)
        ops.gemm(kn, w_kv, None, bias=b_kv, qkv_heads=(None, K, Vt, None, kw, RMS_EPS, 1.0, Lk, a.num_heads, True), defer=pair)
        ops.gemm_pair(pair)
        return Q, K, Vt

    def attend(self, P: Prepared, Q, K, Vt, residual: torch.Tensor, res_rows: int, shared_q: bool,
               bf16_stream: bool = False, want_fold: bool = False):
        a = self.attn
        B, Lq = K.shape[0], Q.shape[2]
        o = torch.empty((B * Lq, a.dim), dtype=P.dtype, device=Q.device)
        ops.attention(Q, K, Vt, o, shared_q=shared_q, prescaled=True)
        xdt = torch.bfloat16 if (bf16_stream and P.dtype == torch.bfloat16 and not torch.is_grad_enabled()) else torch.float32
        x = torch.empty((B * Lq, a.dim), dtype=xdt, device=Q.device)
        fold = LNFold(x) if LNFold.usable(P, B * Lq, a.dim, bf16_stream=xdt == torch.bfloat16) else None
        ops.gemm(o, P.mat(a.fc.weight), x, bias=P.vec(a.fc.bias), residual=residual, res_rows=res_rows,
                 **(fold.producer() if fold is not None else {}))
        _mlp_residual(P, self.norm2, self.mlp, x, fold, feed_next=want_fold)
        return (x, fold) if want_fold else x

    def run(self, P: Prepared, query: torch.Tensor, kv: torch.Tensor, B: int, Lq: int, Lk: int) -> torch.Tensor:
        Q = self.project_q(P, query, B, Lq)
        K, Vt = self.project_kv(P, kv, B, Lk)
        return self.attend(P, Q, K, Vt, query, 0, shared_q=False)

    def forward(self, query, key, value=None):
        if value is not None and value is not key:
            raise NotImplementedError("the HIP path fuses the k/v projections of one tensor (as both reference call sites do)")
        B, Lq, C = query.shape
        Lk = key.shape[1]
        P = Prepared.for_module(self, query.device)
        out = self.run(P, query.detach().float().reshape(B * Lq, C).contiguous(),
                       key.detach().float().reshape(B * Lk, -1).contiguous(), B, Lq, Lk)
        return out.reshape(B, Lq, C)
```

Measured before the change: 3525 frames/s.

## Run the trunk's last per-frame block only on latent rows the decoder reads

In the last local transformer block, keys and values are still projected for every token, but queries, attention output, the output projection and the MLP run only on the latent rows (plus wave-alignment padding) that the decoder consumes. This adds a gather kernel that copies the folded LayerNorm streams and statistics for those rows, a windowed attention kernel variant that writes only the chosen query rows, and an LN-folded variant of the paired projection GEMM. The decoder then reads the compact latent rows directly. The aim is to avoid the query, output-projection and MLP work on the 4 + point tokens that are discarded, at the cost of extra launches and a more specialised path with many eligibility checks.

```diff
diff --git a/include/m324.h b/include/m324.h
--- a/include/m324.h
+++ b/include/m324.h
@@ -51,6 +51,9 @@
 
 int m324_rowstats_finish(const float* part, int ncb, int M, float eps, float* rowstat, void* stream);
 int m324_rowstats(const float* x, long ldx, int rows, int C, float eps, float* rowstat, void* copy, long ldcopy, void* stream);
+int m324_fold_gather(const float* x, long ldx, const void* xb, long ldxb, const float* part, long part_rows, float* x_out,
+                     long ldx_out, void* xb_out, long ldxb_out, float* part_out, long part_out_rows, int G, int gin, int gout,
+                     int off, int x_skip, int x_rows, int C, void* stream);
 
 int m324_n3_finish(const float* part, int ncb, int M, const float* bias3, float* out, void* stream);
 
@@ -76,6 +79,8 @@
 int m324_attention(const void* Q, long q_bstride, const void* K, const void* Vt, void* O, long ldo,
                    int B, int H, int Lq, int Lk, float scale, int q_prescaled, float* lse, int dtype, void* stream);
 int m324_attention_plan(int B, int H, int Lq, int Lk, int flags, int dtype, char* buf, int n);
+int m324_attention_rows(const void* Q, const void* K, const void* V, void* O, long ldo, int B, int H, int Lq, int Lk, int o_lo,
+                        int o_n, void* stream);
 
 int m324_attention_merge(const void* O0, const float* lse0, const void* O1, const float* lse1, const void* O2, const float* lse2,
                          long ldp, void* O, long ldo, int B, int H, int Lq, int dtype, void* stream);
diff --git a/motion324_amd/Pcd_motion.py b/motion324_amd/Pcd_motion.py
--- a/motion324_amd/Pcd_motion.py
+++ b/motion324_amd/Pcd_motion.py
@@ -711,23 +711,32 @@
             if "trunk.qkv" not in mx.roles:
                 fold.from_stream(tok, self.global_transformer_blocks[0].norm1.eps)
         n_pairs = len(self.global_transformer_blocks)
+        lat_rows = None
         for i, (gblk, lblk) in enumerate(zip(self.global_transformer_blocks, self.local_transformer_blocks)):
             with mx:
                 gblk.run(P, tok, B, T * Lt, kv_gather=kv_gather, fold=fold)
-                lblk.run(P, tok, B * T, Lt, fold=fold, feed_next=i + 1 < n_pairs)
+                if i + 1 == n_pairs and cap is None and lblk.rows_usable(P, B * T, Lt, (K, 4), fold):
+                    lat_rows = lblk.run_rows(P, tok, B * T, Lt, (K, 4), fold)
+                else:
+                    lblk.run(P, tok, B * T, Lt, fold=fold, feed_next=i + 1 < n_pairs)
             if cap is not None and "trunk_block0" not in cap:
                 cap["trunk_block0"] = tok.clone()
         if cap is not None:
             cap["trunk_out"] = tok.clone()
 
         latent = None
-        if keep_latent:
+        if keep_latent and lat_rows is not None:
+            latent = lat_rows.view(B, T, K, C)
+        elif keep_latent:
             latent = torch.empty((B * T, K * C), dtype=torch.float32, device=dev)
             ops.cast(tok.view(B * T, Lt * C)[:, 4 * C:(4 + K) * C], torch.float32, out=latent)
             latent = latent.view(B, T, K, C)
         if encode_only:
             return edict(input_data=sample, latent=latent)
-        out = self._decode(P, sample, tok, (K, Lt, 4), B, T, hoisted, cap)
+        if lat_rows is not None:
+            out = self._decode(P, sample, lat_rows, (0, 0, 0), B, T, hoisted, cap)
+        else:
+            out = self._decode(P, sample, tok, (K, Lt, 4), B, T, hoisted, cap)
 
         if shard is not None and parallel.collectives_on(shard[1]):
             rank, world, group = shard[:3]
diff --git a/motion324_amd/csrc/attention.hip b/motion324_amd/csrc/attention.hip
--- a/motion324_amd/csrc/attention.hip
+++ b/motion324_amd/csrc/attention.hip
@@ -47,11 +47,12 @@
 typedef __attribute__((ext_vector_type(8))) short a_s16x8_t;
 typedef __attribute__((address_space(3))) a_s16x4_t a_lds_s16x4_t;
 
-template <bool PRESCALED, int NQ, int NWV, bool VROW = false, int NST = 3>
-__global__ __launch_bounds__(NWV * 64, NWV == 8 ? (VROW ? 2 : 4) : ((NST == 1 || NST == 2) ? 4 : 1)) void attn_bf16_kernel(const bf16_t* __restrict__ Q, long q_bstride,
+template <bool PRESCALED, int NQ, int NWV, bool VROW, int NST, bool WIN>
+__device__ __forceinline__ void attn_bf16_body(const bf16_t* __restrict__ Q, long q_bstride,
                                                         const bf16_t* __restrict__ K, const bf16_t* __restrict__ Vt,
                                                         bf16_t* __restrict__ O, long ldo, int H, int Lq, int Lk,
-                                                        int Lkp, float scale_log2e, float* __restrict__ lse, int nqt) {
+                                                        int Lkp, float scale_log2e, float* __restrict__ lse, int nqt,
+                                                        int o_lo, int o_n) {
     __shared__ __attribute__((aligned(1024))) unsigned char smem[NST * ASTAGE + (NST == 1 ? NWV * 4096 : 0)];
     const int tid = threadIdx.x, lane = tid & 63;
     const int wave = __builtin_amdgcn_readfirstlane(tid >> 6);
@@ -292,14 +293,28 @@
                 *reinterpret_cast<uint4*>(scr + l31 * 128 + ((chunk ^ (l31 & 7)) << 4)) = make_uint4(a[0], a[1], c[0], c[1]);
             }
         const int r8 = lane >> 3, c8 = lane & 7;
-        bf16_t* obase = O + ((long)b * Lq + q0 + n * QW) * ldo + h * 64 + c8 * 8;
+        bf16_t* obase = O + (WIN ? (long)b * o_n + q0 + n * QW - o_lo : (long)b * Lq + q0 + n * QW) * ldo + h * 64 + c8 * 8;
 #pragma unroll
         for (int p = 0; p < 4; ++p) {
             const int r = p * 8 + r8;
             const uint4 v = *reinterpret_cast<const uint4*>(scr + r * 128 + ((c8 ^ (r & 7)) << 4));
-            if (q0 + n * QW + r < Lq) *reinterpret_cast<uint4*>(obase + (long)r * ldo) = v;
-        }
-    }
+            if (WIN ? (unsigned)(q0 + n * QW + r - o_lo) < (unsigned)o_n : q0 + n * QW + r < Lq) *reinterpret_cast<uint4*>(obase + (long)r * ldo) = v;
+        }
+    }
+}
+
+template <bool PRESCALED, int NQ, int NWV, bool VROW = false, int NST = 3>
+__global__ __launch_bounds__(NWV * 64, NWV == 8 ? (VROW ? 2 : 4) : ((NST == 1 || NST == 2) ? 4 : 1)) void attn_bf16_kernel(const bf16_t* __restrict__ Q, long q_bstride,
+                                                        const bf16_t* __restrict__ K, const bf16_t* __restrict__ Vt,
+                                                        bf16_t* __restrict__ O, long ldo, int H, int Lq, int Lk,
+                                                        int Lkp, float scale_log2e, float* __restrict__ lse, int nqt) {
+    attn_bf16_body<PRESCALED, NQ, NWV, VROW, NST, false>(Q, q_bstride, K, Vt, O, ldo, H, Lq, Lk, Lkp, scale_log2e, lse, nqt, 0, 0);
+}
+
+__global__ __launch_bounds__(256, 4) void attn_bf16_rows_kernel(const bf16_t* __restrict__ Q, const bf16_t* __restrict__ K,
+                                                                const bf16_t* __restrict__ V, bf16_t* __restrict__ O, long ldo, int H, int Lq,
+                                                                int Lk, int nqt, int o_lo, int o_n) {
+    attn_bf16_body<true, 1, 4, true, 2, true>(Q, (long)H * Lq * 64, K, V, O, ldo, H, Lq, Lk, (Lk + 63) / 64 * 64, 1.0f, nullptr, nqt, o_lo, o_n);
 }
 
 template <int FB, bool NT>
@@ -1019,6 +1034,22 @@
     return M324_OK;
 }
 
+extern "C" int m324_attention_rows(const void* Q, const void* K, const void* V, void* O, long ldo, int B, int H, int Lq, int Lk,
+                                   int o_lo, int o_n, void* stream) {
+    M324_REQUIRE(Q && K && V && O, "m324_attention_rows: null pointer");
+    M324_REQUIRE(B > 0 && H > 0 && Lq > 0 && Lk > 0 && H <= 65535 && B <= 65535, "m324_attention_rows: bad sizes B=%d H=%d Lq=%d Lk=%d", B, H, Lq, Lk);
+    M324_REQUIRE(o_lo >= 0 && o_n > 0 && (long)o_lo + o_n <= Lq, "m324_attention_rows: window [%d, %d + %d) outside the %d query rows", o_lo,
+                 o_lo, o_n, Lq);
+    M324_REQUIRE(ldo >= (long)H * 64 && (ldo * 2) % 8 == 0, "m324_attention_rows: ldo too small or misaligned");
+    const AttnPlan p = attn_plan(B, H, Lq, Lk, M324_ATTN_Q_PRESCALED | M324_ATTN_V_ROWMAJOR, M324_BF16);
+    if (p.family != ATTN_BF16 || p.nw != 4 || p.nst != 2)
+        M324_FAIL(M324_ERR_UNSUPPORTED, "m324_attention_rows: built for the per-frame kernel attn_bf16_kernel<true, 1, 4, true, 2> (Lq=%d Lk=%d)", Lq, Lk);
+    hipLaunchKernelGGL(attn_bf16_rows_kernel, p.grid, dim3(p.threads), 0, (hipStream_t)stream, (const bf16_t*)Q, (const bf16_t*)K,
+                       (const bf16_t*)V, (bf16_t*)O, ldo, H, Lq, Lk, p.nqt, o_lo, o_n);
+    M324_CHECK_LAUNCH("m324_attention_rows");
+    return M324_OK;
+}
+
 extern "C" int m324_attention_plan(int B, int H, int Lq, int Lk, int flags, int dtype, char* buf, int n) {
     M324_REQUIRE(buf && n > 0 && B > 0 && H > 0 && Lq > 0 && Lk > 0, "m324_attention_plan: bad arguments");
     const AttnPlan p = attn_plan(B, H, Lq, Lk, flags, dtype);
diff --git a/motion324_amd/csrc/elementwise.hip b/motion324_amd/csrc/elementwise.hip
--- a/motion324_amd/csrc/elementwise.hip
+++ b/motion324_amd/csrc/elementwise.hip
@@ -174,6 +174,27 @@
     if (lane == 0) rowstat[row] = make_float2(rstd, -rstd * mean);
     if (copy) {
         LN_FOR(i, c) store4<bf16_t>(copy + row * ldcopy + c, v[i].x, v[i].y, v[i].z, v[i].w);
+    }
+}
+
+__global__ __launch_bounds__(256) void fold_gather_kernel(const float* __restrict__ x, long ldx, const bf16_t* __restrict__ xb, long ldxb,
+                                                          const float2* __restrict__ part, long prows, float* __restrict__ xo, long ldxo,
+                                                          bf16_t* __restrict__ xbo, long ldxbo, float2* __restrict__ parto, long prowso,
+                                                          long rows, int gin, int gout, int off, int xskip, int xrows, int C) {
+    const int lane = threadIdx.x & 63;
+    const long i = (long)blockIdx.x * 4 + (threadIdx.x >> 6);
+    if (i >= rows) return;
+    const long g = i / gin;
+    const int r = (int)(i - g * gin);
+    const long src = g * gout + off + r;
+    const uint4* sb = reinterpret_cast<const uint4*>(xb + src * ldxb);
+    uint4* db = reinterpret_cast<uint4*>(xbo + i * ldxbo);
+    for (int c = lane; c < C / 8; c += 64) db[c] = sb[c];
+    for (int p = lane; p < C / 64; p += 64) parto[p * prowso + i] = part[p * prows + src];
+    if ((unsigned)(r - xskip) < (unsigned)xrows) {
+        const float4* sx = reinterpret_cast<const float4*>(x + src * ldx);
+        float4* dx = reinterpret_cast<float4*>(xo + (g * xrows + r - xskip) * ldxo);
+        for (int c = lane; c < C / 4; c += 64) dx[c] = sx[c];
     }
 }
 
@@ -918,6 +939,29 @@
     return M324_OK;
 }
 
+extern "C" int m324_fold_gather(const float* x, long ldx, const void* xb, long ldxb, const float* part, long part_rows, float* x_out,
+                                long ldx_out, void* xb_out, long ldxb_out, float* part_out, long part_out_rows, int G, int gin, int gout,
+                                int off, int x_skip, int x_rows, int C, void* stream) {
+    M324_REQUIRE(x && xb && part && x_out && xb_out && part_out, "m324_fold_gather: null pointer");
+    M324_REQUIRE(G > 0 && gin > 0 && off >= 0 && (long)off + gin <= gout && x_skip >= 0 && x_rows > 0 && (long)x_skip + x_rows <= gin,
+                 "m324_fold_gather: bad row groups G=%d gin=%d gout=%d off=%d x_skip=%d x_rows=%d", G, gin, gout, off, x_skip, x_rows);
+    M324_REQUIRE(C > 0 && C % 64 == 0, "m324_fold_gather: C=%d must be a multiple of 64 (one table plane per 64 columns)", C);
+    const long rows = (long)G * gin, last = (long)(G - 1) * gout + off + gin;
+    M324_REQUIRE(ldx >= C && ldx_out >= C && ldx % 4 == 0 && ldx_out % 4 == 0 && ldxb >= C && ldxb_out >= C && ldxb % 8 == 0 &&
+                     ldxb_out % 8 == 0 && part_rows >= last && part_out_rows >= rows,
+                 "m324_fold_gather: leading dimensions must cover C in whole 16-byte pieces and the tables their rows");
+    M324_REQUIRE(((uintptr_t)x % 16) == 0 && ((uintptr_t)x_out % 16) == 0 && ((uintptr_t)xb % 16) == 0 && ((uintptr_t)xb_out % 16) == 0 &&
+                     ((uintptr_t)part % 8) == 0 && ((uintptr_t)part_out % 8) == 0,
+                 "m324_fold_gather: misaligned operands");
+    M324_REQUIRE(rows / 4 < (1l << 31) - 1, "m324_fold_gather: grid too large");
+    hipLaunchKernelGGL(fold_gather_kernel, dim3((unsigned)((rows + 3) / 4)), dim3(256), 0, (hipStream_t)stream, x, ldx,
+                       static_cast<const bf16_t*>(xb), ldxb, reinterpret_cast<const float2*>(part), part_rows, x_out, ldx_out,
+                       static_cast<bf16_t*>(xb_out), ldxb_out, reinterpret_cast<float2*>(part_out), part_out_rows, rows, gin, gout, off,
+                       x_skip, x_rows, C);
+    M324_CHECK_LAUNCH("m324_fold_gather");
+    return M324_OK;
+}
+
 extern "C" int m324_layernorm_in(const void* x, int x_dtype, long ldx, const float* w, const float* b, float eps, void* y, long ldy,
                                  int out_dtype, int rows, int C, int gin, int gout, int off, void* stream) {
     if (x_dtype == M324_F32) return m324_layernorm((const float*)x, ldx, w, b, eps, y, ldy, out_dtype, rows, C, gin, gout, off, stream);
diff --git a/motion324_amd/csrc/gemm.hip b/motion324_amd/csrc/gemm.hip
--- a/motion324_amd/csrc/gemm.hip
+++ b/motion324_amd/csrc/gemm.hip
@@ -1191,14 +1191,17 @@
     rc = gemm_validate(b);
     if (rc != M324_OK) return rc;
     const GemmPlan pa = make_plan(a), pb = make_plan(b);
-    if (pa.variant != 13 || pa.actx != 4 || pb.variant != 13 || pb.actx != 4)
+    if (pa.variant != 13 || pb.variant != 13 || pa.actx != pb.actx || (pa.actx != 4 && pa.actx != 12) || pa.res != 0 || pb.res != 0)
         M324_FAIL(M324_ERR_UNSUPPORTED, "m324_gemm_pair: built for two bf16 head-major projections on the 128 x 128 chunk ring");
     auto problem = [](const m324_gemm_args* g, const GemmPlan& p) {
         return Ring2Problem{(const bf16_t*)g->A, g->lda, (const bf16_t*)g->W, g->ldw, g->C, g->ldc, g->M, g->N, g->K, make_epilogue(g),
                             ceil_div(g->N, BN), xcd_mode(g), (int)p.wg};
     };
     const Ring2Problem p0 = problem(a, pa), p1 = problem(b, pb);
-    hipLaunchKernelGGL((gemm_ring2_pair_kernel<bf16_t, 4, 0>), dim3(p0.tiles + p1.tiles), dim3(256), 0, (hipStream_t)stream, p0, p1);
+    if (pa.actx == 4)
+        hipLaunchKernelGGL((gemm_ring2_pair_kernel<bf16_t, 4, 0>), dim3(p0.tiles + p1.tiles), dim3(256), 0, (hipStream_t)stream, p0, p1);
+    else
+        hipLaunchKernelGGL((gemm_ring2_pair_kernel<bf16_t, 12, 0>), dim3(p0.tiles + p1.tiles), dim3(256), 0, (hipStream_t)stream, p0, p1);
     M324_CHECK_LAUNCH("m324_gemm_pair");
     return M324_OK;
 }
diff --git a/motion324_amd/lib.py b/motion324_amd/lib.py
--- a/motion324_amd/lib.py
+++ b/motion324_amd/lib.py
@@ -69,11 +69,13 @@
     "m324_n3_finish": [_P, _I, _I, _P, _P, _P],
     "m324_rowstats_finish": [_P, _I, _I, _F, _P, _P],
     "m324_rowstats": [_P, _L, _I, _I, _F, _P, _P, _L, _P],
+    "m324_fold_gather": [_P, _L, _P, _L, _P, _L, _P, _L, _P, _L, _P, _L, _I, _I, _I, _I, _I, _I, _I, _P],
     "m324_layernorm": [_P, _L, _P, _P, _F, _P, _L, _I, _I, _I, _I, _I, _I, _P],
     "m324_layernorm_in": [_P, _I, _L, _P, _P, _F, _P, _L, _I, _I, _I, _I, _I, _I, _P],
     "m324_layernorm_pair": [_P, _L, _P, _P, _F, _P, _L, _I, _I, _I, _I, _P, _L, _P, _P, _F, _P, _L, _I, _I, _I, _I, _I, _I, _P],
     "m324_qkv_split": [_P, _L, _P, _L, _P, _L, _P, _P, _F, _F, _P, _P, _P, _P, _P, _P, _I, _I, _I, _I, _P],
     "m324_attention": [_P, _L, _P, _P, _P, _L, _I, _I, _I, _I, _F, _I, _P, _I, _P],
+    "m324_attention_rows": [_P, _P, _P, _P, _L, _I, _I, _I, _I, _I, _I, _P],
     "m324_attention_merge": [_P, _P, _P, _P, _P, _P, _L, _P, _L, _I, _I, _I, _I, _P],
     "m324_patchify": [_P, _I, _I, _I, _I, _I, _P, _I, _I, _P],
     "m324_patchify_u8": [_P, _I, _I, _I, _I, _I, _P, _I, _I, _P],
diff --git a/motion324_amd/ops.py b/motion324_amd/ops.py
--- a/motion324_amd/ops.py
+++ b/motion324_amd/ops.py
@@ -365,7 +365,8 @@
         raise L.M324Error("gemm_pair: exactly two deferred projections")
     (a0, f0, b0, t0, _), (a1, f1, b1, t1, _) = deferred
     lib = L.load()
-    with span("gemm_bf16", f0 + f1, b0 + b1, f"gemm_ring2_pair_kernel<unsigned short, 4, 0> | {t0} + {t1}" if _timing() else "") as sp:
+    actx = 12 if a0.ln_rowstat else 4
+    with span("gemm_bf16", f0 + f1, b0 + b1, f"gemm_ring2_pair_kernel<unsigned short, {actx}, 0> | {t0} + {t1}" if _timing() else "") as sp:
         rc = lib.m324_gemm_pair(C.byref(a0), C.byref(a1), _stream())
         if rc == L.ERR_UNSUPPORTED:
             sp.cancel()
@@ -420,6 +421,25 @@
     with span("hbm_pass", 0.0, rows * Cdim * (4.0 + (2.0 if copy is not None else 0.0)), f"rowstats_kernel | rows={rows} C={Cdim}" if _timing() else ""):
         L.check(L.load().m324_rowstats(px, ldx, rows, Cdim, eps, _p(rowstat), pc, ldc, _stream()), "m324_rowstats")
     return rowstat
+
+
+def fold_gather(x: torch.Tensor, xb: torch.Tensor, part: torch.Tensor, G: int, rows: tuple, gout: int, x_rows: tuple):
+    (gin, off), (xn, xskip) = rows, x_rows
+    M, Cdim = x.shape
+    if (x.dtype != torch.float32 or xb.dtype != torch.bfloat16 or tuple(xb.shape) != (M, Cdim) or part.dtype != torch.float32
+            or not part.is_contiguous() or Cdim % 64 or tuple(part.shape) != (Cdim // 64, M, 2)):
+        raise L.M324Error(f"fold_gather: x {x.dtype}{tuple(x.shape)}, xb {xb.dtype}{tuple(xb.shape)}, part {part.dtype}{tuple(part.shape)}")
+    if G < 1 or gin < 1 or off < 0 or off + gin > gout or (G - 1) * gout + off + gin > M or xskip < 0 or xn < 1 or xskip + xn > gin:
+        raise L.M324Error(f"fold_gather: groups G={G} gin={gin} gout={gout} off={off} x_rows={x_rows} outside {M} rows")
+    xo = torch.empty((G * xn, Cdim), dtype=torch.float32, device=x.device)
+    xbo = torch.empty((G * gin, Cdim), dtype=torch.bfloat16, device=x.device)
+    parto = torch.empty((Cdim // 64, G * gin, 2), dtype=torch.float32, device=x.device)
+    (px, ldx), (pb, ldb) = _rows(x, "x"), _rows(xb, "xb")
+    nbytes = float(G) * (gin * (4.0 * Cdim + Cdim // 64 * 16.0) + xn * 8.0 * Cdim)
+    with span("hbm_pass", 0.0, nbytes, f"fold_gather_kernel | rows={G * gin} C={Cdim}" if _timing() else ""):
+        L.check(L.load().m324_fold_gather(px, ldx, pb, ldb, _p(part), M, _p(xo), Cdim, _p(xbo), Cdim, _p(parto), G * gin, G, gin, gout,
+                                          off, xskip, xn, Cdim, _stream()), "m324_fold_gather")
+    return xo, xbo, parto
 
 
 def layernorm(x: torch.Tensor, w: torch.Tensor, b: Optional[torch.Tensor], eps: float, out: torch.Tensor,
@@ -511,6 +531,31 @@
               if _timing() else ""):
         L.check(L.load().m324_attention(_p(Q), qbs, _p(K), _p(Vt), po, ldo, B, H, Lq, Lk, scale, flags, _p(lse), code_of(Q.dtype), _stream()),
                 "m324_attention")
+    return out
+
+
+ROWS_KERNEL = "attn_bf16_kernel<true, 1, 4, true, 2>"
+
+
+def attention_rows_plan(B: int, H: int, Lq: int, Lk: int) -> bool:
+    return _attn_plan(B, H, Lq, Lk, 3, BF16).startswith(ROWS_KERNEL)
+
+
+def attention_rows(Q: torch.Tensor, K: torch.Tensor, V: torch.Tensor, out: torch.Tensor, window: tuple) -> torch.Tensor:
+    B, H, Lk, _ = K.shape
+    Lq = Q.shape[2]
+    lo, n = window
+    if (tuple(Q.shape) != (B, H, Lq, 64) or tuple(K.shape) != (B, H, Lk, 64) or tuple(V.shape) != (B, H, Lk, 64)
+            or not (Q.is_contiguous() and K.is_contiguous() and V.is_contiguous())
+            or any(t.dtype != torch.bfloat16 for t in (Q, K, V, out))):
+        raise L.M324Error(f"attention_rows: Q{tuple(Q.shape)} K{tuple(K.shape)} V{tuple(V.shape)} (contiguous bf16 [B, H, L, 64])")
+    po, ldo = _rows(out, "out")
+    if out.shape[0] < B * n or out.shape[1] < H * 64 or lo < 0 or n < 1 or lo + n > Lq:
+        raise L.M324Error(f"attention_rows: window {window} of {Lq} rows, out {tuple(out.shape)}")
+    with span("attention_bf16", 4.0 * B * H * Lq * Lk * 64, 128.0 * H * B * (Lq + 2 * Lk + n),
+              f"attn_bf16_rows_kernel | B={B} H={H} Lq={Lq} Lk={Lk} rows={lo}+{n}" if _timing() else ""):
+        L.check(L.load().m324_attention_rows(_p(Q), _p(K), _p(V), po, ldo, B, H, Lq, Lk, lo, n, _stream()), "m324_attention_rows")
+    _wrote(out)
     return out
 
 
diff --git a/motion324_amd/switches.py b/motion324_amd/switches.py
--- a/motion324_amd/switches.py
+++ b/motion324_amd/switches.py
@@ -15,6 +15,7 @@
     "M324_FOLD_LN": ("2", "transformer.FOLD_LN", "LayerNorm fold: 0 off, 1 bf16 streams only (the decoder), 2 every stream (trunk, DINO too)"),
     "M324_FOLD_MERGE": ("1", "transformer.FOLD_MERGE", "LayerNorm fold: the consumer GEMM merges the producer's per-block row statistics itself (0: m324_rowstats_finish launch between them)"),
     "M324_PAIR_PROJ": ("1", "transformer.PAIR_PROJ", "bf16 inference, decoder: norm_q + norm_kv in one launch and the q + k|v projections in one launch when the q projection runs inside the block (0: four launches)"),
+    "M324_LATENT_TAIL": ("1", "transformer.LATENT_TAIL", "bf16 inference: the trunk's last per-frame block projects keys and values for every row and runs everything else on the latent rows the decoder reads (QK_Norm_TransformerBlock.run_rows; 0: the full block)"),
     "M324_ATTN_BOUNDED": ("1", "transformer.ATTN_BOUNDED", "bf16 inference, long sequences: softmax without a reference maximum when the q / k RMSNorm weights bound every score (M324_ATTN_SCORES_BOUNDED)"),
     "M324_FUSE_QKV": ("1", "transformer.FUSE_QKV", "bf16 inference: q|k|v projection epilogue writes head-major Q / K / V (RMSNorm, pre-scale)"),
     "M324_FUSE_QKV_VT": ("1", "transformer.FUSE_QKV_VT", "the same for long sequences: the epilogue writes the transposed, key-permuted V"),
diff --git a/motion324_amd/transformer.py b/motion324_amd/transformer.py
--- a/motion324_amd/transformer.py
+++ b/motion324_amd/transformer.py
@@ -95,6 +95,7 @@
 PAIR_PROJ = switches.flag("M324_PAIR_PROJ")
 FOLD_MERGE = switches.flag("M324_FOLD_MERGE")
 ATTN_BOUNDED = switches.flag("M324_ATTN_BOUNDED")
+LATENT_TAIL = switches.flag("M324_LATENT_TAIL")
 
 
 class LNFold:
@@ -229,6 +230,10 @@
 
 def fuse_proj(P: Prepared, rows: int) -> bool:
     return FUSE_QKV and not _FUSE_OFF and P.dtype == torch.bfloat16 and rows > 64 and not torch.is_grad_enabled()
+
+
+def _wave_cover(off: int, n: int, L: int) -> tuple:
+    return off // 32 * 32, min(L, -(-(off + n) // 32) * 32)
 
 
 class QK_Norm_TransformerBlock(nn.Module):
@@ -313,6 +318,40 @@
         ops.gemm(h, P.mat(a.fc.weight), x, bias=P.vec(a.fc.bias), residual=x, **out_kw())
         return _mlp_residual(P, self.norm2, self.mlp, x, fold, feed_next, mx=mlp_mx)
 
+    def rows_usable(self, P: Prepared, B: int, L: int, rows: tuple, fold: Optional[LNFold]) -> bool:
+        n, off = rows
+        C = self.attn.dim
+        lo, hi = _wave_cover(off, n, L)
+        return bool(LATENT_TAIL and fold is not None and fold.pending and FOLD_MERGE and C <= 1024 and C % 128 == 0
+                    and 0 <= off and n >= 1 and off + n <= L and LNFold.usable(P, B * n, C) and fuse_qkv(P, B * L, L) and L < 2048
+                    and not mx_role(P, "trunk.qkv") and not mx_role(P, "trunk.mlp")
+                    and ops.attention_rows_plan(B, self.attn.num_heads, L, L) and ops.attention_rows_plan(B, self.attn.num_heads, hi - lo, L))
+
+    def run_rows(self, P: Prepared, x: torch.Tensor, B: int, L: int, rows: tuple, fold: LNFold) -> torch.Tensor:
+        n, off = rows
+        a = self.attn
+        C, H = a.dim, a.num_heads
+        dev = x.device
+        lo, hi = _wave_cover(off, n, L)
+        nq = hi - lo
+        xc, xbq, partq = ops.fold_gather(x, fold.xb, fold.part, B, (nq, lo), L, (n, off - lo))
+        qw, kw = a._qk_w(P)
+        w, cs, bias = P.folded(self.norm1.weight, self.norm1.bias, a.to_qkv.weight, a.to_qkv.bias)
+        eps = self.norm1.eps
+        Q = torch.empty((B, H, nq, 64), dtype=P.dtype, device=dev)
+        K, V = (torch.empty((B, H, L, 64), dtype=P.dtype, device=dev) for _ in range(2))
+        pair: list = []
+        ops.gemm(fold.xb, w[C:], None, bias=None if bias is None else bias[C:], ln=(fold.part, cs[C:], eps),
+                 qkv_heads=(None, K, V, None, kw, RMS_EPS, 1.0, L, H, False), defer=pair)
+        ops.gemm(xbq, w[:C], None, bias=None if bias is None else bias[:C], ln=(partq, cs[:C], eps),
+                 qkv_heads=(Q, None, None, qw, None, RMS_EPS, ops.Q_PRESCALE, nq, H), defer=pair)
+        ops.gemm_pair(pair)
+        h = torch.empty((B * n, C), dtype=P.dtype, device=dev)
+        ops.attention_rows(Q, K, V, h, (off - lo, n))
+        tail = LNFold(xc)
+        ops.gemm(h, P.mat(a.fc.weight), xc, bias=P.vec(a.fc.bias), residual=xc, **tail.producer())
+        return _mlp_residual(P, self.norm2, self.mlp, xc, tail, feed_next=False)
+
     def forward(self, x: torch.Tensor) -> torch.Tensor:
         B, L, C = x.shape
         P = Prepared.for_module(self, x.device)
```

Measured after the change: 3555 frames/s (median of 6 runs). No clear change (+0.9%).
